# cebarker1000/heatflow

Hardware: AMD Instinct MI355X
Metric: DOF-updates/s (timesteps/s x nDOF) on geballe_with_diamond (higher is better)
Workload: dtype f64

## Files before the change

### heatflow_amd/csrc/heatflow_hip.hip

```cpp

#include "hf_amg_io.hpp"

namespace {

struct MeshTables {
  std::vector<int32_t> rowptr, colidx;
  ColDict spmv;
  RowGather rg;
  std::vector<char> tag_used;
  int max_blk_nnz = 0;
};

constexpr char BLOB_MAGIC[8] = {'H', 'F', 'P', 'A', 'T', '0', '2', 0};
struct BlobHeader {
  char magic[8];
  int64_t total_bytes, nnz;
  int32_t n, ne, rba, ts, max_blk_nnz, tab_len, rg_ok, rg_max_dict, spmv_max_dict, reserved;
  int64_t count[12];
};

void steady_swap(hf_ctx* ctx) {
  hf_ctx::Steady& S = ctx->steady;
  std::swap(ctx->nbc, S.nbc); std::swap(ctx->d_bc_dofs, S.bc_dofs); std::swap(ctx->d_g, S.g);
  std::swap(ctx->nlift_rows, S.nlift_rows); std::swap(ctx->nlift, S.nlift);
// ... 918 lines not shown
    ctx->pred_iters = 0;
    ctx->scheme = scheme;
  }
  return HF_OK;
}

int kt_set_tables(hf_ctx* ctx, bool cap, int32_t n_tab, const int32_t* tags, const double* t0, const double* dT, const int32_t* n_knots,
                  const double* values) {
  const char* fn = cap ? "hf_set_rhoc_tables" : "hf_set_kappa_tables";
  const char* what = cap ? "rho_c(T)" : "kappa(T)";
  if (!ctx) return HF_ERR_ARG;
  if (!ctx->have_mesh) return fail(ctx, HF_ERR_STATE, "%s before hf_set_mesh", fn);
  if (n_tab < 0) return fail(ctx, HF_ERR_ARG, "%s: negative table count", fn);
  HF_HIP(hipSetDevice(ctx->dev));
  hf_ctx::KappaT& K = ctx->kt;
  if (n_tab == 0) {
    if (ctx->steady.picard) ctx->steady.ready = false;
    if (cap ? K.c_on : K.k_on) {
      free_batch(ctx);
      ctx->assembled = false;
      ctx->pred_iters = 0;
    }
    if (!(cap ? K.k_on : K.c_on)) { kt_free(ctx); return HF_OK; }
    if (cap ? K.c_on : K.k_on) {
      const std::vector<KTab> none(64, KTab{0.0, 0.0, 0, 0});
      HF_HIP(copy_sync(ctx, cap ? K.chdr : K.hdr, none.data(), sizeof(KTab) * 64, hipMemcpyHostToDevice));
      dev_free(cap ? &K.cvals : &K.vals);
      (cap ? K.ctabled : K.tabled).clear();
      (cap ? K.c_on : K.k_on) = false;
      K.have_change = false;
    }
    return HF_OK;
  }
  if (!tags || !t0 || !dT || !n_knots || !values) return fail(ctx, HF_ERR_ARG, "%s: null pointer", fn);
  if (ctx->an.on) return fail(ctx, HF_ERR_STATE, "%s: anisotropic conductivities are set (hf_set_anisotropy; the table kernels are isotropic)", fn);
  if (!ctx->rg_ok || (ctx->assembled && ctx->mode != HF_ASM_ROW_GATHER))
    return fail(ctx, HF_ERR_ARG, "%s: %s is evaluated by the row-gather kernel only (HF_ASM_ROW_GATHER on a mesh with row-gather lists)", fn, what);
  if (cap && ct_smem_bytes(ctx->max_blk_nnz, ctx->rg_max_dict) + 2 * 64 * sizeof(KTab) > 160 * 1024)
    return fail(ctx, HF_ERR_ARG, "%s: the (M, A) slab, the staged state and the table headers of this mesh exceed the 160 KiB of LDS", fn);
  std::vector<KTab> hdr(64, KTab{0.0, 0.0, 0, 0});
  std::vector<double> vals;
  std::vector<char> tabled(ctx->tab_len, 0);
  for (int32_t i = 0; i < n_tab; ++i) {
    const int32_t tg = tags[i];
    if (tg < 0 || tg >= ctx->tab_len || !ctx->h_tag_used[tg]) return fail(ctx, HF_ERR_ARG, "%s: tag %d is not a cell tag of the mesh", fn, tg);
    if (tabled[tg]) return fail(ctx, HF_ERR_ARG, "%s: tag %d listed twice", fn, tg);
    if (n_knots[i] < 2 || n_knots[i] > KT_MAX_KNOTS)
      return fail(ctx, HF_ERR_ARG, "%s: table of tag %d has %d knots (2..%d)", fn, tg, n_knots[i], KT_MAX_KNOTS);
    if (!std::isfinite(t0[i]) || !(dT[i] > 0.0) || !std::isfinite(dT[i]) || !std::isfinite(t0[i] + (n_knots[i] - 1) * dT[i]))
      return fail(ctx, HF_ERR_ARG, "%s: table of tag %d: T0 finite and dT > 0 needed", fn, tg);
    tabled[tg] = 1;
    const size_t q = std::find(ctx->h_rg_tags.begin(), ctx->h_rg_tags.end(), tg) - ctx->h_rg_tags.begin();
    if (q >= ctx->h_rg_tags.size()) return fail(ctx, HF_ERR_ARG, "%s: tag %d has no row-gather dictionary entry", fn, tg);
    hdr[q] = KTab{t0[i], 1.0 / dT[i], n_knots[i], static_cast<int>(vals.size())};
    for (int32_t k = 0; k < n_knots[i]; ++k) {
      const double v = values[vals.size()];
      if (!(v > 0.0) || !std::isfinite(v)) return fail(ctx, HF_ERR_ARG, "%s: value %d of the table of tag %d is not positive and finite", fn, k, tg);
      vals.push_back(v);
    }
  }
  free_batch(ctx);
  if (ctx->steady.picard) ctx->steady.ready = false;
  if (!K.hdr) {
    HF_TRY(dev_alloc(ctx, &K.hdr, 64));
    HF_TRY(dev_alloc(ctx, &K.pic, ctx->n));
    HF_TRY(dev_alloc(ctx, &K.b0, ctx->n));
    HF_TRY(dev_alloc(ctx, &K.change, 1));
  }
  if (cap && !K.chdr) {
    HF_TRY(dev_alloc(ctx, &K.chdr, 64));
    HF_TRY(dev_alloc(ctx, &K.w, ctx->n));
    if (!K.k_on) {
      const std::vector<KTab> none(64, KTab{0.0, 0.0, 0, 0});
      HF_HIP(copy_sync(ctx, K.hdr, none.data(), sizeof(KTab) * 64, hipMemcpyHostToDevice));
    }
  }
  double*& dvals = cap ? K.cvals : K.vals;
  dev_free(&dvals);
  HF_TRY(dev_alloc(ctx, &dvals, vals.size()));
  HF_HIP(copy_sync(ctx, cap ? K.chdr : K.hdr, hdr.data(), sizeof(KTab) * 64, hipMemcpyHostToDevice));
  HF_HIP(copy_sync(ctx, dvals, vals.data(), sizeof(double) * vals.size(), hipMemcpyHostToDevice));
  (cap ? K.ctabled : K.tabled) = std::move(tabled);
  (cap ? K.c_on : K.k_on) = true;
  K.on = true;
  K.have_change = false;
  ctx->assembled = false;
  ctx->pred_iters = 0;
  return HF_OK;
}

int hf_set_kappa_tables(hf_ctx* ctx, int32_t n_tab, const int32_t* tags, const double* t0, const double* dT, const int32_t* n_knots,
                        const double* values, int32_t picard_sweeps) {
  if (ctx && ctx->have_mesh && n_tab > 0 && tags && t0 && dT && n_knots && values &&
      (picard_sweeps < 1 || picard_sweeps > KT_MAX_PICARD))
    return fail(ctx, HF_ERR_ARG, "hf_set_kappa_tables: picard_sweeps %d outside 1..%d", picard_sweeps, KT_MAX_PICARD);
  HF_TRY(kt_set_tables(ctx, false, n_tab, tags, t0, dT, n_knots, values));
  if (n_tab > 0) ctx->kt.picard = picard_sweeps;
  return HF_OK;
}

int hf_set_rhoc_tables(hf_ctx* ctx, int32_t n_tab, const int32_t* tags, const double* t0, const double* dT, const int32_t* n_knots,
                       const double* values) {
  return kt_set_tables(ctx, true, n_tab, tags, t0, dT, n_knots, values);
}

int hf_set_picard(hf_ctx* ctx, int32_t sweeps) {
  if (!ctx) return HF_ERR_ARG;
  if (sweeps < 1 || sweeps > KT_MAX_PICARD) return fail(ctx, HF_ERR_ARG, "hf_set_picard: sweeps %d outside 1..%d", sweeps, KT_MAX_PICARD);
  if (!ctx->kt.on) return fail(ctx, HF_ERR_STATE, "hf_set_picard: no tables are set (hf_set_kappa_tables / hf_set_rhoc_tables first)");
  ctx->kt.picard = sweeps;
  return HF_OK;
}

int hf_get_picard_change(hf_ctx* ctx, double* max_du) {
  if (!ctx || !max_du) return HF_ERR_ARG;
  if (!ctx->kt.on || !ctx->kt.have_change) return fail(ctx, HF_ERR_STATE, "hf_get_picard_change: no step with kappa(T) tables since they were set");
  HF_HIP(hipSetDevice(ctx->dev));
  unsigned long long bits = 0;
  HF_HIP(copy_sync(ctx, &bits, ctx->kt.change, sizeof bits, hipMemcpyDeviceToHost));
  std::memcpy(max_du, &bits, sizeof bits);
  return HF_OK;
}

int hf_set_start_vector(hf_ctx* ctx, int32_t kind) {
  if (!ctx) return HF_ERR_ARG;
  if (kind < 0 || kind > 3) return fail(ctx, HF_ERR_ARG, "hf_set_start_vector: unknown kind %d", kind);
  ctx->start_kind = kind;
  ctx->extrapolate = kind >= 1 ? 1 : 0;
  if (kind == 0) ctx->have_prev = false;
  return HF_OK;
}

int hf_get_response_solves(hf_ctx* ctx, int64_t* count) {
  if (!ctx || !count) return HF_ERR_ARG;
  *count = ctx->resp_solves;
  return HF_OK;
}

int hf_get_amg_fallbacks(hf_ctx* ctx, int64_t* count) {
  if (!ctx || !count) return HF_ERR_ARG;
  *count = ctx->amg_fallbacks;
  return HF_OK;
}

int hf_get_amg_info(hf_ctx* ctx, int32_t* n_levels, int32_t* level_rows, int32_t max_levels, double* op_complexity,
                    double* setup_seconds) {
  if (!ctx) return HF_ERR_ARG;
  const int nl = ctx->amg_ready ? static_cast<int>(ctx->amg.size()) : 0;
  if (n_levels) *n_levels = nl;
  if (level_rows)
    for (int l = 0; l < nl && l < max_levels; ++l) level_rows[l] = ctx->amg[l].n;
  if (op_complexity) *op_complexity = ctx->amg_ready ? ctx->amg_opc : 0.0;
  if (setup_seconds) *setup_seconds = ctx->amg_ready ? ctx->amg_setup_s : 0.0;
  return HF_OK;
}

int hf_amg_export_size(hf_ctx* ctx, int64_t* bytes) {
  if (!ctx || !bytes) return HF_ERR_ARG;
  if (!ctx->amg_ready || !ctx->assembled) return fail(ctx, HF_ERR_STATE, "hf_amg_export_size: no multigrid hierarchy (hf_set_precond(1, ...) and hf_assemble first)");
  BlobOut o;
  o.ctx = ctx;
  HF_TRY(walk_hierarchy(ctx, o, ctx->amg_print));
  *bytes = static_cast<int64_t>(o.at);
  return HF_OK;
}

int hf_amg_export(hf_ctx* ctx, void* blob, int64_t bytes) {
  if (!ctx || !blob) return HF_ERR_ARG;
  if (!ctx->amg_ready || !ctx->assembled) return fail(ctx, HF_ERR_STATE, "hf_amg_export: no multigrid hierarchy (hf_set_precond(1, ...) and hf_assemble first)");
  HF_HIP(hipSetDevice(ctx->dev));
  BlobOut sz;
  sz.ctx = ctx;
  HF_TRY(walk_hierarchy(ctx, sz, ctx->amg_print));
  if (bytes != static_cast<int64_t>(sz.at)) return fail(ctx, HF_ERR_ARG, "hf_amg_export: buffer of %lld bytes, need %lld", (long long)bytes, (long long)sz.at);
  std::vector<unsigned char> host(sz.at, 0);
  BlobOut o;
  o.ctx = ctx;
  o.dst = host.data();
  HF_TRY(walk_hierarchy(ctx, o, ctx->amg_print));
  HF_HIP(hipStreamSynchronize(ctx->stream));
  HF_HIP(hipMemcpy(blob, host.data(), host.size(), hipMemcpyDefault));
  return HF_OK;
}

int hf_amg_install(hf_ctx* ctx, const void* blob, int64_t bytes) {
  if (!ctx || !blob || bytes <= 0) return HF_ERR_ARG;
  if (!ctx->have_mesh) return fail(ctx, HF_ERR_STATE, "hf_amg_install before hf_set_mesh");
  if (ctx->precond != 1 || !ctx->amg_reuse) return fail(ctx, HF_ERR_STATE, "hf_amg_install needs hf_set_precond(1, reuse = 1): an installed hierarchy is a kept one");
  HF_HIP(hipSetDevice(ctx->dev));
  free_batch(ctx);
  std::vector<unsigned char> staged;
  const unsigned char* src = nullptr;
  HF_TRY(blob_on_host(ctx, blob, bytes, staged, &src));
  HF_TRY(install_hierarchy(ctx, src, static_cast<size_t>(bytes)));
  ctx->assembled = false;
  return HF_OK;
}

int hf_flux_setup(hf_ctx* ctx) {
  if (!ctx) return HF_ERR_ARG;
  if (!ctx->have_mesh) return fail(ctx, HF_ERR_STATE, "hf_flux_setup before hf_set_mesh");
  HF_HIP(hipSetDevice(ctx->dev));
  const int n = ctx->n;
  HF_TRY(dev_alloc(ctx, &ctx->d_M1, ctx->nnz));
  HF_TRY(dev_alloc(ctx, &ctx->d_dinv1, n));
  HF_TRY(dev_alloc(ctx, &ctx->d_gz, n));
  HF_TRY(dev_alloc(ctx, &ctx->d_gr, n));
  HF_TRY(dev_alloc(ctx, &ctx->d_bz, n));
  HF_TRY(dev_alloc(ctx, &ctx->d_br, n));
  const int tab = ctx->rg_ok ? 64 : ctx->tab_len;
  DevTemp<double> t_one, t_zero, t_scratch;
  double *&d_one = t_one.p, *&d_zero = t_zero.p, *&d_scratch = t_scratch.p;
  HF_TRY(dev_alloc(ctx, &d_one, tab));
  HF_TRY(dev_alloc(ctx, &d_zero, tab));
  HF_TRY(dev_alloc(ctx, &d_scratch, ctx->nnz));
  std::vector<double> ones(tab, 1.0), zeros(tab, 0.0);
  HF_HIP(copy_sync(ctx, d_one, ones.data(), sizeof(double) * tab, hipMemcpyHostToDevice));
  HF_HIP(copy_sync(ctx, d_zero, zeros.data(), sizeof(double) * tab, hipMemcpyHostToDevice));
  if (ctx->rg_ok) HF_TRY(launch_assemble_rows(ctx, d_zero, d_one, 0.0, ctx->d_M1, d_scratch));
  else HF_TRY(launch_assemble_lds(ctx, true, d_zero, d_one, 0.0, ctx->d_M1, d_scratch));
  hipLaunchKernelGGL(k_dinv, dim3((n + 255) / 256), dim3(256), 0, ctx->stream, n, ctx->d_rowptr, ctx->d_colidx,
                     ctx->d_M1, ctx->d_dinv1);
  HF_HIP(hipMemsetAsync(ctx->d_gz, 0, sizeof(double) * n, ctx->stream));
  HF_HIP(hipMemsetAsync(ctx->d_gr, 0, sizeof(double) * n, ctx->stream));
  HF_HIP(hipGetLastError());
  HF_HIP(hipStreamSynchronize(ctx->stream));
  {
    hf_ctx::Batch& F = ctx->fluxb;
    free_batch_state(F);
    const size_t vec = static_cast<size_t>(n) * 2;
    for (double** v : {&F.u, &F.b, &F.r, &F.p, &F.Ap, &F.z}) {
      HF_TRY(dev_alloc(ctx, v, vec));
      HF_HIP(hipMemsetAsync(*v, 0, sizeof(double) * vec, ctx->stream));
    }
    HF_TRY(dev_alloc(ctx, &F.part_pAp, 2 * static_cast<size_t>(MAXP)));
    HF_TRY(dev_alloc(ctx, &F.part_rz, 4 * static_cast<size_t>(MAXP)));
    HF_TRY(dev_alloc(ctx, &F.part_zz, 2 * static_cast<size_t>(MAXP)));
    HF_TRY(dev_alloc(ctx, &F.part_bn, 2 * static_cast<size_t>(MAXP)));
    HF_TRY(dev_alloc(ctx, &F.scal, 2));
    HF_TRY(dev_alloc(ctx, &F.red, 1));
    HF_HIP(hipMemsetAsync(F.scal, 0, sizeof(Scal) * 2, ctx->stream));
    HF_HIP(hipMemsetAsync(F.red, 0, sizeof(BRed), ctx->stream));
    if (hipHostMalloc(reinterpret_cast<void**>(&F.h_scal), sizeof(Scal) * 2) != hipSuccess) return fail(ctx, HF_ERR_ALLOC, "hipHostMalloc failed");
    F.Pb = static_cast<int>(std::min<size_t>((static_cast<size_t>(n) + 127) / 128, MAXP));
    if (F.Pb >= 64) F.Pb &= ~7;
    F.nv = 2; F.opk = 0; F.pred_iters = 0;
    F.sysA = ctx->d_M1; F.sysDinv = ctx->d_dinv1;
    HF_HIP(hipStreamSynchronize(ctx->stream));
  }
  ctx->flux_ready = true;
  ctx->pred_flux[0] = ctx->pred_flux[1] = 0;
  return HF_OK;
}

int hf_flux_solve(hf_ctx* ctx, int32_t components, double rtol, int32_t max_it, int32_t* iters) {
  if (!ctx) return HF_ERR_ARG;
  if (!ctx->flux_ready) return fail(ctx, HF_ERR_STATE, "hf_flux_solve before hf_flux_setup");
  if (max_it <= 0 || rtol < 0 || components < 0 || components > 3) return fail(ctx, HF_ERR_ARG, "hf_flux_solve: bad arguments");
  HF_HIP(hipSetDevice(ctx->dev));
  const bool both = components == 3 && ctx->rg_ok && ctx->fluxb.nv == 2;
  if (ctx->rg_ok) {
    const int capd = ctx->rg_max_dict;
    const size_t sm = static_cast<size_t>(capd) * 16 + static_cast<size_t>(capd + (capd & 1)) * 8 + (RBA + 4) * 4 +
                      (static_cast<size_t>((ctx->max_blk_nnz + 1) & ~1) / 8 + 3) * 16;
    const int grid = std::min(ctx->nblk_a, 2048);
    hipLaunchKernelGGL(k_grad_rows, dim3(grid), dim3(RBA), sm, ctx->stream, ctx->nblk_a, capd, ctx->d_rg_hdr,
                       reinterpret_cast<const uint4*>(ctx->d_rg_ell), reinterpret_cast<const uint4*>(ctx->d_rg_cid), ctx->d_rg_zrb,
                       ctx->d_rg_dict, ctx->d_rowptr, ctx->d_u, both ? ctx->fluxb.b : ctx->d_bz, both ? ctx->fluxb.b + 1 : ctx->d_br,
                       both ? 2 : 1, 1, 0);
  } else {
    HF_TRY(ensure_owner_lists(ctx));
    hipLaunchKernelGGL(k_grad_rhs, dim3(ctx->nblk_a), dim3(RBA), 0, ctx->stream, ctx->n, ctx->d_blk_eptr, ctx->d_blk_ent,
                       ctx->d_zr, ctx->d_u, ctx->d_bz, ctx->d_br);
  }
  HF_HIP(hipGetLastError());
  if (both) {
    std::swap(ctx->batch, ctx->fluxb);
    const int rc = BatchOps<2, OP_SHARED>::pcg(ctx, false, rtol, 0.0, max_it);
    const int it0 = ctx->batch.h_scal[0].iters, it1 = ctx->batch.h_scal[1].iters;
    std::swap(ctx->batch, ctx->fluxb);
    if (iters) { iters[0] = it0; iters[1] = it1; }
    ctx->flux_valid = 0;
    if (rc != HF_OK) return rc;
    hipLaunchKernelGGL(kb_get_column, dim3(1024), dim3(256), 0, ctx->stream, static_cast<size_t>(ctx->n), 2, 0, ctx->fluxb.u, ctx->d_gz);
    hipLaunchKernelGGL(kb_get_column, dim3(1024), dim3(256), 0, ctx->stream, static_cast<size_t>(ctx->n), 2, 1, ctx->fluxb.u, ctx->d_gr);
    HF_HIP(hipGetLastError());
    ctx->flux_valid = 3;
    return HF_OK;
  }
  if (iters) iters[0] = iters[1] = 0;
  ctx->flux_valid = 0;
  if (components & 1) {
    const LinSys sz{ctx->d_M1, ctx->d_dinv1, ctx->d_gz, ctx->d_bz};
    const int rc = pcg_solve(ctx, sz, false, rtol, 0.0, max_it, &ctx->pred_flux[0]);
    if (iters) iters[0] = ctx->h_scal->iters;
    if (rc != HF_OK) return rc;
    ctx->flux_valid |= 1;
  }
  if (components & 2) {
    const LinSys sr{ctx->d_M1, ctx->d_dinv1, ctx->d_gr, ctx->d_br};
    const int rc = pcg_solve(ctx, sr, false, rtol, 0.0, max_it, &ctx->pred_flux[1]);
    if (iters) iters[1] = ctx->h_scal->iters;
    if (rc != HF_OK) return rc;
    ctx->flux_valid |= 2;
  }
  return HF_OK;
// ... 1274 lines not shown
```

### heatflow_amd/csrc/hf_context.hpp

```cpp

#pragma once
#include <hip/hip_runtime.h>
#include <hip/hip_ext.h>

#include <algorithm>
#include <chrono>
#include <cmath>
#include <cstdarg>
#include <cstdint>
#include <cstdio>
#include <cstdlib>
#include <cstring>
#include <string>
#include <thread>
#include <vector>

#include "amg_host.hpp"
#include "heatflow_hip.h"

namespace {

constexpr int RB = 256;
#ifndef HF_RBA
#define HF_RBA 256
// ... 31 lines not shown
  unsigned long long tested_st;
};
inline int mirror_tested(const ScalMirror* m, unsigned epoch) {
  const unsigned long long v = __atomic_load_n(&m->tested_st, __ATOMIC_ACQUIRE);
  return static_cast<unsigned>(v >> 32) == epoch ? static_cast<int>(v & 0xffffffffu) - 1 : -1;
}
inline int mirror_done(const ScalMirror* m, unsigned epoch) {
  const unsigned long long v = __atomic_load_n(&m->done_st, __ATOMIC_ACQUIRE);
  return static_cast<unsigned>(v >> 32) == epoch ? static_cast<int>(v & 0xffffffffu) : 0;
}

struct Scal {
  double tol2;
  double bn2;
  double zz;
  int iters;
  int done;
  int first;
  unsigned epoch;
  ScalMirror* mirror;
};

constexpr int NV_MAX = 16;
struct BRed { double pAp[NV_MAX], rz[2][NV_MAX], zz[NV_MAX], bn[NV_MAX]; };

constexpr int KT_MAX_KNOTS = 256;
constexpr int KT_MAX_PICARD = 8;
struct KTab { double t0, inv_dt; int n, off; };

struct TanDir { int32_t c_r, c_z; double w_r, w_z; };

enum RgVariant { RG_ROWS, RG_ROWS_K, RG_AN, RG_AN_K, RG_KT, RG_CT, RG_KT_K, RG_SOURCE, RG_SHAPE1, RG_SHAPE2, RG_SHAPE4, RG_VARIANTS };

}

struct hf_ctx {
  int dev = 0;
  hipStream_t stream = nullptr;
  hipEvent_t ev0 = nullptr, ev1 = nullptr;
  std::string err;
  double last_ms = 0.0;

  int32_t n = 0, ne = 0, nbc = 0;
  int64_t nnz = 0;
  int nchunks = 0, P = 0;
  int nchunks_s = 0, Ps = 0;
  int max_chunk_nnz_s = 0;
  int32_t *d_cdict_ptr = nullptr, *d_cdict = nullptr;
  uint16_t* d_cid = nullptr;
  int max_cdict = 0;
  bool cdict_own = false;
  bool c16 = true;
  struct ValueLists {
    const double* src = nullptr;
    int32_t *vptr = nullptr, *count = nullptr, *info = nullptr;
    double* vlist = nullptr;
    uint32_t* cv = nullptr;
    int64_t cap = 0;
    int64_t sum_vlist = 0;
    int max_vlist = 0;
    bool valid = false;
  } vl[2];
  int vl_mode = 1;
  int vl_vcap = 0;
  int vl_occ = 0;
  bool have_mesh = false, have_mat = false, assembled = false;
  double dt = 0.0;
  double dt_step = 0.0;
  int mode = 0;
  int scheme = HF_TIME_BACKWARD_EULER;

  std::vector<int32_t> h_rowptr, h_colidx, h_tri, h_tag;
  std::vector<char> h_tag_used;
  bool owner_ready = false;

  double2* d_zr = nullptr;
  int4* d_elem = nullptr;
  int tab_len = 0;
  double *d_kappa = nullptr, *d_rhoc = nullptr;
  int32_t *d_rowptr = nullptr, *d_colidx = nullptr;
  int32_t *d_blk_eptr = nullptr, *d_blk_cptr = nullptr;
  int2* d_blk_ent = nullptr;
  int nblk_a = 0;
  int max_blk_nnz = 0, ncolors = 0;
  int64_t elist_len = 0;
  bool rg_ok = false;
  int4* d_rg_hdr = nullptr;
  uint16_t *d_rg_ell = nullptr, *d_rg_cid = nullptr;
  int32_t* d_rg_dict = nullptr;
  double2* d_rg_zrb = nullptr;
  int rg_max_dict = 0;
  int rg_grid[RG_VARIANTS] = {};
  int64_t n_rg_ell = 0, n_rg_dict = 0, n_cdict = 0;
  std::vector<int32_t> h_rg_tags;
  double *d_kappa_rg = nullptr, *d_rhoc_rg = nullptr;
  struct Aniso {
    bool on = false;
    double2* d_m = nullptr;
    std::vector<char> h_tag;
    std::vector<double> h_m;
    uint64_t hash = 0;
  } an;
  double *d_M = nullptr, *d_A = nullptr, *d_dinv = nullptr;
  int32_t* d_bc_dofs = nullptr;
  double* d_g = nullptr;
  int32_t nlift_rows = 0, nlift = 0;
  int32_t *d_lift_rows = nullptr, *d_lift_ptr = nullptr, *d_lift_bc = nullptr, *d_lift_slot = nullptr;
  double* d_lift_val = nullptr;
  double *d_u = nullptr, *d_b = nullptr, *d_r = nullptr, *d_p = nullptr, *d_Ap = nullptr;
  double *d_uprev = nullptr, *d_ustart = nullptr;
  bool have_prev = false;
  bool bdf_hist = false;
  int extrapolate = 1;
  int start_kind = 3;
  std::vector<double> h_g0, h_g1;
  int g_hist = 0;
  struct BcResponse { std::vector<double> dir; double* w = nullptr; };
  std::vector<BcResponse> resp;
  long long resp_solves = 0;
  struct Proj {
    double *V[PROJ_MT] = {nullptr}, *F[PROJ_MT] = {nullptr};
    bool used[PROJ_MT] = {false};
    int next = 0, pending = -1;
    double *G = nullptr, *alpha = nullptr, *part = nullptr;
    bool ready = false;
  } proj;
  double *d_tmp = nullptr;
  double *d_part_pAp = nullptr, *d_part_rz = nullptr, *d_part_zz = nullptr, *d_part_bn = nullptr;
  Scal* d_scal = nullptr;
  Scal* h_scal = nullptr;
  ScalMirror* h_mirror = nullptr;
  ScalMirror* d_mirror = nullptr;
  unsigned epoch = 0;
  int32_t* d_samp_idx = nullptr;
  double* d_samp = nullptr;
  int samp_cap = 0;
  int pred_iters = 0;
  int precond = 0;
  int amg_reuse = 0;
  bool amg_ready = false;
  struct DevCsr {
    int nrow = 0, ncol = 0, lanes = 8; int64_t nnz = 0; int32_t *ptr = nullptr, *idx = nullptr; double* val = nullptr;
    float* valf = nullptr;
    int max_row = 0;
    int rpc = 0, nchunks = 0, chunk_nnz = 0;
    int32_t *dptr = nullptr, *dict = nullptr;
    uint16_t* cid = nullptr;
    int max_dict = 0;
    int64_t ndict = 0;
  };
  struct DevLevel {
    DevCsr A, P, R, Rt, GP;
    double *dinv = nullptr, *x = nullptr, *cat = nullptr, *b = nullptr, *res = nullptr;
    bool own_b = false;
    double omega = 0; int n = 0;
  };
  std::vector<DevLevel> amg;
  double* d_coarse_inv = nullptr;
  float* d_coarse_inv_f = nullptr;
  int coarse_n = 0, coarse_ld = 0;
  bool amg_fine_stale = false;
  int amg_fuse0 = 0;
  bool amg_f32 = true;
  double amg_opc = 0.0, amg_setup_s = 0.0;
  struct OperatorPrint { double dt = 0.0; std::vector<double> kappa, rhoc; int32_t nbc = 0; uint64_t bc_hash = 0; int32_t scheme = 0; uint64_t an_hash = 0; } amg_print;
  long long amg_fallbacks = 0;
  struct Steady {
    bool ready = false;
    bool picard = false;
    KTab* hdr0 = nullptr;
    double* xprev = nullptr;
    unsigned long long* change = nullptr;
    int precond = 0, pred_iters = 0;
    int32_t nbc = 0, nlift_rows = 0, nlift = 0;
    int32_t *bc_dofs = nullptr, *lift_rows = nullptr, *lift_ptr = nullptr, *lift_bc = nullptr, *lift_slot = nullptr;
    double *g = nullptr, *lift_val = nullptr, *K = nullptr, *dinv = nullptr, *Kfree = nullptr;
    std::vector<DevLevel> amg;
    double* coarse_inv = nullptr;
    float* coarse_inv_f = nullptr;
    int coarse_n = 0, coarse_ld = 0;
    bool amg_ready = false, amg_fine_stale = false;
    double amg_opc = 0.0, amg_setup_s = 0.0;
    OperatorPrint amg_print;
  } steady;
  double* d_load = nullptr;
  bool have_load = false;
  struct Source {
    bool on = false;
    double* F1 = nullptr;
    double* sum = nullptr;
    int32_t* absorb = nullptr;
    std::vector<double> amp;
    size_t next = 0;
  } src;
  double *d_z = nullptr, *d_z2 = nullptr;
  bool flux_ready = false;
  int flux_valid = 0;
  double *d_M1 = nullptr, *d_dinv1 = nullptr, *d_gz = nullptr, *d_gr = nullptr, *d_bz = nullptr, *d_br = nullptr;
  int pred_flux[2] = {0, 0};
  struct BatchLevel { double *x = nullptr, *cat = nullptr, *b = nullptr, *res = nullptr; bool own_b = false; };
  struct Batch {
    int nv = 0;
    int opk = 0;
    const double *sysA = nullptr, *sysDinv = nullptr;
    double *A = nullptr, *dinv = nullptr, *lift_val = nullptr;
    double *A1 = nullptr, *lift1 = nullptr;
    double delta[NV_MAX] = {};
    double *g = nullptr;
    double *u = nullptr, *uprev = nullptr, *ustart = nullptr, *b = nullptr, *r = nullptr, *p = nullptr, *Ap = nullptr;
    double *z = nullptr, *z2 = nullptr, *tmp = nullptr;
    double *part_pAp = nullptr, *part_rz = nullptr, *part_zz = nullptr, *part_bn = nullptr;
    Scal *scal = nullptr, *h_scal = nullptr;
    ScalMirror *h_mirror = nullptr, *d_mirror = nullptr;
    unsigned epoch = 0;
    BRed* red = nullptr;
    std::vector<BatchLevel> lev;
    int Pb = 0, pred_iters = 0;
    bool have_prev = false;
    bool bdf_hist = false;
    double *pV[PROJ_MH] = {nullptr}, *pF[PROJ_MH] = {nullptr}, *pG = nullptr, *palpha = nullptr, *ppart = nullptr;
    bool pused[PROJ_MH] = {false};
    int pnext = 0, ppending = -1;
    unsigned loaded = 0;
    bool lds = false;
    const double* load = nullptr;
  } batch;
  struct BatchCols {
    int nv = 0, rpc = 0, nchunks = 0, cap_nnz = 0, cap_dict = 0;
    int32_t *ptr = nullptr, *dict = nullptr, *own = nullptr;
    uint16_t* id = nullptr;
  } bcols;
  Batch fluxb;
  Batch fluxnb;
  int32_t* d_fsamp_idx = nullptr;
  Batch tanb;
  struct Tangent {
    bool ready = false;
    int npar = 0, nv = 0;
    int32_t* col = nullptr;
    TanDir* dir = nullptr;
    double* F = nullptr;
    bool steady_state = false;
    std::vector<int64_t> lev_sig;
    struct Shape {
      int ncol = 0, ns = 0;
      int32_t col[4] = {0, 0, 0, 0};
      std::vector<double> h_v[4];
      double* d_v = nullptr;
      double *un = nullptr, *um1 = nullptr;
      int wmode = 0;
      bool hist = false;
    } sh;
  } tan;
  int fsamp_cap = 0;
  struct KappaT {
    bool on = false;
    bool k_on = false, c_on = false;
    int picard = 1;
    KTab* hdr = nullptr;
    double* vals = nullptr;
    std::vector<char> tabled;
    KTab* chdr = nullptr;
    double* cvals = nullptr;
    std::vector<char> ctabled;
    double* w = nullptr;
    double *pic = nullptr, *b0 = nullptr;
    unsigned long long* change = nullptr;
    bool have_change = false;
  } kt;
  bool prof = false;
  std::vector<hipEvent_t> prof_ev;
  int prof_used = 0, prof_base = 0;
  double prof_spmv_ms = 0.0;
  long long prof_spmv_n = 0;
};

namespace {

int fail(hf_ctx* c, int code, const char* fmt, ...);
inline size_t pad16(size_t b) { return (b + 15) & ~static_cast<size_t>(15); }

inline void cpu_relax() {
#if defined(__x86_64__) || defined(__i386__)
  __builtin_ia32_pause();
#else
  std::this_thread::yield();
#endif
}

hipError_t copy_sync(hf_ctx* ctx, void* dst, const void* src, size_t bytes, hipMemcpyKind kind) {
  if (bytes == 0) return hipSuccess;
  const hipError_t e = hipMemcpyAsync(dst, src, bytes, kind, ctx->stream);
  return e != hipSuccess ? e : hipStreamSynchronize(ctx->stream);
}

int fail(hf_ctx* c, int code, const char* fmt, ...) {
  char buf[512];
  va_list ap;
  va_start(ap, fmt);
  vsnprintf(buf, sizeof buf, fmt, ap);
  va_end(ap);
  if (c) c->err = buf;
  return code;
}

#define HF_HIP(call)                                                                          \
// ... 34 lines not shown
```

### heatflow_amd/csrc/hf_kernels.hpp

```cpp
#pragma once
#include <type_traits>

#include "hf_context.hpp"

namespace {


template <int NW = 4>
__device__ __forceinline__ double block_sum(double v, double* sw) {
#pragma unroll
  for (int o = 32; o > 0; o >>= 1) v += __shfl_down(v, o, 64);
  const int w = threadIdx.x >> 6;
  if ((threadIdx.x & 63) == 0) sw[w] = v;
  __syncthreads();
  double t = sw[0];
#pragma unroll
  for (int k = 1; k < NW; ++k) t += sw[k];
  __syncthreads();
  return t;
}

__device__ __forceinline__ double sum_partials(const double* __restrict__ part, int P, double* s4) {
  double v = 0.0;
  for (int k = threadIdx.x; k < P; k += TPB) v += part[k];
  return block_sum(v, s4);
}

#ifndef HF_XCD_MAP
#define HF_XCD_MAP 1
#endif
struct ChunkIter {
  int chunk, step, end;
  __device__ __forceinline__ ChunkIter(int nchunks) {
    if (HF_XCD_MAP && (gridDim.x & 7) == 0) {
      const int per = (nchunks + 7) >> 3;
      const int xcd = blockIdx.x & 7;
      chunk = xcd * per + (blockIdx.x >> 3);
      step = gridDim.x >> 3;
      end = min(nchunks, (xcd + 1) * per);
    } else {
      chunk = blockIdx.x;
      step = gridDim.x;
      end = nchunks;
    }
  }
};

__device__ __forceinline__ void element_local(const double2 p0, const double2 p1, const double2 p2, double rho_c,
                                              double kappa, double m[6], double k[6]) {
#pragma clang fp contract(off)
  const double d = (p1.x - p0.x) * (p2.y - p0.y) - (p2.x - p0.x) * (p1.y - p0.y);
  const double area = 0.5 * fabs(d);
  const double b0 = p1.y - p2.y, b1 = p2.y - p0.y, b2 = p0.y - p1.y;
  const double c0 = p2.x - p1.x, c1 = p0.x - p2.x, c2 = p1.x - p0.x;
  const double rsum = (p0.y + p1.y) + p2.y;
  const double ks = kappa * area * (rsum / 3.0) / (d * d);
  k[0] = ks * (b0 * b0 + c0 * c0);
  k[1] = ks * (b1 * b1 + c1 * c1);
  k[2] = ks * (b2 * b2 + c2 * c2);
  k[3] = ks * (b0 * b1 + c0 * c1);
  k[4] = ks * (b0 * b2 + c0 * c2);
  k[5] = ks * (b1 * b2 + c1 * c2);
  const double ms = rho_c * area;
  m[0] = ms * ((2.0 * p0.y + rsum) / 30.0);
  m[1] = ms * ((2.0 * p1.y + rsum) / 30.0);
  m[2] = ms * ((2.0 * p2.y + rsum) / 30.0);
  m[3] = ms * ((rsum + p0.y + p1.y) / 60.0);
  m[4] = ms * ((rsum + p0.y + p2.y) / 60.0);
  m[5] = ms * ((rsum + p1.y + p2.y) / 60.0);
}

__device__ __forceinline__ int sym_index(int a, int b) {
  return a == b ? a : (a + b + 2);
}

struct AsmEntry { int n0, n1, n2; unsigned w3, off03, off47; };

__device__ __forceinline__ AsmEntry load_entry(const int2* __restrict__ ent, int q) {
  const int2 a = ent[3 * q], b = ent[3 * q + 1], c = ent[3 * q + 2];
  return AsmEntry{a.x, a.y, b.x, static_cast<unsigned>(b.y), static_cast<unsigned>(c.x), static_cast<unsigned>(c.y)};
}

template <bool COLORED>
__global__ __launch_bounds__(RBA) void k_assemble_lds(int n, int cap, const int32_t* __restrict__ rowptr,
                                                      const int32_t* __restrict__ blk_eptr,
                                                      const int32_t* __restrict__ blk_cptr,
                                                      const int2* __restrict__ blk_ent,
                                                      const double2* __restrict__ zr,
                                                      const double* __restrict__ kappa_tab,
                                                      const double* __restrict__ rhoc_tab, double dt,
                                                      double* __restrict__ Mv, double* __restrict__ Av) {
  extern __shared__ double smem[];
  double2* sMA = reinterpret_cast<double2*>(smem);
  double* sM = smem;
  double* sA = smem + cap;
  int* sR = reinterpret_cast<int*>(smem + 2 * cap);

  const int blk = blockIdx.x;
  const int r0 = blk * RBA;
  const int r1 = min(n, r0 + RBA);
  const int k0 = rowptr[r0];
  const int nk = rowptr[r1] - k0;
  for (int k = threadIdx.x; k < nk; k += RBA) {
    if (COLORED) {
      sMA[k] = make_double2(0.0, 0.0);
    } else {
      sM[k] = 0.0;
      sA[k] = 0.0;
    }
  }
  for (int k = threadIdx.x; k <= r1 - r0; k += RBA) sR[k] = rowptr[r0 + k] - k0;
  __syncthreads();

  auto scatter = [&](const AsmEntry e, const double2 p0, const double2 p1, const double2 p2) {
    double m[6], kk[6], av6[6];
    const int tag = static_cast<int>(e.w3 >> 11);
    element_local(p0, p1, p2, rhoc_tab[tag], kappa_tab[tag], m, kk);
#pragma unroll
    for (int q = 0; q < 6; ++q) av6[q] = fma(dt, kk[q], m[q]);
    const int nd[3] = {e.n0, e.n1, e.n2};
#pragma unroll
    for (int a = 0; a < 3; ++a) {
      if (!((e.w3 >> (8 + a)) & 1u)) continue;
      const int base = sR[nd[a] - r0];
#pragma unroll
      for (int b = 0; b < 3; ++b) {
        const int q9 = a * 3 + b;
        const unsigned off = q9 < 4 ? (e.off03 >> (8 * q9)) & 0xFFu : q9 < 8 ? (e.off47 >> (8 * (q9 - 4))) & 0xFFu : e.w3 & 0xFFu;
        const int slot = base + static_cast<int>(off);
        const int q = sym_index(a, b);
        if (COLORED) {
          double2 t = sMA[slot];
          t.x += m[q];
          t.y += av6[q];
          sMA[slot] = t;
        } else {
          atomicAdd(&sM[slot], m[q]);
          atomicAdd(&sA[slot], av6[q]);
        }
      }
    }
  };
  constexpr int NF = 3;
  auto run_range = [&](int e0, int e1) {
    for (int k = e0 + threadIdx.x; k < e1; k += NF * RBA) {
      AsmEntry e[NF];
      double2 pa[NF], pb[NF], pc[NF];
#pragma unroll
      for (int u = 0; u < NF; ++u) e[u] = load_entry(blk_ent, min(k + u * RBA, e1 - 1));
#pragma unroll
      for (int u = 0; u < NF; ++u) { pa[u] = zr[e[u].n0]; pb[u] = zr[e[u].n1]; pc[u] = zr[e[u].n2]; }
#pragma unroll
      for (int u = 0; u < NF; ++u)
        if (k + u * RBA < e1) scatter(e[u], pa[u], pb[u], pc[u]);
    }
  };

  if (COLORED) {
    const int32_t* cp = blk_cptr + static_cast<size_t>(blk) * (NCOL + 1);
    for (int c = 0; c < NCOL; ++c) {
      const int e0 = cp[c], e1 = cp[c + 1];
      if (e0 == e1) { if (e1 == cp[NCOL]) break; else continue; }
      run_range(e0, e1);
      __syncthreads();
    }
  } else {
    run_range(blk_eptr[blk], blk_eptr[blk + 1]);
  }
  __syncthreads();
  for (int k = threadIdx.x; k < nk; k += RBA) {
    if (COLORED) {
      const double2 t = sMA[k];
      Mv[k0 + k] = t.x;
      Av[k0 + k] = t.y;
    } else {
      Mv[k0 + k] = sM[k];
      Av[k0 + k] = sA[k];
    }
  }
}

struct ElemRow { double m0, m1, m2, k0, k1, k2; };

__device__ __forceinline__ double sorted_sum3(double a, double b, double c) {
#pragma clang fp contract(off)
  const double ab_lo = fmin(a, b), ab_hi = fmax(a, b);
  const double lo = fmin(ab_lo, c), hi = fmax(ab_hi, c), mid = fmax(ab_lo, fmin(ab_hi, c));
  return (lo + mid) + hi;
}

template <bool ANISO>
__device__ __forceinline__ ElemRow element_row_of(const double2 Pi, const double2 Pj, const double2 Pk, double rho_c, double k_z, double k_r) {
#pragma clang fp contract(off)
  const double eix = Pk.x - Pj.x, eiy = Pk.y - Pj.y;
  const double ejx = Pi.x - Pk.x, ejy = Pi.y - Pk.y;
// ... 777 lines not shown
#pragma clang fp contract(off)
    const AsmEntry e = load_entry(blk_ent, q);
    const double2 p0 = zr[e.n0], p1 = zr[e.n1], p2 = zr[e.n2];
    const double u0 = u[e.n0], u1 = u[e.n1], u2 = u[e.n2];
    const double d = (p1.x - p0.x) * (p2.y - p0.y) - (p2.x - p0.x) * (p1.y - p0.y);
    const double area = 0.5 * fabs(d);
    const double gz = (u0 * (p1.y - p2.y) + u1 * (p2.y - p0.y) + u2 * (p0.y - p1.y)) / d;
    const double gr = (u0 * (p2.x - p1.x) + u1 * (p0.x - p2.x) + u2 * (p1.x - p0.x)) / d;
    const double rsum = (p0.y + p1.y) + p2.y;
    const double wgt[3] = {area * (p0.y + rsum) / 12.0, area * (p1.y + rsum) / 12.0, area * (p2.y + rsum) / 12.0};
    const int nd[3] = {e.n0, e.n1, e.n2};
    const unsigned owned = (e.w3 >> 8) & 7u;
#pragma unroll
    for (int a = 0; a < 3; ++a) {
      if (!((owned >> a) & 1u)) continue;
      atomicAdd(&sB[2 * (nd[a] - r0)], gz * wgt[a]);
      atomicAdd(&sB[2 * (nd[a] - r0) + 1], gr * wgt[a]);
    }
  }
  __syncthreads();
  for (int k = threadIdx.x; k < r1 - r0; k += RBA) {
    bz[r0 + k] = sB[2 * k];
    br[r0 + k] = sB[2 * k + 1];
  }
}

__global__ void k_take_lift(int nlift, const int32_t* __restrict__ slot, double* __restrict__ A,
                            double* __restrict__ val) {
  const int q = blockIdx.x * blockDim.x + threadIdx.x;
  if (q >= nlift) return;
  val[q] = A[slot[q]];
  A[slot[q]] = 0.0;
}

__global__ void k_bc_rows(int nbc, const int32_t* __restrict__ dofs, const int32_t* __restrict__ rowptr,
                          const int32_t* __restrict__ colidx, double* __restrict__ A) {
  const int q = blockIdx.x * blockDim.x + threadIdx.x;
  if (q >= nbc) return;
  const int row = dofs[q];
  for (int k = rowptr[row]; k < rowptr[row + 1]; ++k) A[k] = (colidx[k] == row) ? 1.0 : 0.0;
}

__global__ void k_dinv(int n, const int32_t* __restrict__ rowptr, const int32_t* __restrict__ colidx,
                       const double* __restrict__ A, double* __restrict__ dinv) {
  const int row = blockIdx.x * blockDim.x + threadIdx.x;
  if (row >= n) return;
  double d = 0.0;
  for (int k = rowptr[row]; k < rowptr[row + 1]; ++k)
    if (colidx[k] == row) d = A[k];
  dinv[row] = 1.0 / d;
}

__global__ void k_lift(int nrows, const int32_t* __restrict__ rows, const int32_t* __restrict__ ptr,
                       const int32_t* __restrict__ bc, const double* __restrict__ val,
                       const double* __restrict__ g, double* __restrict__ b) {
  const int q = blockIdx.x * blockDim.x + threadIdx.x;
  if (q >= nrows) return;
  double s = 0.0;
  for (int k = ptr[q]; k < ptr[q + 1]; ++k) s += val[k] * g[bc[k]];
  b[rows[q]] -= s;
}

__global__ void k_set_bc(int nbc, const int32_t* __restrict__ dofs, const double* __restrict__ g,
                         double* __restrict__ b, double* __restrict__ u) {
  const int q = blockIdx.x * blockDim.x + threadIdx.x;
  if (q >= nbc) return;
  b[dofs[q]] = g[q];
  u[dofs[q]] = g[q];
}

__global__ void k_gather(int ns, const int32_t* __restrict__ idx, const double* __restrict__ u,
                         double* __restrict__ out) {
  const int q = blockIdx.x * blockDim.x + threadIdx.x;
  if (q < ns) out[q] = u[idx[q]];
}

__global__ __launch_bounds__(TPB) void k_hold_load(int n, const int32_t* __restrict__ rowptr, const int32_t* __restrict__ colidx,
                                                   const double* __restrict__ K, const double* __restrict__ u,
                                                   const unsigned char* __restrict__ mask, double* __restrict__ F) {
  const int row = blockIdx.x * blockDim.x + threadIdx.x;
  if (row >= n) return;
  double s = 0.0;
  if (!mask[row])
    for (int k = rowptr[row]; k < rowptr[row + 1]; ++k) s += K[k] * u[colidx[k]];
  F[row] = s;
}

__global__ void k_mark_rows(int nq, const int32_t* __restrict__ idx, unsigned char* __restrict__ mask) {
  const int q = blockIdx.x * blockDim.x + threadIdx.x;
  if (q < nq) mask[idx[q]] = 1;
}

__device__ __forceinline__ unsigned long long mirror_stamp(unsigned epoch, int v) {
  return (static_cast<unsigned long long>(epoch) << 32) | static_cast<unsigned>(v);
}
__device__ __forceinline__ void mirror_publish(ScalMirror* m, double zz, int iters, int done, unsigned epoch) {
  if (m == nullptr) return;
  m->zz = zz;
  m->iters = iters;
  __hip_atomic_store(&m->done_st, mirror_stamp(epoch, done), __ATOMIC_RELAXED, __HIP_MEMORY_SCOPE_SYSTEM);
  __threadfence_system();
  __hip_atomic_store(&m->tested_st, mirror_stamp(epoch, iters + 1), __ATOMIC_RELEASE, __HIP_MEMORY_SCOPE_SYSTEM);
}
__device__ __forceinline__ void mirror_breakdown(ScalMirror* m, unsigned epoch) {
  if (m != nullptr) __hip_atomic_store(&m->done_st, mirror_stamp(epoch, 2), __ATOMIC_RELEASE, __HIP_MEMORY_SCOPE_SYSTEM);
}

struct ColComp { const int32_t* dptr; const int32_t* dict; const uint16_t* id; int xd_off; int own; };
struct ValComp : ColComp { const int32_t* vptr; const double* vlist; const uint32_t* cv; int vl_off; int vcap; };

#ifndef HF_NT_STREAM
#define HF_NT_STREAM 0
#endif
#ifndef HF_PIPE
#define HF_PIPE 1
#endif
#ifndef HF_PHASE_CLOCK
#define HF_PHASE_CLOCK -1
#endif
#if HF_PHASE_CLOCK >= 0
#ifndef HF_PHASE_CONV
#define HF_PHASE_CONV 0
#endif
__device__ unsigned long long g_phase[MAXP * 16];
#define HF_STAMP(slot)                                                                                   \
  do {                                                                                                   \
    if (MODE == HF_PHASE_CLOCK && C16 && (MODE != 0 || (part2 != nullptr) == (HF_PHASE_CONV != 0)) && threadIdx.x == 0 && (slot) < 16) \
      g_phase[blockIdx.x * 16 + (slot)] = wall_clock64();                                                \
  } while (0)
#else
#define HF_STAMP(slot) do { } while (0)
#endif
template <typename T>
__device__ __forceinline__ T stream_load(const T* p) {
#if HF_NT_STREAM
  return __builtin_nontemporal_load(p);
#else
  return *p;
#endif
}

__device__ __forceinline__ double bdf2_operand(double un, double unm1) { return (4.0 * un - unm1) * (1.0 / 3.0); }

template <int MODE, bool C16 = false, typename VT = double, int UN = 8, bool VC = false>
__global__ __launch_bounds__(TS) __attribute__((amdgpu_waves_per_eu(8, 8))) void k_spmv(int n, int nchunks, int rpc ,
                                              const int32_t* __restrict__ rowptr, const int32_t* __restrict__ colidx,
                                              const VT* __restrict__ vals, const double* __restrict__ x,
                                              double* __restrict__ y, Scal* __restrict__ scal,
                                              double* __restrict__ part0, const double* __restrict__ bvec,
                                              const double* __restrict__ dinv, double* __restrict__ pvec,
                                              double* __restrict__ part1, double* __restrict__ part2, double w,
                                              int npart ,
                                              int parity, typename std::conditional<VC, ValComp, ColComp>::type comp) {
  extern __shared__ double sprod[];
  __shared__ double s4[TS / 64];
  __shared__ int s_own;
  constexpr bool BDF = MODE >= 12 && MODE <= 15;
  auto opnd = [&](int c) { return BDF ? bdf2_operand(x[c], bvec[c]) : x[c]; };
  if ((MODE == 3 || MODE == 4 || MODE == 6 || MODE == 9) && scal->done) return;
  if ((MODE == 0 || MODE == 7) && scal != nullptr && scal->done) return;
  double acc0 = 0.0, acc1 = 0.0, acc2 = 0.0;
  double beta = 0.0;
  bool first9 = false;
  if (MODE == 9) {
    first9 = scal->first != 0;
    if (!first9) {
      double v0 = 0.0, v1 = 0.0, v2 = 0.0;
      for (int k = threadIdx.x; k < npart; k += TS) {
        v0 += part1[parity * MAXP + k];
        v1 += part1[(parity ^ 1) * MAXP + k];
        v2 += part2[k];
      }
      const double rz_new = block_sum<TS / 64>(v0, s4);
      const double rz_old = block_sum<TS / 64>(v1, s4);
      const double zz = block_sum<TS / 64>(v2, s4);
      const bool conv = zz <= scal->tol2;
      if (blockIdx.x == 0 && threadIdx.x == 0) {
        scal->zz = zz;
        if (conv) scal->done = 1;
      }
      if (conv) return;
      beta = rz_new / rz_old;
    }
  }
  auto cycle_gate = [&]() {
    if (!((MODE == 3 || MODE == 0) && part2 != nullptr)) return false;
    double v2 = 0.0;
    for (int k = threadIdx.x; k < npart; k += TS) v2 += part2[k];
    const double zz = block_sum<TS / 64>(v2, s4);
    const bool conv = zz <= scal->tol2;
    if (blockIdx.x == 0 && threadIdx.x == 0) {
      if (conv) { scal->zz = zz; scal->done = 1; }
      mirror_publish(scal->mirror, zz, scal->iters, conv ? 1 : 0, scal->epoch);
    }
    return conv;
  };
  constexpr bool PIPELINED = C16 && !VC && (HF_PIPE == 2 || (HF_PIPE == 1 && sizeof(VT) == 4));
  static_assert(!VC || (C16 && sizeof(VT) == 8), "value lists: the fine operator's f64 arrays on compressed columns");
  if (!PIPELINED && cycle_gate()) return;
  const ChunkIter sched(nchunks);
  HF_STAMP(0);
  int stamp_at = 1;
  (void)stamp_at;
  const int tpr = (MODE == 0 || MODE == 6 || MODE == 7) ? TS / rpc : 1;
  const int prel = static_cast<int>(threadIdx.x) / tpr;
  const int psub = static_cast<int>(threadIdx.x) % tpr;
  struct RowOps { double b, d, y, p, x; };
  auto row_operands = [&](int prc, bool from_slice) {
    RowOps e{0.0, 0.0, 0.0, 0.0, 0.0};
    if (MODE == 2 || MODE == 3 || MODE == 4 || MODE == 5 || MODE == 7 || MODE == 8 || MODE == 11 || MODE == 13 || MODE == 15) e.b = bvec[prc];
    if (MODE == 2 || MODE == 4 || MODE == 5 || MODE == 10 || MODE == 11 || MODE == 14 || MODE == 15) e.d = dinv[prc];
    if (MODE == 6 || (MODE == 9 && !first9)) e.y = y[prc];
    if (MODE == 9 && !first9) e.p = pvec[prc];
    if ((MODE == 4 || MODE == 8 || MODE == 9 || MODE == 11) && !from_slice) e.x = x[prc];
    if (BDF) e.x = x[prc];
    return e;
  };
  auto rows_phase = [&](bool pin, int prow, int pa, int pb, const RowOps& e) {
    if ((MODE == 0 || MODE == 6 || MODE == 7) && tpr > 1) {
      double s = 0.0;
      if (pin)
        for (int j = pa + psub; j < pb; j += tpr) s += sprod[j];
      for (int o = tpr >> 1; o > 0; o >>= 1) s += __shfl_down(s, o, 64);
      if (pin && psub == 0) {
        y[prow] = (MODE == 6) ? e.y + s : s;
        if (MODE == 7) acc0 += e.b * s;
      }
    } else if (pin) {
      const int row = prow;
      double s = 0.0;
      for (int j = pa; j < pb; ++j) s += sprod[j];
      if (MODE == 0) {
        y[row] = s;
      } else if (MODE == 2) {
        const double ri = e.b - s;
        const double zi = e.d * ri;
        y[row] = ri;
        pvec[row] = zi;
        acc0 += ri * zi;
        acc1 += zi * zi;
        acc2 += (e.d * e.b) * (e.d * e.b);
      } else if (MODE == 3) {
        y[row] = e.b - s;
      } else if (MODE == 4) {
        const double yi = e.x + w * e.d * (e.b - s);
        y[row] = yi;
        acc0 += e.b * yi;
      } else if (MODE == 5) {
        const double ri = e.b - s;
        y[row] = ri;
        pvec[row] = w * e.d * ri;
        acc1 += (e.d * ri) * (e.d * ri);
        acc2 += (e.d * e.b) * (e.d * e.b);
      } else if (MODE == 7) {
        y[row] = s;
        acc0 += e.b * s;
      } else if (MODE == 6) {
        y[row] = e.y + s;
      } else if (MODE == 8) {
        y[row] = s;
        pvec[row] = 2.0 * e.x - e.b;
      } else if (MODE == 10) {
        y[row] = s + w * e.d;
      } else if (MODE == 11) {
        y[row] = s + w * e.d;
        pvec[row] = 2.0 * e.x - e.b;
      } else if (BDF) {
        y[row] = (MODE == 14 || MODE == 15) ? s + w * e.d : s;
        pvec[row] = (MODE == 13 || MODE == 15) ? 2.0 * e.x - e.b : e.x;
      } else {
        const double api = first9 ? s : s + beta * e.y;
        const double pi = first9 ? e.x : e.x + beta * e.p;
        y[row] = api;
        pvec[row] = pi;
        acc0 += pi * api;
      }
    }
  };
  if (PIPELINED) {
    struct Bounds { int k0, k1, d0, d1; };
    auto bounds = [&](int ch) {
      Bounds q;
      const int a0 = ch * rpc, a1 = min(n, a0 + rpc);
      q.k0 = rowptr[a0]; q.k1 = rowptr[a1];
      q.d0 = comp.dptr[ch]; q.d1 = comp.dptr[ch + 1];
      return q;
    };
    int lhead[HF_STAGE_U];
    double v[UN];
    int id[UN];
    auto heads = [&](const Bounds& q, bool live) {
      const int dl = max(q.d1 - 1, 0), kl = max(q.k1 - 1, 0);
      const int t = static_cast<int>(threadIdx.x);
#pragma unroll
      for (int u = 0; u < HF_STAGE_U; ++u) lhead[u] = comp.dict[min(q.d0 + (live ? t + u * TS : (t & 31)), dl)];
      __builtin_amdgcn_sched_barrier(0);
#pragma unroll
      for (int u = 0; u < UN; ++u) {
        const int kk = min(q.k0 + (live ? t + u * TS : (t & 31)), kl);
        v[u] = static_cast<double>(stream_load(&vals[kk]));
        id[u] = static_cast<int>(stream_load(&comp.id[kk]));
      }
    };
    double* xd = sprod + comp.xd_off;
    Bounds cur = bounds(min(sched.chunk, nchunks - 1));
    heads(cur, sched.chunk < sched.end);
    if (cycle_gate()) return;
    for (int chunk = sched.chunk; chunk < sched.end; chunk += sched.step) {
      const bool more = chunk + sched.step < sched.end;
      const int r0 = chunk * rpc, r1 = min(n, r0 + rpc);
      const int k0 = cur.k0, k1 = cur.k1, d0 = cur.d0, nd = cur.d1 - cur.d0;
      const int prow = r0 + prel;
      const bool pin = prow < r1;
      const int prc = min(prow, r1 - 1);
      int c0[HF_STAGE_U];
      double x0[HF_STAGE_U];
#pragma unroll
      for (int u = 0; u < HF_STAGE_U; ++u) { c0[u] = lhead[u]; x0[u] = opnd(c0[u]); }
      const Bounds nxt = bounds(more ? chunk + sched.step : chunk);
      const int pa = rowptr[prc] - k0, pb = rowptr[prc + 1] - k0;
      RowOps e = row_operands(prc, comp.own != 0);
#pragma unroll
      for (int u = 0; u < HF_STAGE_U; ++u) {
        const int i = static_cast<int>(threadIdx.x) + u * TS;
        if (i < nd) {
          xd[i] = x0[u];
          if ((MODE == 4 || MODE == 8 || MODE == 9 || MODE == 11) && c0[u] == r0) s_own = i;
        }
      }
      for (int i = threadIdx.x + HF_STAGE_U * TS; i < nd; i += HF_STAGE_U * TS) {
        int c[HF_STAGE_U];
        double xv[HF_STAGE_U];
#pragma unroll
        for (int u = 0; u < HF_STAGE_U; ++u) c[u] = comp.dict[d0 + min(i + u * TS, nd - 1)];
#pragma unroll
        for (int u = 0; u < HF_STAGE_U; ++u) xv[u] = opnd(c[u]);
#pragma unroll
        for (int u = 0; u < HF_STAGE_U; ++u)
          if (i + u * TS < nd) {
            xd[i + u * TS] = xv[u];
            if ((MODE == 4 || MODE == 8 || MODE == 9 || MODE == 11) && c[u] == r0) s_own = i + u * TS;
          }
      }
      __syncthreads();
      HF_STAMP(stamp_at); ++stamp_at;
      if ((MODE == 4 || MODE == 8 || MODE == 9 || MODE == 11) && comp.own && pin) e.x = xd[s_own + (prow - r0)];
#pragma unroll
      for (int u = 0; u < UN; ++u) {
        const int kk = k0 + static_cast<int>(threadIdx.x) + u * TS;
        if (kk < k1) sprod[kk - k0] = v[u] * xd[id[u]];
      }
      for (int kb = k0 + UN * TS; kb < k1; kb += UN * TS) {
#pragma unroll
        for (int u = 0; u < UN; ++u) {
          const int kk = min(kb + static_cast<int>(threadIdx.x) + u * TS, k1 - 1);
          v[u] = static_cast<double>(stream_load(&vals[kk]));
          id[u] = static_cast<int>(stream_load(&comp.id[kk]));
        }
#pragma unroll
        for (int u = 0; u < UN; ++u) {
          const int kk = kb + static_cast<int>(threadIdx.x) + u * TS;
          if (kk < k1) sprod[kk - k0] = v[u] * xd[id[u]];
        }
      }
      heads(nxt, more);
      __syncthreads();
      HF_STAMP(stamp_at); ++stamp_at;
      rows_phase(pin, prow, pa, pb, e);
      __syncthreads();
      HF_STAMP(stamp_at); ++stamp_at;
      cur = nxt;
    }
  } else {
  const ChunkIter& sched_ = sched;
  for (int chunk = sched_.chunk; chunk < sched_.end; chunk += sched_.step) {
    const int r0 = chunk * rpc;
    const int r1 = min(n, r0 + rpc);
    const int k0 = rowptr[r0];
    const int k1 = rowptr[r1];
    const int prow = r0 + prel;
    const bool pin = prow < r1;
    int pa = 0, pb = 0;
    if (pin) {
      pa = rowptr[prow] - k0;
      pb = rowptr[prow + 1] - k0;
    }
    RowOps e = row_operands(min(prow, r1 - 1), C16 && comp.own != 0);
    if constexpr (VC) {
      double* xd = sprod + comp.xd_off;
      double* vl = sprod + comp.vl_off;
      const int d0 = comp.dptr[chunk], nd = comp.dptr[chunk + 1] - d0;
      const int v0 = comp.vptr[chunk], nv = comp.vptr[chunk + 1] - v0;
      const bool vin = nv <= comp.vcap;
      int k = k0 + threadIdx.x;
      std::uint32_t cw[HF_UNROLL];
#pragma unroll
      for (int u = 0; u < HF_UNROLL; ++u) cw[u] = (k + u * TS < k1) ? stream_load(&comp.cv[k + u * TS]) : 0u;
      double lv[2];
#pragma unroll
      for (int u = 0; u < 2; ++u) {
        const int i = static_cast<int>(threadIdx.x) + u * TS;
        lv[u] = (vin && i < nv) ? comp.vlist[v0 + i] : 0.0;
      }
      for (int i = threadIdx.x; i < nd; i += HF_STAGE_U * TS) {
        int c[HF_STAGE_U];
        double xv[HF_STAGE_U];
#pragma unroll
        for (int u = 0; u < HF_STAGE_U; ++u) c[u] = (i + u * TS < nd) ? comp.dict[d0 + i + u * TS] : 0;
#pragma unroll
        for (int u = 0; u < HF_STAGE_U; ++u) xv[u] = (i + u * TS < nd) ? opnd(c[u]) : 0.0;
#pragma unroll
        for (int u = 0; u < HF_STAGE_U; ++u)
          if (i + u * TS < nd) {
            xd[i + u * TS] = xv[u];
            if ((MODE == 4 || MODE == 8 || MODE == 9 || MODE == 11) && c[u] == r0) s_own = i + u * TS;
          }
      }
#pragma unroll
      for (int u = 0; u < 2; ++u) {
        const int i = static_cast<int>(threadIdx.x) + u * TS;
        if (vin && i < nv) vl[i] = lv[u];
      }
      if (vin)
        for (int i = threadIdx.x + 2 * TS; i < nv; i += TS) vl[i] = comp.vlist[v0 + i];
      __syncthreads();
      HF_STAMP(stamp_at); ++stamp_at;
      if ((MODE == 4 || MODE == 8 || MODE == 9 || MODE == 11) && comp.own && pin) e.x = xd[s_own + (prow - r0)];
      while (k < k1) {
        const int kn = k + HF_UNROLL * TS;
        std::uint32_t cn[HF_UNROLL];
#pragma unroll
        for (int u = 0; u < HF_UNROLL; ++u) cn[u] = (kn + u * TS < k1) ? stream_load(&comp.cv[kn + u * TS]) : 0u;
        if (vin) {
#pragma unroll
          for (int u = 0; u < HF_UNROLL; ++u)
            if (k + u * TS < k1) sprod[k - k0 + u * TS] = vl[cw[u] >> 16] * xd[cw[u] & 0xffffu];
        } else {
          double gv[HF_UNROLL];
#pragma unroll
          for (int u = 0; u < HF_UNROLL; ++u) gv[u] = (k + u * TS < k1) ? comp.vlist[v0 + static_cast<int>(cw[u] >> 16)] : 0.0;
#pragma unroll
          for (int u = 0; u < HF_UNROLL; ++u)
            if (k + u * TS < k1) sprod[k - k0 + u * TS] = gv[u] * xd[cw[u] & 0xffffu];
        }
#pragma unroll
        for (int u = 0; u < HF_UNROLL; ++u) cw[u] = cn[u];
        k = kn;
      }
    } else if (C16) {
      double* xd = sprod + comp.xd_off;
      const int d0 = comp.dptr[chunk], nd = comp.dptr[chunk + 1] - d0;
      int k = k0 + threadIdx.x;
      double v[HF_UNROLL];
      int id[HF_UNROLL];
#pragma unroll
      for (int u = 0; u < HF_UNROLL; ++u) {
        const bool in = k + u * TS < k1;
        v[u] = in ? static_cast<double>(stream_load(&vals[k + u * TS])) : 0.0;
        id[u] = in ? static_cast<int>(stream_load(&comp.id[k + u * TS])) : 0;
      }
      for (int i = threadIdx.x; i < nd; i += HF_STAGE_U * TS) {
        int c[HF_STAGE_U];
        double xv[HF_STAGE_U];
#pragma unroll
        for (int u = 0; u < HF_STAGE_U; ++u) c[u] = (i + u * TS < nd) ? comp.dict[d0 + i + u * TS] : 0;
#pragma unroll
        for (int u = 0; u < HF_STAGE_U; ++u) xv[u] = (i + u * TS < nd) ? opnd(c[u]) : 0.0;
#pragma unroll
        for (int u = 0; u < HF_STAGE_U; ++u)
          if (i + u * TS < nd) {
            xd[i + u * TS] = xv[u];
            if ((MODE == 4 || MODE == 8 || MODE == 9 || MODE == 11) && c[u] == r0) s_own = i + u * TS;
          }
      }
      __syncthreads();
      HF_STAMP(stamp_at); ++stamp_at;
      if ((MODE == 4 || MODE == 8 || MODE == 9 || MODE == 11) && comp.own && pin) e.x = xd[s_own + (prow - r0)];
      while (k < k1) {
        const int kn = k + HF_UNROLL * TS;
        double vn[HF_UNROLL];
        int idn[HF_UNROLL];
#pragma unroll
        for (int u = 0; u < HF_UNROLL; ++u) {
          const bool in = kn + u * TS < k1;
          vn[u] = in ? static_cast<double>(stream_load(&vals[kn + u * TS])) : 0.0;
          idn[u] = in ? static_cast<int>(stream_load(&comp.id[kn + u * TS])) : 0;
        }
#pragma unroll
        for (int u = 0; u < HF_UNROLL; ++u)
          if (k + u * TS < k1) sprod[k - k0 + u * TS] = v[u] * xd[id[u]];
#pragma unroll
        for (int u = 0; u < HF_UNROLL; ++u) { v[u] = vn[u]; id[u] = idn[u]; }
        k = kn;
      }
    } else {
      for (int k = k0 + threadIdx.x; k < k1; k += HF_UNROLL * TS) {
        int c[HF_UNROLL];
        double v[HF_UNROLL], xv[HF_UNROLL];
#pragma unroll
        for (int u = 0; u < HF_UNROLL; ++u) {
          const bool in = k + u * TS < k1;
          c[u] = in ? colidx[k + u * TS] : 0;
          v[u] = in ? static_cast<double>(vals[k + u * TS]) : 0.0;
        }
#pragma unroll
        for (int u = 0; u < HF_UNROLL; ++u) xv[u] = (k + u * TS < k1) ? opnd(c[u]) : 0.0;
#pragma unroll
        for (int u = 0; u < HF_UNROLL; ++u)
          if (k + u * TS < k1) sprod[k - k0 + u * TS] = v[u] * xv[u];
      }
    }
    __syncthreads();
    HF_STAMP(stamp_at); ++stamp_at;
    rows_phase(pin, prow, pa, pb, e);
    __syncthreads();
    HF_STAMP(stamp_at); ++stamp_at;
  }
  }
  if (MODE == 2 || MODE == 7 || MODE == 9 || (MODE == 4 && part0 != nullptr)) {
    const double t0 = block_sum<TS / 64>(acc0, s4);
    if (threadIdx.x == 0) {
      part0[blockIdx.x] = t0;
      for (int q = blockIdx.x + gridDim.x; q < npart; q += gridDim.x) part0[q] = 0.0;
    }
  }
  if (MODE == 2 || MODE == 5) {
    const double t1 = block_sum<TS / 64>(acc1, s4);
    const double t2 = block_sum<TS / 64>(acc2, s4);
    if (threadIdx.x == 0) {
      part1[blockIdx.x] = t1;
      part2[blockIdx.x] = t2;
      for (int q = blockIdx.x + gridDim.x; q < npart; q += gridDim.x) { part1[q] = 0.0; part2[q] = 0.0; }
    }
  }
}

constexpr int VL_MAX_CHUNK = 4096;

template <int NW>
__device__ __forceinline__ int block_scan_incl(int v, int* sw, int& total) {
  const int lane = threadIdx.x & 63, w = threadIdx.x >> 6;
#pragma unroll
  for (int o = 1; o < 64; o <<= 1) {
    const int t = __shfl_up(v, o, 64);
    if (lane >= o) v += t;
  }
  if (lane == 63) sw[w] = v;
  __syncthreads();
  int before = 0;
  total = 0;
#pragma unroll
  for (int q = 0; q < NW; ++q) {
    const int t = sw[q];
    if (q < w) before += t;
    total += t;
  }
  __syncthreads();
  return v + before;
}

__global__ __launch_bounds__(TS) void k_vl_ids(int n, int nchunks, int rpc, const int32_t* __restrict__ rowptr,
                                               const double* __restrict__ vals, const uint16_t* __restrict__ cid,
                                               std::uint32_t* __restrict__ cv, int32_t* __restrict__ count) {
  __shared__ unsigned long long skey[VL_MAX_CHUNK];
  __shared__ uint16_t sorg[VL_MAX_CHUNK];
  __shared__ int sw[TS / 64];
  const int tid = static_cast<int>(threadIdx.x);
  for (int chunk = blockIdx.x; chunk < nchunks; chunk += gridDim.x) {
    const int r0 = chunk * rpc, r1 = min(n, r0 + rpc);
    const int k0 = rowptr[r0], m = min(rowptr[r1] - k0, VL_MAX_CHUNK);
    int np = 64;
    while (np < m) np <<= 1;
    for (int i = tid; i < np; i += TS) {
      skey[i] = i < m ? static_cast<unsigned long long>(__double_as_longlong(vals[k0 + i])) : ~0ull;
      sorg[i] = static_cast<uint16_t>(i);
    }
    __syncthreads();
    for (int size = 2; size <= np; size <<= 1)
      for (int stride = size >> 1; stride > 0; stride >>= 1) {
        for (int t = tid; t < (np >> 1); t += TS) {
          const int lo = 2 * t - (t & (stride - 1)), hi = lo + stride;
          const bool up = (lo & size) == 0;
          const unsigned long long ka = skey[lo], kb = skey[hi];
          const uint16_t oa = sorg[lo], ob = sorg[hi];
          const bool gt = ka > kb || (ka == kb && oa > ob);
          if (gt == up) { skey[lo] = kb; skey[hi] = ka; sorg[lo] = ob; sorg[hi] = oa; }
        }
        __syncthreads();
      }
    const int per = (np + TS - 1) / TS;
    const int i0 = tid * per;
    int heads = 0;
    for (int j = 0; j < per; ++j) {
      const int i = i0 + j;
      if (i < m && (i == 0 || skey[i] != skey[i - 1])) ++heads;
    }
    int total = 0;
    int run = block_scan_incl<TS / 64>(heads, sw, total) - heads;
    for (int j = 0; j < per; ++j) {
      const int i = i0 + j;
      if (i < m) {
        if (i == 0 || skey[i] != skey[i - 1]) ++run;
        const int k = k0 + sorg[i];
        cv[k] = static_cast<std::uint32_t>(cid[k]) | (static_cast<std::uint32_t>(run - 1) << 16);
      }
    }
    if (tid == 0) count[chunk] = total;
    __syncthreads();
  }
}

__global__ __launch_bounds__(1024) void k_vl_scan(int nchunks, const int32_t* __restrict__ count, int32_t* __restrict__ vptr,
                                                  int32_t* __restrict__ info) {
  __shared__ int sw[16];
  __shared__ int smax[16];
  const int tid = static_cast<int>(threadIdx.x);
  int carry = 0, mx = 0;
  for (int base = 0; base < nchunks; base += 1024) {
    const int i = base + tid;
    const int v = i < nchunks ? count[i] : 0;
    mx = max(mx, v);
    int total = 0;
    const int incl = block_scan_incl<16>(v, sw, total);
    if (i < nchunks) vptr[i] = carry + incl - v;
    carry += total;
  }
#pragma unroll
  for (int o = 32; o > 0; o >>= 1) mx = max(mx, __shfl_down(mx, o, 64));
  if ((tid & 63) == 0) smax[tid >> 6] = mx;
  __syncthreads();
  if (tid == 0) {
    for (int q = 1; q < 16; ++q) mx = max(mx, smax[q]);
    vptr[nchunks] = carry;
    info[0] = carry;
    info[1] = mx;
  }
}

__global__ __launch_bounds__(TS) void k_vl_lists(int n, int nchunks, int rpc, const int32_t* __restrict__ rowptr,
                                                 const double* __restrict__ vals, const std::uint32_t* __restrict__ cv,
                                                 const int32_t* __restrict__ vptr, long long cap, double* __restrict__ vlist) {
  if (vptr[nchunks] > cap) return;
  for (int chunk = blockIdx.x; chunk < nchunks; chunk += gridDim.x) {
    const int r0 = chunk * rpc, r1 = min(n, r0 + rpc);
    const int k0 = rowptr[r0], k1 = rowptr[r1], v0 = vptr[chunk];
    for (int k = k0 + threadIdx.x; k < k1; k += TS) vlist[v0 + static_cast<int>(cv[k] >> 16)] = vals[k];
  }
}

__global__ __launch_bounds__(TPB) void k_pcg_begin(int P, double rtol, double atol, const double* __restrict__ part_zz,
                                                   const double* __restrict__ part_bn, Scal* __restrict__ scal, unsigned epoch) {
  __shared__ double s4[4];
  const double zz = sum_partials(part_zz, P, s4);
  const double bn2 = sum_partials(part_bn, P, s4);
  if (threadIdx.x == 0) {
    const double tol = fmax(rtol * sqrt(bn2 > 0.0 ? bn2 : zz), atol);
    scal->tol2 = tol * tol;
    scal->bn2 = bn2;
    scal->zz = zz;
    scal->iters = 0;
    scal->first = 1;
    scal->done = (zz <= tol * tol) ? 1 : 0;
    scal->epoch = epoch;
    if (scal->mirror != nullptr) scal->mirror->bn2 = bn2;
    mirror_publish(scal->mirror, zz, 0, scal->done, epoch);
  }
}

__global__ __launch_bounds__(TPB) void k_pcg_update(int n, int nchunks, int P, int parity, Scal* __restrict__ scal,
                                                    const double* __restrict__ part_pAp, double* __restrict__ part_rz,
                                                    double* __restrict__ part_zz, double* __restrict__ x,
                                                    double* __restrict__ r, const double* __restrict__ p,
                                                    const double* __restrict__ Ap, const double* __restrict__ dinv,
                                                    double* __restrict__ z) {
  __shared__ double s4[4];
  if (scal->done) return;
  const double pAp = sum_partials(part_pAp, P, s4);
  const double rz = sum_partials(part_rz + parity * MAXP, P, s4);
  if (!(pAp > 0.0)) {
    if (blockIdx.x == 0 && threadIdx.x == 0) {
      scal->done = 2;
      mirror_breakdown(scal->mirror, scal->epoch);
    }
    return;
  }
  if (blockIdx.x == 0 && threadIdx.x == 0) { scal->iters += 1; scal->first = 0; }
  const double alpha = rz / pAp;
  double a_rz = 0.0, a_zz = 0.0;
  const ChunkIter sched(nchunks);
  for (int chunk = sched.chunk; chunk < sched.end; chunk += sched.step) {
    const int i = chunk * RB + threadIdx.x;
    if (i < n) {
      const double ri = r[i] - alpha * Ap[i];
      const double zi = dinv[i] * ri;
      x[i] += alpha * p[i];
      r[i] = ri;
      z[i] = zi;
      a_rz += ri * zi;
      a_zz += zi * zi;
    }
  }
  const double t0 = block_sum(a_rz, s4);
  const double t1 = block_sum(a_zz, s4);
  if (threadIdx.x == 0) {
    part_rz[(parity ^ 1) * MAXP + blockIdx.x] = t0;
    part_zz[blockIdx.x] = t1;
  }
}

template <int LANES, int VMODE, typename VT = double>
__global__ __launch_bounds__(TPB) void k_spmv_vec(int nrow, const int32_t* __restrict__ ptr,
                                                  const int32_t* __restrict__ idx, const VT* __restrict__ val,
                                                  const double* __restrict__ x, double* __restrict__ y,
                                                  const Scal* __restrict__ scal) {
  if (scal->done) return;
  const int lane = threadIdx.x % LANES;
  const int rows_per_pass = (gridDim.x * TPB) / LANES;
  for (int row = (blockIdx.x * TPB + threadIdx.x) / LANES; row < nrow; row += rows_per_pass) {
    const int k1 = ptr[row + 1];
    const double y0 = (VMODE == 1 && lane == 0) ? y[row] : 0.0;
    double s = 0.0;
    for (int k = ptr[row] + lane; k < k1; k += 4 * LANES) {
      int c[4];
      double v[4], xv[4];
#pragma unroll
      for (int u = 0; u < 4; ++u) {
        const bool in = k + u * LANES < k1;
        c[u] = in ? idx[k + u * LANES] : 0;
        v[u] = in ? static_cast<double>(val[k + u * LANES]) : 0.0;
      }
#pragma unroll
      for (int u = 0; u < 4; ++u) xv[u] = (k + u * LANES < k1) ? x[c[u]] : 0.0;
#pragma unroll
      for (int u = 0; u < 4; ++u) s += v[u] * xv[u];
    }
#pragma unroll
    for (int o = LANES / 2; o > 0; o >>= 1) s += __shfl_down(s, o, LANES);
    if (lane == 0) y[row] = (VMODE == 1) ? y0 + s : s;
  }
}

template <int VMODE, typename VT = double>
__global__ __launch_bounds__(TPB) void k_spmv_row(int nrow, const int32_t* __restrict__ ptr,
                                                  const int32_t* __restrict__ idx, const VT* __restrict__ val,
                                                  const double* __restrict__ x, double* __restrict__ y,
                                                  const Scal* __restrict__ scal) {
  __shared__ double s4[TPB / 64];
  if (scal->done) return;
  for (int row = blockIdx.x; row < nrow; row += gridDim.x) {
    const int k1 = ptr[row + 1];
    const double y0 = (VMODE == 1 && threadIdx.x == 0) ? y[row] : 0.0;
    double s = 0.0;
    for (int k = ptr[row] + threadIdx.x; k < k1; k += 4 * TPB) {
      int c[4];
      double v[4], xv[4];
#pragma unroll
      for (int u = 0; u < 4; ++u) {
        const bool in = k + u * TPB < k1;
        c[u] = in ? idx[k + u * TPB] : 0;
        v[u] = in ? static_cast<double>(val[k + u * TPB]) : 0.0;
      }
#pragma unroll
      for (int u = 0; u < 4; ++u) xv[u] = (k + u * TPB < k1) ? x[c[u]] : 0.0;
#pragma unroll
      for (int u = 0; u < 4; ++u) s += v[u] * xv[u];
    }
    const double t = block_sum<TPB / 64>(s, s4);
    if (threadIdx.x == 0) y[row] = (VMODE == 1) ? y0 + t : t;
  }
}

struct RespArgs { const double* w[MAXRESP]; double c[MAXRESP]; int k; };
__global__ __launch_bounds__(TPB) void k_start_vector(int n, const double* __restrict__ base, RespArgs a,
                                                      double* __restrict__ u) {
  for (int i = blockIdx.x * TPB + threadIdx.x; i < n; i += gridDim.x * TPB) {
    double s = base[i];
    for (int k = 0; k < a.k; ++k) s += a.c[k] * a.w[k][i];
    u[i] = s;
  }
}

struct ProjVecs { const double* V[PROJ_MT]; int slot[PROJ_MT]; int m; };

__global__ __launch_bounds__(TPB) void k_proj_dots(int n, ProjVecs a, const double* __restrict__ f, const double* __restrict__ Fnew,
                                                   double* __restrict__ part ) {
  __shared__ double sw[TPB / 64][2 * PROJ_MT];
  double ah[PROJ_MT], ag[PROJ_MT];
#pragma unroll
  for (int k = 0; k < PROJ_MT; ++k) { ah[k] = 0.0; ag[k] = 0.0; }
  const int stride = gridDim.x * TPB;
  for (int i = blockIdx.x * TPB + threadIdx.x; i < n; i += 2 * stride) {
    const int i2 = i + stride;
    const bool two = i2 < n;
    const double fi = f ? f[i] : 0.0, gi = Fnew ? Fnew[i] : 0.0;
    const double fj = (f && two) ? f[i2] : 0.0, gj = (Fnew && two) ? Fnew[i2] : 0.0;
    double v0[PROJ_MT], v1[PROJ_MT];
#pragma unroll
    for (int k = 0; k < PROJ_MT; ++k) {
      v0[k] = k < a.m ? a.V[k][i] : 0.0;
      v1[k] = (k < a.m && two) ? a.V[k][i2] : 0.0;
    }
#pragma unroll
    for (int k = 0; k < PROJ_MT; ++k) {
      ah[k] += v0[k] * fi;
      ag[k] += v0[k] * gi;
      ah[k] += v1[k] * fj;
      ag[k] += v1[k] * gj;
    }
  }
  const int lane = threadIdx.x & 63, wave = threadIdx.x >> 6;
#pragma unroll
  for (int k = 0; k < PROJ_MT; ++k)
    if (k < a.m) {
      double th = ah[k], tg = ag[k];
#pragma unroll
      for (int o = 32; o > 0; o >>= 1) { th += __shfl_down(th, o, 64); tg += __shfl_down(tg, o, 64); }
      if (lane == 0) { sw[wave][2 * k] = th; sw[wave][2 * k + 1] = tg; }
    }
  __syncthreads();
  if (static_cast<int>(threadIdx.x) < 2 * a.m) {
    double t = sw[0][threadIdx.x];
#pragma unroll
    for (int w = 1; w < TPB / 64; ++w) t += sw[w][threadIdx.x];
    part[threadIdx.x * MAXP + blockIdx.x] = t;
  }
}

static_assert(PROJ_MT * PROJ_MT <= 1024, "k_proj_solve holds one matrix entry per thread");
constexpr int PROJ_SOLVE_T = 1024;
__global__ __launch_bounds__(PROJ_SOLVE_T) void k_proj_solve(int P, ProjVecs a, int jnew, int do_solve, double* __restrict__ part,
                                                    double* __restrict__ G , double* __restrict__ alpha) {
  __shared__ double sh[PROJ_MT], sg[PROJ_MT];
  __shared__ double A[PROJ_MT][PROJ_MT + 1], bb[PROJ_MT], dd[PROJ_MT], xx[PROJ_MT];
  __shared__ int perm[PROJ_MT], piv, stop, rank_s;
  __shared__ double pmax;
  part += static_cast<size_t>(blockIdx.x) * 2 * PROJ_MT * MAXP;
  G += blockIdx.x * PROJ_MT * PROJ_MT;
  alpha += blockIdx.x * (PROJ_MT + 1);
  const int m = a.m, t = threadIdx.x, lane = t & 63, wave = t >> 6;
  for (int q = wave; q < 2 * m; q += PROJ_SOLVE_T / 64) {
    double v = 0.0;
    for (int k0 = 0; k0 < P; k0 += 256) {
      double e[4];
#pragma unroll
      for (int u = 0; u < 4; ++u) { const int k = k0 + lane + 64 * u; e[u] = k < P ? part[q * MAXP + k] : 0.0; }
      v += (e[0] + e[1]) + (e[2] + e[3]);
    }
#pragma unroll
    for (int o = 32; o > 0; o >>= 1) v += __shfl_down(v, o, 64);
    if (lane == 0) { if (q & 1) sg[q >> 1] = v; else sh[q >> 1] = v; }
  }
  __syncthreads();
  if (jnew >= 0 && t < m) { G[a.slot[t] * PROJ_MT + jnew] = sg[t]; G[jnew * PROJ_MT + a.slot[t]] = sg[t]; }
  if (!do_solve) return;
  __syncthreads();
  if (t < PROJ_MT + 1) alpha[t] = 0.0;
  if (t < m) {
    double gii = (jnew >= 0 && a.slot[t] == jnew) ? sg[t] : G[a.slot[t] * PROJ_MT + a.slot[t]];
    const bool ok = gii > 0.0 && gii < 1e300;
    dd[t] = ok ? 1.0 / sqrt(gii) : 0.0;
    perm[t] = t;
    xx[t] = 0.0;
  }
  __syncthreads();
  const int i = t / PROJ_MT, j = t % PROJ_MT;
  if (i < m && j < m) {
    double gij;
    if (jnew >= 0 && a.slot[j] == jnew) gij = sg[i];
    else if (jnew >= 0 && a.slot[i] == jnew) gij = sg[j];
    else gij = G[a.slot[i] * PROJ_MT + a.slot[j]];
    const bool ok = dd[i] > 0.0 && dd[j] > 0.0;
    A[i][j] = ok ? gij * dd[i] * dd[j] : (i == j ? 0.0 : 0.0);
  }
  if (t < m) bb[t] = sh[t] * dd[t];
  if (t == 0) { rank_s = 0; stop = 0; }
  __syncthreads();
  for (int c = 0; c < m; ++c) {
    if (t == 0) {
      int pi = c;
      double best = A[c][c];
      for (int q = c + 1; q < m; ++q)
        if (A[q][q] > best) { best = A[q][q]; pi = q; }
      if (c == 0) pmax = best;
      piv = pi;
      stop = !(best > 1e-12 * pmax) || !(best > 0.0);
    }
    __syncthreads();
    if (stop) break;
    const int pv = piv;
    if (pv != c) {
      if (t < m) { const double x0 = A[c][t]; A[c][t] = A[pv][t]; A[pv][t] = x0; }
      __syncthreads();
      if (t < m) { const double x0 = A[t][c]; A[t][c] = A[t][pv]; A[t][pv] = x0; }
// ... 128 lines not shown
      const int nv = ld >> 2;
      for (int j = (wave & 1) * 64 + lane; j < nv; j += 128) {
        const float4 a = arow[j];
        const double2 v0 = bv[2 * j], v1 = bv[2 * j + 1];
        s += static_cast<double>(a.x) * v0.x + static_cast<double>(a.y) * v0.y + static_cast<double>(a.z) * v1.x + static_cast<double>(a.w) * v1.y;
      }
    }
#pragma unroll
    for (int o = 32; o > 0; o >>= 1) s += __shfl_down(s, o, 64);
    if (lane == 0) half_sum[wave] = s;
    __syncthreads();
    if (lane == 0 && (wave & 1) == 0 && row < n) x[row] = half_sum[wave] + half_sum[wave + 1];
    __syncthreads();
  }
}

__global__ void k_to_float(size_t n, const double* __restrict__ src, float* __restrict__ dst) {
  for (size_t i = static_cast<size_t>(blockIdx.x) * blockDim.x + threadIdx.x; i < n; i += static_cast<size_t>(gridDim.x) * blockDim.x)
    dst[i] = static_cast<float>(src[i]);
}

constexpr int GJ_B = 32;
__global__ __launch_bounds__(TPB) void k_gjb_rows(int n, int c0, int b, const double* __restrict__ W, double* __restrict__ R ) {
  __shared__ double D[GJ_B][GJ_B + 1], Di[GJ_B][GJ_B + 1];
  const int t = threadIdx.x, ld = 2 * n;
  for (int q = t; q < GJ_B * GJ_B; q += TPB) {
    const int r = q / GJ_B, c = q % GJ_B;
    D[r][c] = (r < b && c < b) ? W[static_cast<size_t>(c0 + r) * ld + c0 + c] : (r == c ? 1.0 : 0.0);
    Di[r][c] = r == c ? 1.0 : 0.0;
  }
  __syncthreads();
  for (int p = 0; p < b; ++p) {
    const double piv = D[p][p];
    __syncthreads();
    for (int q = t; q < 2 * GJ_B; q += TPB) {
      if (q < GJ_B) D[p][q] /= piv; else Di[p][q - GJ_B] /= piv;
    }
    __syncthreads();
    for (int q = t; q < GJ_B * 2 * GJ_B; q += TPB) {
      const int r = q / (2 * GJ_B), c = q % (2 * GJ_B);
      if (r == p) continue;
      const double f = D[r][p];
      if (c < GJ_B) { if (c != p) D[r][c] -= f * D[p][c]; } else Di[r][c - GJ_B] -= f * Di[p][c - GJ_B];
    }
    __syncthreads();
    for (int r = t; r < GJ_B; r += TPB)
      if (r != p) D[r][p] = 0.0;
    __syncthreads();
  }
  for (int j = blockIdx.x * TPB + t; j < n; j += gridDim.x * TPB) {
    const size_t col = static_cast<size_t>(c0 + b + j);
    double w[GJ_B];
#pragma unroll
    for (int r = 0; r < GJ_B; ++r) w[r] = r < b ? W[static_cast<size_t>(c0 + r) * ld + col] : 0.0;
    for (int r = 0; r < b; ++r) {
      double s = 0.0;
#pragma unroll
      for (int c = 0; c < GJ_B; ++c) s += Di[r][c] * w[c];
      R[static_cast<size_t>(r) * n + j] = s;
    }
  }
}

__global__ void k_gjb_fill(int n, const int32_t* __restrict__ ptr, const int32_t* __restrict__ idx, const double* __restrict__ val,
                           double* __restrict__ W) {
  const int i = blockIdx.x * blockDim.x + threadIdx.x;
  if (i >= n) return;
  double* w = W + static_cast<size_t>(i) * 2 * n;
  for (int k = ptr[i]; k < ptr[i + 1]; ++k) w[idx[k]] = val[k];
  w[n + i] = 1.0;
}

__global__ __launch_bounds__(TPB) void k_gjb_update(int n, int c0, int b, double* __restrict__ W, const double* __restrict__ R) {
  __shared__ double sC[64][GJ_B + 1], sR[GJ_B][64 + 1];
  const int ld = 2 * n, t = threadIdx.x;
  const int i0 = blockIdx.y * 64, j0 = blockIdx.x * 64;
  for (int q = t; q < 64 * GJ_B; q += TPB) {
    const int r = q / GJ_B, c = q % GJ_B;
    sC[r][c] = (i0 + r < n && c < b) ? W[static_cast<size_t>(i0 + r) * ld + c0 + c] : 0.0;
  }
  for (int q = t; q < GJ_B * 64; q += TPB) {
    const int r = q / 64, c = q % 64;
    sR[r][c] = (r < b && j0 + c < n) ? R[static_cast<size_t>(r) * n + j0 + c] : 0.0;
  }
  __syncthreads();
  const int ti = (t / 16) * 4, tj = (t % 16) * 4;
  double acc[4][4];
#pragma unroll
  for (int u = 0; u < 4; ++u)
#pragma unroll
    for (int v = 0; v < 4; ++v) acc[u][v] = 0.0;
  for (int k = 0; k < GJ_B; ++k) {
    double cu[4], rv[4];
#pragma unroll
    for (int u = 0; u < 4; ++u) cu[u] = sC[ti + u][k];
#pragma unroll
    for (int v = 0; v < 4; ++v) rv[v] = sR[k][tj + v];
#pragma unroll
    for (int u = 0; u < 4; ++u)
#pragma unroll
      for (int v = 0; v < 4; ++v) acc[u][v] += cu[u] * rv[v];
  }
#pragma unroll
  for (int u = 0; u < 4; ++u) {
    const int i = i0 + ti + u;
    if (i >= n) continue;
    const bool pivot_row = i >= c0 && i < c0 + b;
#pragma unroll
    for (int v = 0; v < 4; ++v) {
      const int j = j0 + tj + v;
      if (j >= n) continue;
      double* w = W + static_cast<size_t>(i) * ld + c0 + b + j;
      *w = pivot_row ? sR[i - c0][tj + v] : *w - acc[u][v];
    }
  }
}

__global__ __launch_bounds__(TPB) void k_pcg_update_amg(int n, int nchunks, int P, int parity, Scal* __restrict__ scal,
                                                        const double* __restrict__ part_pAp,
                                                        const double* __restrict__ part_rz, double* __restrict__ part_zz,
                                                        double* __restrict__ x, double* __restrict__ r,
                                                        const double* __restrict__ p, const double* __restrict__ Ap,
                                                        const double* __restrict__ dinv, double w, double* __restrict__ z0) {
  __shared__ double s4[4];
  if (scal->done) return;
  const double pAp = sum_partials(part_pAp, P, s4);
  const double rz = sum_partials(part_rz + parity * MAXP, P, s4);
  if (!(pAp > 0.0)) {
    if (blockIdx.x == 0 && threadIdx.x == 0) {
      scal->done = 2;
      mirror_breakdown(scal->mirror, scal->epoch);
    }
    return;
  }
  if (blockIdx.x == 0 && threadIdx.x == 0) { scal->iters += 1; scal->first = 0; }
  const double alpha = rz / pAp;
  double a_zz = 0.0;
  const ChunkIter sched(nchunks);
  for (int chunk = sched.chunk; chunk < sched.end; chunk += sched.step) {
    const int i = chunk * RB + threadIdx.x;
    if (i < n) {
      const double ri = r[i] - alpha * Ap[i];
      const double zi = dinv[i] * ri;
      x[i] += alpha * p[i];
      r[i] = ri;
      if (z0 != nullptr) z0[i] = w * zi;
      a_zz += zi * zi;
    }
  }
  const double t1 = block_sum(a_zz, s4);
  if (threadIdx.x == 0) part_zz[blockIdx.x] = t1;
}

}
```

### heatflow_amd/csrc/hf_solver.hpp

```cpp
#pragma once
#include "hf_pattern.hpp"

namespace {

using DevCsr = hf_ctx::DevCsr;
using DevLevel = hf_ctx::DevLevel;

void free_dev_csr(DevCsr& m) { dev_free(&m.ptr); dev_free(&m.idx); dev_free(&m.val); dev_free(&m.valf); dev_free(&m.dptr); dev_free(&m.dict); dev_free(&m.cid); m = DevCsr(); }

void free_amg(hf_ctx* ctx) {
  for (size_t l = 0; l < ctx->amg.size(); ++l) {
    DevLevel& L = ctx->amg[l];
    if (l > 0) { free_dev_csr(L.A); dev_free(&L.dinv); dev_free(&L.x); dev_free(&L.cat); }
    if (L.own_b) dev_free(&L.b);
    free_dev_csr(L.P); free_dev_csr(L.R); free_dev_csr(L.Rt); free_dev_csr(L.GP);
  }
  ctx->amg.clear();
  dev_free(&ctx->d_coarse_inv);
  dev_free(&ctx->d_coarse_inv_f);
  ctx->coarse_n = 0;
  ctx->amg_ready = false;
}

int lanes_for_avg(double avg) {
// ... 151 lines not shown
                          hipMemcpyDeviceToDevice, ctx->stream));
  HF_HIP(hipStreamSynchronize(ctx->stream));
  return HF_OK;
}

int finish_amg(hf_ctx* ctx, const amg::Csr& Ac, int coarse_n, double op_complexity, const std::chrono::steady_clock::time_point t0) {
  const bool f32 = ctx->amg_f32;
  const size_t nl = ctx->amg.size();
  auto lap = [&](const char* what) {
    if (std::getenv("HEATFLOW_DEBUG")) std::fprintf(stderr, "[amg setup] %-28s %.3f s\n", what, std::chrono::duration<double>(std::chrono::steady_clock::now() - t0).count());
  };
  {
    DevLevel& L = ctx->amg[0];
    if (L.Rt.nrow > 0 && (L.Rt.rpc == 0 || (L.GP.nrow > 0 && L.GP.rpc == 0))) {
      free_dev_csr(L.Rt);
      free_dev_csr(L.GP);
    }
  }
  if (std::getenv("HEATFLOW_DEBUG")) {
    auto show = [](const char* nm, size_t l, const DevCsr& m) {
      if (m.nrow) std::fprintf(stderr, "[amg] level %zu %-2s %8d x %8d nnz %9lld (%.1f/row, max %d) %s rpc %d lanes %d %s%s\n", l, nm, m.nrow, m.ncol,
                               static_cast<long long>(m.nnz), static_cast<double>(m.nnz) / m.nrow, m.max_row, m.rpc ? "stream" : "vec", m.rpc, m.lanes,
                               m.valf ? "f32" : "f64", m.cid ? " c16" : "");
    };
    for (size_t l = 0; l < nl; ++l) {
      show("A", l, ctx->amg[l].A); show("P", l, ctx->amg[l].P); show("R", l, ctx->amg[l].R);
      show("Rt", l, ctx->amg[l].Rt); show("GP", l, ctx->amg[l].GP);
    }
  }
  HF_TRY(wire_levels(ctx));
  lap("+ operators on the device");
  ctx->coarse_n = 0;
  if (nl > 1 && coarse_n > 0 && coarse_n <= 4096) {
    const int nc = coarse_n;
    const int ld = (nc + 3) & ~3;
    HF_TRY(dev_alloc(ctx, &ctx->d_coarse_inv, static_cast<size_t>(nc) * ld));
    HF_TRY(dense_inverse(ctx, nc, Ac.ptr.data(), Ac.idx.data(), Ac.val.data(), ctx->d_coarse_inv));
    if (f32) {
      HF_TRY(dev_alloc(ctx, &ctx->d_coarse_inv_f, static_cast<size_t>(nc) * ld));
      hipLaunchKernelGGL(k_to_float, dim3(1024), dim3(256), 0, ctx->stream, static_cast<size_t>(nc) * ld, ctx->d_coarse_inv, ctx->d_coarse_inv_f);
      HF_HIP(hipGetLastError());
    }
    HF_HIP(hipStreamSynchronize(ctx->stream));
    ctx->coarse_ld = ld;
    ctx->coarse_n = nc;
  }
  lap("+ dense inverse");
  ctx->amg_opc = op_complexity;
  ctx->amg_fine_stale = false;
  ctx->amg_ready = true;
  ctx->amg_setup_s = std::chrono::duration<double>(std::chrono::steady_clock::now() - t0).count();
  return HF_OK;
}

int build_amg(hf_ctx* ctx) {
  const auto t0 = std::chrono::steady_clock::now();
  free_amg(ctx);
  amg::Csr A0;
  A0.nrow = A0.ncol = ctx->n;
  A0.ptr.assign(ctx->h_rowptr.begin(), ctx->h_rowptr.end());
  A0.idx.assign(ctx->h_colidx.begin(), ctx->h_colidx.end());
  A0.val.resize(ctx->nnz);
  HF_HIP(copy_sync(ctx, A0.val.data(), ctx->d_A, sizeof(double) * ctx->nnz, hipMemcpyDeviceToHost));
  amg::Hierarchy H;
  amg::Params prm;
  amg_params(ctx, prm);
  auto lap = [&](const char* what) {
    if (prm.verbose) std::fprintf(stderr, "[amg setup] %-28s %.3f s\n", what, std::chrono::duration<double>(std::chrono::steady_clock::now() - t0).count());
  };
  lap("operator downloaded");
  if (!amg::build(std::move(A0), prm, H)) return fail(ctx, HF_ERR_STATE, "AMG set-up failed (non-positive diagonal or singular coarse operator)");
  lap("+ host hierarchy");
  ctx->amg.resize(H.levels.size());
  HF_TRY(upload_host_levels(ctx, H, 0));
  return finish_amg(ctx, H.levels.back().A, H.coarse_n, H.op_complexity, t0);
}

inline bool short_chunks(const DevCsr& m) { return m.nchunks > 0 && m.nnz <= static_cast<int64_t>(m.nchunks) * (7 * TS / 2); }

template <int SM, typename VT>
void launch_stream_t(hf_ctx* c, const DevCsr& m, const VT* val, const double* x, double* y, double* part0, const double* bvec,
                     double* conv_part) {
  const int npart = c->P;
  static const int grid_cap = std::getenv("HEATFLOW_STREAM_GRID") ? std::atoi(std::getenv("HEATFLOW_STREAM_GRID")) : MAXP;
  int grid = std::min(m.nchunks, (SM == 0 && part0 == nullptr) ? std::max(grid_cap, 1) : npart);
  if (grid >= 64) grid &= ~7;
#define HF_STREAM_ARGS2 m.nrow, m.nchunks, m.rpc, m.ptr, m.idx, val, x, y, c->d_scal, part0, bvec, static_cast<const double*>(nullptr), \
                        static_cast<double*>(nullptr), static_cast<double*>(nullptr), conv_part, 0.0, npart, 0
  if (m.cid != nullptr && sizeof(VT) == 4 && short_chunks(m))
    hipLaunchKernelGGL((k_spmv<SM, true, VT, 4>), dim3(grid), dim3(TS), static_cast<size_t>(m.chunk_nnz + m.max_dict) * 8, c->stream,
                       HF_STREAM_ARGS2, ColComp{m.dptr, m.dict, m.cid, m.chunk_nnz, 0});
  else if (m.cid != nullptr)
    hipLaunchKernelGGL((k_spmv<SM, true, VT>), dim3(grid), dim3(TS), static_cast<size_t>(m.chunk_nnz + m.max_dict) * 8, c->stream,
                       HF_STREAM_ARGS2, ColComp{m.dptr, m.dict, m.cid, m.chunk_nnz, 0});
  else
    hipLaunchKernelGGL((k_spmv<SM, false, VT>), dim3(grid), dim3(TS), static_cast<size_t>(m.chunk_nnz) * 8, c->stream,
                       HF_STREAM_ARGS2, ColComp{nullptr, nullptr, nullptr, 0, 0});
#undef HF_STREAM_ARGS2
}

template <int SM>
void launch_stream(hf_ctx* c, const DevCsr& m, const double* x, double* y, double* part0, const double* bvec, double* conv_part) {
  if (m.valf != nullptr) launch_stream_t<SM, float>(c, m, m.valf, x, y, part0, bvec, conv_part);
  else launch_stream_t<SM, double>(c, m, m.val, x, y, part0, bvec, conv_part);
}

template <int VMODE, typename VT>
void launch_vec_t(hf_ctx* c, const DevCsr& m, const VT* val, const double* x, double* y) {
  if (m.rpc > 0) {
    constexpr int SM = VMODE == 0 ? 0 : 6;
    static const int grid_cap = std::getenv("HEATFLOW_STREAM_GRID") ? std::atoi(std::getenv("HEATFLOW_STREAM_GRID")) : MAXP;
    int grid = std::min(m.nchunks, std::max(grid_cap, 1));
    if (grid >= 64) grid &= ~7;
#define HF_STREAM_ARGS m.nrow, m.nchunks, m.rpc, m.ptr, m.idx, val, x, y, c->d_scal, static_cast<double*>(nullptr),                       \
                       static_cast<const double*>(nullptr), static_cast<const double*>(nullptr), static_cast<double*>(nullptr),   \
                       static_cast<double*>(nullptr), static_cast<double*>(nullptr), 0.0, 0, 0
    if (m.cid != nullptr && sizeof(VT) == 4 && short_chunks(m))
      hipLaunchKernelGGL((k_spmv<SM, true, VT, 4>), dim3(grid), dim3(TS), static_cast<size_t>(m.chunk_nnz + m.max_dict) * 8, c->stream,
                         HF_STREAM_ARGS, ColComp{m.dptr, m.dict, m.cid, m.chunk_nnz, 0});
    else if (m.cid != nullptr)
      hipLaunchKernelGGL((k_spmv<SM, true, VT>), dim3(grid), dim3(TS), static_cast<size_t>(m.chunk_nnz + m.max_dict) * 8, c->stream,
                         HF_STREAM_ARGS, ColComp{m.dptr, m.dict, m.cid, m.chunk_nnz, 0});
    else
      hipLaunchKernelGGL((k_spmv<SM, false, VT>), dim3(grid), dim3(TS), static_cast<size_t>(m.chunk_nnz) * 8, c->stream,
                         HF_STREAM_ARGS, ColComp{nullptr, nullptr, nullptr, 0, 0});
#undef HF_STREAM_ARGS
    return;
  }
  if (m.lanes > 64) {
    hipLaunchKernelGGL((k_spmv_row<VMODE, VT>), dim3(std::max(1, std::min(m.nrow, 4096))), dim3(TPB), 0, c->stream, m.nrow, m.ptr,
                       m.idx, val, x, y, c->d_scal);
    return;
  }
  const int lanes = m.lanes;
  const long long threads = static_cast<long long>(m.nrow) * lanes;
  const int grid = static_cast<int>(std::max(1LL, std::min<long long>((threads + TPB - 1) / TPB, 2048)));
#define HF_VEC(L) hipLaunchKernelGGL((k_spmv_vec<L, VMODE, VT>), dim3(grid), dim3(TPB), 0, c->stream, m.nrow, m.ptr, m.idx, val, x, y, c->d_scal)
  switch (lanes) {
    case 4: HF_VEC(4); break;
    case 8: HF_VEC(8); break;
    case 16: HF_VEC(16); break;
    case 32: HF_VEC(32); break;
    default: HF_VEC(64); break;
  }
#undef HF_VEC
}

template <int VMODE>
void launch_vec(hf_ctx* c, const DevCsr& m, const double* x, double* y) {
  if (m.valf != nullptr) launch_vec_t<VMODE, float>(c, m, m.valf, x, y);
  else launch_vec_t<VMODE, double>(c, m, m.val, x, y);
}

enum CyclePart { CYCLE_ALL = 0, CYCLE_FIRST = 1, CYCLE_REST = 2 };
void vcycle(hf_ctx* c, int out_slot, bool test_convergence = false, CyclePart part = CYCLE_ALL) {
  const int nl = static_cast<int>(c->amg.size());
  DevLevel& L0 = c->amg[0];
  if (nl == 1) {
    if (part != CYCLE_REST)
      launch_spmv<4>(c, c->d_A, c->d_z, c->d_z2, c->d_part_rz + out_slot * MAXP, c->d_r, nullptr, nullptr, nullptr, L0.omega);
    return;
  }
  const bool fused0 = L0.GP.nrow > 0;
  if (L0.Rt.nrow > 0 && (fused0 || !c->amg_fine_stale)) {
    if (part != CYCLE_REST) launch_stream<0>(c, L0.Rt, c->d_r, c->amg[1].b, nullptr, nullptr, test_convergence ? c->d_part_zz : nullptr);
  } else {
    if (part != CYCLE_REST)
      launch_spmv<3>(c, c->d_A, c->d_z, c->d_tmp, nullptr, c->d_r, nullptr, nullptr,
                     test_convergence ? c->d_part_zz : nullptr);
    if (part != CYCLE_FIRST) launch_vec<0>(c, L0.R, c->d_tmp, c->amg[1].b);
  }
  if (part == CYCLE_FIRST) return;
  for (int l = 1; l + 1 < nl; ++l) launch_vec<0>(c, c->amg[l].Rt, c->amg[l].b, c->amg[l + 1].b);
  {
    DevLevel& Lc = c->amg[nl - 1];
    if (c->coarse_n > 0) {
      const int g = std::max(1, std::min((Lc.n + 1) / 2, 2048));
      if (c->d_coarse_inv_f != nullptr)
        hipLaunchKernelGGL(k_dense_mv_f32, dim3(g), dim3(TPB), 0, c->stream, Lc.n, c->coarse_ld, c->d_coarse_inv_f, Lc.b, Lc.res, c->d_scal);
      else
        hipLaunchKernelGGL(k_dense_mv, dim3(g), dim3(TPB), 0, c->stream, Lc.n, c->coarse_ld, c->d_coarse_inv, Lc.b, Lc.res, c->d_scal);
    } else {
      const int g = std::max(1, std::min((Lc.n + TPB - 1) / TPB, 1024));
      hipLaunchKernelGGL(k_scale, dim3(g), dim3(TPB), 0, c->stream, Lc.n, Lc.omega, Lc.dinv, Lc.b, Lc.res, c->d_scal);
    }
  }
  for (int l = nl - 2; l >= 1; --l) launch_vec<0>(c, c->amg[l].GP, c->amg[l].cat, c->amg[l].res);
  if (fused0) {
    launch_stream<7>(c, L0.GP, c->d_r, c->d_z2, c->d_part_rz + out_slot * MAXP, c->d_r, nullptr);
    return;
  }
  launch_vec<1>(c, L0.P, c->amg[1].res, c->d_z);
  launch_spmv<4>(c, c->d_A, c->d_z, c->d_z2, c->d_part_rz + out_slot * MAXP, c->d_r, nullptr, nullptr, nullptr, L0.omega);
}

void launch_amg_iteration(hf_ctx* c, double* x, int parity, CyclePart part = CYCLE_ALL) {
  if (part == CYCLE_REST) { vcycle(c, parity ^ 1, true, CYCLE_REST); return; }
  const bool timed = c->prof && c->prof_used < PROF_PAIRS;
  hipEvent_t e0 = timed ? c->prof_ev[2 * c->prof_used] : nullptr, e1 = timed ? c->prof_ev[2 * c->prof_used + 1] : nullptr;
  launch_spmv<9>(c, c->d_A, c->d_z2, c->d_Ap, c->d_part_pAp, nullptr, c->d_p, c->d_part_rz, c->d_part_zz, 0.0, nullptr, e0,
                 e1, parity);
  if (timed) c->prof_used++;
  hipLaunchKernelGGL(k_pcg_update_amg, dim3(c->P), dim3(TPB), 0, c->stream, c->n, c->nchunks, c->P, parity, c->d_scal,
                     c->d_part_pAp, c->d_part_rz, c->d_part_zz, x, c->d_r, c->d_p, c->d_Ap, c->d_dinv,
                     c->amg[0].omega, c->amg[0].GP.nrow > 0 ? static_cast<double*>(nullptr) : c->d_z);
  vcycle(c, parity ^ 1, true, part);
}

inline bool poll_enabled() {
  static const bool on = !(std::getenv("HEATFLOW_POLL") && std::getenv("HEATFLOW_POLL")[0] == '0');
  return on;
}

int reset_scal(hf_ctx* ctx) {
  *ctx->h_scal = Scal{};
  ctx->h_scal->mirror = ctx->d_mirror;
  HF_HIP(hipMemcpyAsync(ctx->d_scal, ctx->h_scal, sizeof(Scal), hipMemcpyHostToDevice, ctx->stream));
  HF_HIP(hipStreamSynchronize(ctx->stream));
  return HF_OK;
}

void harvest_profile(hf_ctx* ctx);

int read_scal(hf_ctx* ctx) {
  HF_HIP(hipMemcpyAsync(ctx->h_scal, ctx->d_scal, sizeof(Scal), hipMemcpyDeviceToHost, ctx->stream));
  HF_HIP(hipStreamSynchronize(ctx->stream));
  harvest_profile(ctx);
  return HF_OK;
}

int wait_tested(hf_ctx* ctx, int k) {
  static const double limit_s = std::getenv("HEATFLOW_POLL_TIMEOUT_S") ? std::atof(std::getenv("HEATFLOW_POLL_TIMEOUT_S")) : 60.0;
  ScalMirror* m = ctx->h_mirror;
  const unsigned ep = ctx->epoch;
  const auto t0 = std::chrono::steady_clock::now();
  auto last_query = t0;
  for (unsigned spin = 1;; ++spin) {
    const int tested = mirror_tested(m, ep);
    const int done = mirror_done(m, ep);
    if (tested >= k || done != 0) break;
    cpu_relax();
    if ((spin & 0x3ff) == 0) {
      const auto now = std::chrono::steady_clock::now();
      if (now - last_query < std::chrono::milliseconds(2)) continue;
      last_query = now;
      if (hipStreamQuery(ctx->stream) == hipSuccess) {
        if (mirror_tested(m, ep) >= k || mirror_done(m, ep) != 0) break;
        return fail(ctx, HF_ERR_HIP, "PCG progress: stream drained before the test of iteration %d ran (%s)", k, hipGetErrorString(hipGetLastError()));
      }
      if (std::chrono::duration<double>(std::chrono::steady_clock::now() - t0).count() > limit_s)
        return fail(ctx, HF_ERR_HIP, "PCG progress: no convergence test within %.0f s (waiting for iteration %d, at %d)", limit_s, k, tested);
    }
  }
  __atomic_thread_fence(__ATOMIC_ACQUIRE);
  ctx->h_scal->iters = m->iters;
  ctx->h_scal->zz = m->zz;
  ctx->h_scal->bn2 = m->bn2;
  ctx->h_scal->done = mirror_done(m, ep);
  return HF_OK;
}

void harvest_profile(hf_ctx* ctx) {
  if (ctx->prof) {
    for (int k = 0; k < ctx->prof_used; ++k) {
      float ms = 0.f;
      const bool ran = !ctx->h_scal->done || (ctx->prof_base + k) < ctx->h_scal->iters;
      if (ran && hipEventElapsedTime(&ms, ctx->prof_ev[2 * k], ctx->prof_ev[2 * k + 1]) == hipSuccess) {
        ctx->prof_spmv_ms += ms;
        ctx->prof_spmv_n += 1;
      }
    }
    ctx->prof_used = 0;
  }
}

int pcg_solve(hf_ctx* ctx, const LinSys& sys, bool use_amg, double rtol, double atol, int max_it, int* pred) {
  static const bool trace_res = std::getenv("HEATFLOW_TRACE_RES") != nullptr;
  ctx->epoch += 1;
  if (!use_amg) {
    launch_spmv<2>(ctx, sys.A, sys.x, ctx->d_r, ctx->d_part_rz, sys.b, ctx->d_z, ctx->d_part_zz, ctx->d_part_bn, 0.0,
                   sys.dinv);
    hipLaunchKernelGGL(k_pcg_begin, dim3(1), dim3(TPB), 0, ctx->stream, ctx->P, rtol, atol, ctx->d_part_zz,
                       ctx->d_part_bn, ctx->d_scal, ctx->epoch);
  } else {
    launch_spmv<5>(ctx, sys.A, sys.x, ctx->d_r, nullptr, sys.b, ctx->d_z, ctx->d_part_zz, ctx->d_part_bn,
                   ctx->amg[0].omega);
    hipLaunchKernelGGL(k_pcg_begin, dim3(1), dim3(TPB), 0, ctx->stream, ctx->P, rtol, atol, ctx->d_part_zz,
                       ctx->d_part_bn, ctx->d_scal, ctx->epoch);
    vcycle(ctx, 0);
  }
  HF_HIP(hipGetLastError());

  int launched = 0;
  if (use_amg && !trace_res && ctx->amg.size() > 1 && poll_enabled()) {
    ctx->prof_base = 0;
    auto finish = [&](int rc) {
      if (ctx->prof) { (void)hipStreamSynchronize(ctx->stream); harvest_profile(ctx); }
      return rc;
    };
    if (*pred <= 0) {
      HF_TRY(wait_tested(ctx, 0));
      if (ctx->h_scal->done == 1) return finish(HF_OK);
    }
    static const bool hold_back = !(std::getenv("HEATFLOW_HOLD_BACK") && std::getenv("HEATFLOW_HOLD_BACK")[0] == '0');
    int burst = std::max(1, std::min(max_it, *pred - 2));
    bool rest_pending = false;
    while (true) {
      if (rest_pending) launch_amg_iteration(ctx, sys.x, (launched - 1) & 1, CYCLE_REST);
      const bool split = hold_back && burst == 1 && launched > 0;
      for (int k = 0; k < burst; ++k) launch_amg_iteration(ctx, sys.x, (launched + k) & 1, split ? CYCLE_FIRST : CYCLE_ALL);
      rest_pending = split;
      launched += burst;
      HF_HIP(hipGetLastError());
      const int rc = wait_tested(ctx, launched);
      if (rc != HF_OK) return finish(rc);
      if (ctx->h_scal->done || launched >= max_it) break;
      burst = 1;
    }
    *pred = ctx->h_scal->iters;
    if (ctx->h_scal->done == 2) return finish(fail(ctx, HF_ERR_NOCONV, "PCG breakdown (p.Ap <= 0) after %d iterations", ctx->h_scal->iters));
    if (!ctx->h_scal->done)
      return finish(fail(ctx, HF_ERR_NOCONV, "PCG not converged in %d iterations (rel. residual %.3e)", ctx->h_scal->iters,
                         std::sqrt(ctx->h_scal->zz / std::max(ctx->h_scal->bn2, 1e-300))));
    return finish(HF_OK);
  }
  if (*pred <= 0) {
    HF_TRY(read_scal(ctx));
    if (ctx->h_scal->done == 1) return HF_OK;
  }
  int burst = std::max(1, std::min(max_it, *pred > 0 ? *pred : (use_amg ? 8 : 32)));
  if (trace_res) burst = 2;
  while (true) {
    ctx->prof_base = launched;
    for (int k = 0; k < burst; ++k) {
      if (use_amg) launch_amg_iteration(ctx, sys.x, (launched + k) & 1);
      else launch_pcg_iteration(ctx, sys, (launched + k) & 1);
    }
    launched += burst;
    HF_HIP(hipGetLastError());
    HF_TRY(read_scal(ctx));
    if (trace_res) std::fprintf(stderr, "[res] it %d rel %.3e\n", ctx->h_scal->iters, std::sqrt(ctx->h_scal->zz / std::max(ctx->h_scal->bn2, 1e-300)));
    if (ctx->h_scal->done) break;
    if (launched >= max_it) break;
    burst = std::max(1, std::min(std::max(use_amg ? 1 : 8, launched / 8), max_it - launched));
    if (trace_res) burst = 2;
  }
  *pred = ctx->h_scal->iters;
  if (ctx->h_scal->done == 2) return fail(ctx, HF_ERR_NOCONV, "PCG breakdown (p.Ap <= 0) after %d iterations", ctx->h_scal->iters);
  if (!ctx->h_scal->done)
    return fail(ctx, HF_ERR_NOCONV, "PCG not converged in %d iterations (rel. residual %.3e)", ctx->h_scal->iters,
                std::sqrt(ctx->h_scal->zz / std::max(ctx->h_scal->bn2, 1e-300)));
  return HF_OK;
}

void proj_clear(hf_ctx* ctx, bool ring_only = false) {
// ... 379 lines not shown
```

### heatflow_amd/hip_backend.py

```python
from __future__ import annotations

import ctypes as C
import os
import subprocess

import numpy as np

_HERE = os.path.dirname(os.path.abspath(__file__))
LIB_PATH = os.environ.get("HEATFLOW_HIP_LIB") or os.path.join(_HERE, "csrc", "libheatflow_hip.so")

HF_OK, HF_ERR_ARG, HF_ERR_STATE, HF_ERR_HIP, HF_ERR_NOCONV, HF_ERR_ALLOC = 0, -1, -2, -3, -4, -5
ASM_LDS_ATOMIC, ASM_LDS_COLORED, ASM_GLOBAL_ATOMIC, ASM_ROW_GATHER = 0, 1, 2, 3
PC_JACOBI, PC_AMG = 0, 1
K_SPMV, K_PCG_SPMV, K_PCG_UPDATE, K_PCG_DIR, K_ASSEMBLE, K_RHS, K_STREAM_READ = range(7)
BATCH_SHARED, BATCH_PER_COLUMN, BATCH_AFFINE = 0, 1, 2
TIME_BACKWARD_EULER, TIME_BDF2 = 0, 1
TIME_SCHEMES = {"backward_euler": TIME_BACKWARD_EULER, "bdf2": TIME_BDF2}


def time_scheme_code(name):
    if name not in TIME_SCHEMES:
        raise ValueError(f"unknown time scheme {name!r} (expected one of {sorted(TIME_SCHEMES)})")
    return TIME_SCHEMES[name]

EXPORTS = [
    "hf_version", "hf_create", "hf_destroy", "hf_last_error", "hf_set_mesh", "hf_set_mesh_prebuilt", "hf_pattern_export_size",
    "hf_pattern_export", "hf_amg_export_size", "hf_amg_export", "hf_amg_install", "hf_set_materials",
    "hf_update_kappa", "hf_set_dirichlet", "hf_assemble", "hf_set_time_scheme", "hf_set_precond", "hf_set_start_vector", "hf_get_response_solves", "hf_get_amg_info", "hf_get_amg_fallbacks", "hf_set_state", "hf_get_state", "hf_sample", "hf_step", "hf_run",
    "hf_batch_begin", "hf_batch_load_column", "hf_batch_set_affine", "hf_batch_set_state", "hf_batch_get_state", "hf_batch_run", "hf_batch_run_flux", "hf_batch_end",
    "hf_flux_setup", "hf_flux_project", "hf_flux_solve", "hf_flux_sample",
    "hf_steady_setup", "hf_steady_solve", "hf_steady_picard_setup", "hf_steady_picard_solve", "hf_set_load", "hf_get_load", "hf_hold_load",
    "hf_set_source", "hf_get_source", "hf_set_source_amplitudes",
    "hf_tangent_setup", "hf_tangent_setup_dir", "hf_tangent_set_shape", "hf_tangent_load", "hf_run_tangent", "hf_get_tangent", "hf_set_kappa_tables", "hf_get_picard_change", "hf_set_rhoc_tables", "hf_set_picard", "hf_set_anisotropy", "hf_get_sizes", "hf_get_csr", "hf_spmv",
    "hf_set_value_lists", "hf_get_value_lists", "hf_get_projection",
    "hf_amg_apply", "hf_batch_apply_precond", "hf_dense_inverse", "hf_time_kernel", "hf_set_profile", "hf_get_profile", "hf_last_gpu_ms",
]


class HipUnavailable(RuntimeError):
    """libheatflow_hip.so is not built or no HIP device is usable."""


class HipError(RuntimeError):
    def __init__(self, code, msg):
        super().__init__(f"heatflow_hip error {code}: {msg}")
        self.code = code


class NotConverged(HipError):
    pass


def build_library(force=False, verbose=False):
    src = os.path.join(_HERE, "csrc", "heatflow_hip.hip")
    hdr = os.path.join(_HERE, "..", "include", "heatflow_hip.h")
    if not force and os.path.isfile(LIB_PATH):
        csrc = os.path.join(_HERE, "csrc")
        newest = max([os.path.getmtime(src), os.path.getmtime(hdr)] +
                     [os.path.getmtime(os.path.join(csrc, f)) for f in os.listdir(csrc) if f.endswith(".hpp")])
        if os.path.getmtime(LIB_PATH) >= newest:
            return LIB_PATH
    cmd = ["make", "-C", os.path.join(_HERE, "csrc"), "libheatflow_hip.so"]
    if force:
        cmd.insert(1, "-B")
    res = subprocess.run(cmd, capture_output=True, text=True)
    if verbose or res.returncode != 0:
        print(res.stdout, res.stderr)
    if res.returncode != 0:
        raise RuntimeError("building libheatflow_hip.so failed:\n" + res.stderr)
    return LIB_PATH


_lib = None


def load_library():
    global _lib
    if _lib is not None:
        return _lib
    if not os.path.isfile(LIB_PATH):
        raise HipUnavailable(f"{LIB_PATH} not found - run `python -c 'import __graft_entry__ as g; g.build()'` "
                             "or `make -C heatflow_amd/csrc`")
    lib = C.CDLL(LIB_PATH)
    vp, i32, i64, dbl = C.c_void_p, C.c_int32, C.c_int64, C.c_double
    pd, pi = C.POINTER(C.c_double), C.POINTER(C.c_int32)
    lib.hf_version.restype = C.c_char_p
    lib.hf_last_error.restype = C.c_char_p
    lib.hf_last_error.argtypes = [vp]
    protos = {
        "hf_create": [C.c_int, C.POINTER(vp)],
        "hf_destroy": [vp],
        "hf_set_mesh": [vp, i32, i32, pd, pi, pi],
        "hf_set_mesh_prebuilt": [vp, i32, i32, pd, pi, pi, vp, i64],
        "hf_pattern_export_size": [vp, C.POINTER(i64)],
        "hf_pattern_export": [vp, vp, i64],
        "hf_amg_export_size": [vp, C.POINTER(i64)],
        "hf_amg_export": [vp, vp, i64],
        "hf_amg_install": [vp, vp, i64],
        "hf_set_materials": [vp, i32, pi, pd, pd],
        "hf_update_kappa": [vp, i32, pi, pd],
        "hf_set_dirichlet": [vp, i32, pi],
        "hf_assemble": [vp, dbl, i32],
        "hf_set_time_scheme": [vp, i32],
        "hf_set_precond": [vp, i32, i32],
        "hf_set_start_vector": [vp, i32],
        "hf_get_response_solves": [vp, C.POINTER(i64)],
        "hf_get_amg_info": [vp, pi, pi, i32, pd, pd],
        "hf_get_amg_fallbacks": [vp, C.POINTER(i64)],
        "hf_set_state": [vp, pd],
        "hf_get_state": [vp, pd],
        "hf_sample": [vp, i32, pi, pd],
        "hf_step": [vp, pd, dbl, dbl, i32, pi, pd],
        "hf_run": [vp, i32, pd, dbl, dbl, i32, i32, pi, pd, pi],
        "hf_batch_begin": [vp, i32, i32],
        "hf_batch_load_column": [vp, i32],
        "hf_batch_set_affine": [vp, i32, pi, pd],
        "hf_batch_set_state": [vp, i32, pd],
        "hf_batch_get_state": [vp, i32, pd],
        "hf_batch_run": [vp, i32, pd, dbl, dbl, i32, i32, pi, pd, pi],
        "hf_batch_run_flux": [vp, i32, pd, dbl, dbl, i32, i32, pi, pd, pi, i32, dbl, i32, i32, pi, pd, pi],
        "hf_batch_end": [vp],
        "hf_flux_setup": [vp],
        "hf_flux_project": [vp, dbl, i32, pd, pd, pi],
        "hf_flux_solve": [vp, i32, dbl, i32, pi],
        "hf_flux_sample": [vp, i32, pi, pd, pd],
        "hf_steady_setup": [vp, i32, pi, i32],
        "hf_steady_solve": [vp, pd, i32, dbl, dbl, i32, pi, pd],
        "hf_steady_picard_setup": [vp, i32, pi, i32],
        "hf_steady_picard_solve": [vp, pd, i32, dbl, dbl, i32, dbl, i32, pi, pi, pd, pd],
        "hf_set_load": [vp, pd],
        "hf_get_load": [vp, pd],
        "hf_hold_load": [vp],
        "hf_set_source": [vp, i32, pi, dbl, dbl, dbl],
        "hf_get_source": [vp, pd],
        "hf_set_source_amplitudes": [vp, i32, pd],
        "hf_tangent_setup": [vp, i32, pi],
        "hf_tangent_setup_dir": [vp, i32, pi, pi, pi],
        "hf_tangent_set_shape": [vp, i32, pd],
        "hf_tangent_load": [vp, i32, pd],
        "hf_run_tangent": [vp, i32, pd, pd, dbl, dbl, i32, i32, pi, pd, pi, pd, pi],
        "hf_get_tangent": [vp, i32, pd],
        "hf_set_kappa_tables": [vp, i32, pi, pd, pd, pi, pd, i32],
        "hf_get_picard_change": [vp, pd],
        "hf_set_rhoc_tables": [vp, i32, pi, pd, pd, pi, pd],
        "hf_set_picard": [vp, i32],
        "hf_set_anisotropy": [vp, i32, pi, pd, pd],
        "hf_get_sizes": [vp, pi, pi, C.POINTER(i64), pi],
        "hf_get_csr": [vp, pi, pi, pd, pd],
        "hf_spmv": [vp, i32, pd, pd],
        "hf_set_value_lists": [vp, i32],
        "hf_get_value_lists": [vp, i32, pi, C.POINTER(i64), pi, pi, pi, pd, C.POINTER(C.c_uint32)],
        "hf_get_projection": [vp, i32, pi, pi, pi, pi, pi, pd, pd, pd, pd],
        "hf_amg_apply": [vp, pd, pd, pd],
        "hf_batch_apply_precond": [vp, pd, pd, pd],
        "hf_dense_inverse": [vp, i32, pi, pi, pd, pd, pd, pd, pd],
        "hf_time_kernel": [vp, i32, i32, pd],
        "hf_last_gpu_ms": [vp, pd],
        "hf_set_profile": [vp, i32],
        "hf_get_profile": [vp, pd, C.POINTER(i64)],
    }
    for name, args in protos.items():
        fn = getattr(lib, name)
        fn.argtypes = args
        fn.restype = C.c_int
    _lib = lib
    return lib


def projection_sizes():
    mh, mt = C.c_int32(), C.c_int32()
    rc = load_library().hf_get_projection(None, -1, C.byref(mh), C.byref(mt), None, None, None, None, None, None, None)
    if rc != HF_OK:
        raise HipError(rc, "hf_get_projection: size query failed")
    return mh.value, mt.value


def blob_address(blob):
    if isinstance(blob, tuple):
        return int(blob[0]), int(blob[1]), blob
    if hasattr(blob, "address") and hasattr(blob, "nbytes") and not isinstance(blob, np.ndarray):
        return int(blob.address), int(blob.nbytes), blob
    arr = np.ascontiguousarray(blob, dtype=np.uint8)
    return arr.ctypes.data, arr.nbytes, arr


def _pd(a):
    return a.ctypes.data_as(C.POINTER(C.c_double)) if a is not None else None


def _pi(a):
    return a.ctypes.data_as(C.POINTER(C.c_int32)) if a is not None else None


def _f64(a):
    return np.ascontiguousarray(a, dtype=np.float64)


def _i32(a):
    return np.ascontiguousarray(a, dtype=np.int32)


class HeatflowHIP:

    def __init__(self, device_id=0):
        self._lib = load_library()
        self._ctx = C.c_void_p()
        rc = self._lib.hf_create(int(device_id), C.byref(self._ctx))
        if rc != HF_OK:
            msg = self._lib.hf_last_error(self._ctx).decode() if self._ctx else "no usable HIP device"
            if self._ctx:
                self._lib.hf_destroy(self._ctx)
                self._ctx = C.c_void_p()
            raise HipUnavailable(f"hf_create(device {device_id}) failed ({rc}): {msg}")
        self.n = self.n_e = self.n_bc = 0
        self.nnz = 0
        self.batch_nv = 0

    def close(self):
        if getattr(self, "_ctx", None):
            self._lib.hf_destroy(self._ctx)
            self._ctx = C.c_void_p()

    def __del__(self):
        try:
            self.close()
        except Exception:
            pass

    def __enter__(self):
        return self

    def __exit__(self, *exc):
        self.close()

    def _check(self, rc):
        if rc == HF_OK:
            return
        msg = self._lib.hf_last_error(self._ctx).decode()
        if rc == HF_ERR_NOCONV:
            raise NotConverged(rc, msg)
        if rc == HF_ERR_ARG:
            raise ValueError(f"heatflow_hip: {msg}")
        raise HipError(rc, msg)

    def set_mesh(self, coords, tris, tags, pattern=None):
        zr, tri, tag = _f64(coords), _i32(tris), _i32(tags)
        if zr.ndim != 2 or zr.shape[1] != 2 or tri.ndim != 2 or tri.shape[1] != 3 or tag.shape != (tri.shape[0],):
            raise ValueError("set_mesh: coords (n,2), tris (n_e,3), tags (n_e,) expected")
        self.tab_len = int(tag.max()) + 1 if tag.size else 0
        self.tangent_nv = 0
        if pattern is None:
            self._check(self._lib.hf_set_mesh(self._ctx, zr.shape[0], tri.shape[0], _pd(zr), _pi(tri), _pi(tag)))
        else:
            addr, nbytes, _keep = blob_address(pattern)
            self._check(self._lib.hf_set_mesh_prebuilt(self._ctx, zr.shape[0], tri.shape[0], _pd(zr), _pi(tri), _pi(tag),
                                                       C.c_void_p(addr), nbytes))
        self._refresh_sizes()

    def pattern_bytes(self):
        nb = C.c_int64()
        self._check(self._lib.hf_pattern_export_size(self._ctx, C.byref(nb)))
        return int(nb.value)

    def export_pattern(self, into=None):
        nb = self.pattern_bytes()
        if into is not None:
            if int(into[1]) != nb:
                raise ValueError(f"export_pattern: buffer of {into[1]} bytes, need {nb}")
            self._check(self._lib.hf_pattern_export(self._ctx, C.c_void_p(int(into[0])), nb))
            return None
        blob = np.empty(nb, dtype=np.uint8)
        self._check(self._lib.hf_pattern_export(self._ctx, C.c_void_p(blob.ctypes.data), nb))
        return blob

    def amg_export(self, into=None):
        nb = C.c_int64()
        self._check(self._lib.hf_amg_export_size(self._ctx, C.byref(nb)))
        if into is not None:
            if int(into[1]) != nb.value:
                raise ValueError(f"amg_export: buffer of {into[1]} bytes, need {nb.value}")
            self._check(self._lib.hf_amg_export(self._ctx, C.c_void_p(int(into[0])), nb.value))
            return None
        blob = np.empty(nb.value, dtype=np.uint8)
        self._check(self._lib.hf_amg_export(self._ctx, C.c_void_p(blob.ctypes.data), nb.value))
        return blob

    def amg_install(self, blob):
        addr, nbytes, _keep = blob_address(blob)
        self._check(self._lib.hf_amg_install(self._ctx, C.c_void_p(addr), nbytes))

    def _refresh_sizes(self):
        n, ne, nbc, nnz = C.c_int32(), C.c_int32(), C.c_int32(), C.c_int64()
        self._check(self._lib.hf_get_sizes(self._ctx, C.byref(n), C.byref(ne), C.byref(nnz), C.byref(nbc)))
        self.n, self.n_e, self.nnz, self.n_bc = n.value, ne.value, nnz.value, nbc.value

    def set_materials(self, tags, kappa, rho_c):
        t, k, c = _i32(tags), _f64(kappa), _f64(rho_c)
        if not (t.shape == k.shape == c.shape) or t.ndim != 1:
            raise ValueError("set_materials: three 1-D arrays of equal length expected")
        self._check(self._lib.hf_set_materials(self._ctx, len(t), _pi(t), _pd(k), _pd(c)))

    def update_kappa(self, tags, kappa):
        t, k = _i32(tags), _f64(kappa)
        self._check(self._lib.hf_update_kappa(self._ctx, len(t), _pi(t), _pd(k)))

    def set_dirichlet(self, dofs):
        d = _i32(dofs)
        self._check(self._lib.hf_set_dirichlet(self._ctx, len(d), _pi(d) if len(d) else None))
        self._refresh_sizes()

    def set_precond(self, kind=PC_JACOBI, reuse=False):
        self._check(self._lib.hf_set_precond(self._ctx, int(kind), 1 if reuse else 0))

    def set_time_scheme(self, scheme=TIME_BACKWARD_EULER):
        code = time_scheme_code(scheme) if isinstance(scheme, str) else int(scheme)
        self._check(self._lib.hf_set_time_scheme(self._ctx, code))

    def set_start_vector(self, kind=3):
        self._check(self._lib.hf_set_start_vector(self._ctx, int(kind)))

    def response_solves(self):
        c = C.c_int64()
        self._check(self._lib.hf_get_response_solves(self._ctx, C.byref(c)))
        return int(c.value)

    def amg_info(self):
        nl, opc, secs = C.c_int32(), C.c_double(), C.c_double()
        rows = np.zeros(16, dtype=np.int32)
        self._check(self._lib.hf_get_amg_info(self._ctx, C.byref(nl), _pi(rows), 16, C.byref(opc), C.byref(secs)))
        fb = C.c_int64()
        self._check(self._lib.hf_get_amg_fallbacks(self._ctx, C.byref(fb)))
        return {"levels": nl.value, "rows": rows[:nl.value].tolist(), "op_complexity": opc.value, "setup_s": secs.value,
                "jacobi_fallbacks": fb.value}

    def assemble(self, dt, mode=ASM_LDS_ATOMIC):
        self._check(self._lib.hf_assemble(self._ctx, float(dt), int(mode)))

    def set_state(self, u):
        u = _f64(u)
        if u.shape != (self.n,):
            raise ValueError(f"set_state: expected {self.n} values")
        self._check(self._lib.hf_set_state(self._ctx, _pd(u)))

    def get_state(self):
        u = np.empty(self.n, dtype=np.float64)
        self._check(self._lib.hf_get_state(self._ctx, _pd(u)))
        return u

    def sample(self, nodes):
        idx = _i32(nodes)
        out = np.empty(len(idx), dtype=np.float64)
        self._check(self._lib.hf_sample(self._ctx, len(idx), _pi(idx), _pd(out)))
        return out

    def step(self, g_bc, rtol=1e-10, atol=0.0, max_it=20000):
        g = _f64(g_bc)
        if g.shape != (self.n_bc,):
            raise ValueError(f"step: expected {self.n_bc} boundary values")
        it, res = C.c_int32(), C.c_double()
        rc = self._lib.hf_step(self._ctx, _pd(g) if self.n_bc else None, rtol, atol, int(max_it), C.byref(it), C.byref(res))
        self.last_iters, self.last_resid = it.value, res.value
        self._check(rc)
        return it.value, res.value

    def run(self, g_all, rtol=1e-10, atol=0.0, max_it=20000, nodes=None):
        g = _f64(g_all)
        if g.ndim != 2 or g.shape[1] != self.n_bc:
            raise ValueError(f"run: g_all must be (n_steps, {self.n_bc})")
        nsteps = g.shape[0]
        idx = _i32(nodes) if nodes is not None and len(nodes) else None
        ns = 0 if idx is None else len(idx)
        samples = np.empty((nsteps, ns), dtype=np.float64)
        iters = np.zeros(nsteps, dtype=np.int32)
        rc = self._lib.hf_run(self._ctx, nsteps, _pd(g) if self.n_bc else None, rtol, atol, int(max_it), ns, _pi(idx),
                              _pd(samples) if ns else None, _pi(iters))
        self.last_run_iters = iters
        self._check(rc)
        return samples, iters

    def tangent_setup(self, n_par, tag_col):
        tab = np.full(self.tab_len, -1, dtype=np.int32)
        for t, j in dict(tag_col).items():
            if not 0 <= int(t) < self.tab_len:
                raise ValueError(f"tangent_setup: tag {t} is not a cell tag of the mesh")
            tab[int(t)] = int(j)
        self.tangent_nv = 0
        self._check(self._lib.hf_tangent_setup(self._ctx, int(n_par), _pi(tab)))
        self.tangent_nv = next(v for v in (2, 4, 8, 16) if v >= int(n_par))

    def tangent_setup_dir(self, n_par, k=None, r=None, z=None):
        tabs = []
        for name, m in (("k", k), ("r", r), ("z", z)):
            if not m:
                tabs.append(None)
                continue
            tab = np.full(self.tab_len, -1, dtype=np.int32)
            for t, j in dict(m).items():
                if not 0 <= int(t) < self.tab_len:
                    raise ValueError(f"tangent_setup_dir: tag {t} ({name}) is not a cell tag of the mesh")
                tab[int(t)] = int(j)
            tabs.append(tab)
        self.tangent_nv = 0
        self._check(self._lib.hf_tangent_setup_dir(self._ctx, int(n_par), *(None if t is None else _pi(t) for t in tabs)))
        self.tangent_nv = next(v for v in (2, 4, 8, 16) if v >= int(n_par))

    def tangent_set_shape(self, j, vz):
        if vz is None:
            self._check(self._lib.hf_tangent_set_shape(self._ctx, int(j), None))
            return
        v = np.ascontiguousarray(vz, dtype=np.float64).reshape(-1)
        if v.size != self.n:
            raise ValueError(f"tangent_set_shape: {v.size} velocities for {self.n} nodes")
        self._check(self._lib.hf_tangent_set_shape(self._ctx, int(j), _pd(v)))

    def tangent_load(self, j):
        F = np.empty(self.n, dtype=np.float64)
        self._check(self._lib.hf_tangent_load(self._ctx, int(j), _pd(F)))
        return F

    def run_tangent(self, g_all, h_all=None, rtol=1e-10, atol=0.0, max_it=20000, nodes=None):
        g = _f64(g_all)
        if g.ndim != 2 or g.shape[1] != self.n_bc:
            raise ValueError(f"run_tangent: g_all must be (n_steps, {self.n_bc})")
        nsteps, nv = g.shape[0], self.tangent_nv or 2
        h = None
        if h_all is not None:
            h = _f64(h_all)
            if h.shape != (nsteps, self.n_bc, nv):
                raise ValueError(f"run_tangent: h_all must be ({nsteps}, {self.n_bc}, {nv})")
        idx = _i32(nodes) if nodes is not None and len(nodes) else None
        ns = 0 if idx is None else len(idx)
        samples = np.empty((nsteps, ns), dtype=np.float64)
        tsamples = np.empty((nsteps, nv, ns), dtype=np.float64)
        iters = np.zeros(nsteps, dtype=np.int32)
        titers = np.zeros((nsteps, nv), dtype=np.int32)
        rc = self._lib.hf_run_tangent(self._ctx, nsteps, _pd(g) if self.n_bc else None, _pd(h) if (h is not None and self.n_bc) else None,
                                      rtol, atol, int(max_it), ns, _pi(idx), _pd(samples) if ns else None, _pi(iters),
                                      _pd(tsamples) if ns else None, _pi(titers))
        self.last_run_iters = iters
        self._check(rc)
        return samples, iters, tsamples, titers

    def get_tangent(self, j):
        s = np.empty(self.n, dtype=np.float64)
        self._check(self._lib.hf_get_tangent(self._ctx, int(j), _pd(s)))
        return s

    def set_kappa_tables(self, tables, picard=1):
        items = sorted((int(t), v) for t, v in (tables or {}).items())
        if not items:
            self._check(self._lib.hf_set_kappa_tables(self._ctx, 0, None, None, None, None, None, int(picard)))
            return
        tags = _i32([t for t, _ in items])
        t0 = _f64([float(v[0]) for _, v in items])
        dT = _f64([float(v[1]) for _, v in items])
        vals = [np.asarray(v[2], dtype=np.float64).ravel() for _, v in items]
        nk = _i32([len(v) for v in vals])
        allv = _f64(np.concatenate(vals))
        self._check(self._lib.hf_set_kappa_tables(self._ctx, len(tags), _pi(tags), _pd(t0), _pd(dT), _pi(nk), _pd(allv),
                                                  int(picard)))

    def set_rhoc_tables(self, tables):
        items = sorted((int(t), v) for t, v in (tables or {}).items())
        if not items:
            self._check(self._lib.hf_set_rhoc_tables(self._ctx, 0, None, None, None, None, None))
            return
        tags = _i32([t for t, _ in items])
        t0 = _f64([float(v[0]) for _, v in items])
        dT = _f64([float(v[1]) for _, v in items])
        vals = [np.asarray(v[2], dtype=np.float64).ravel() for _, v in items]
        nk = _i32([len(v) for v in vals])
        allv = _f64(np.concatenate(vals))
        self._check(self._lib.hf_set_rhoc_tables(self._ctx, len(tags), _pi(tags), _pd(t0), _pd(dT), _pi(nk), _pd(allv)))

    def set_anisotropy(self, multipliers):
        items = sorted((int(t), v) for t, v in (multipliers or {}).items())
        if not items:
            self._check(self._lib.hf_set_anisotropy(self._ctx, 0, None, None, None))
            return
        for t, v in items:
            if len(tuple(v)) != 2:
                raise ValueError(f"set_anisotropy: tag {t} needs a pair (m_r, m_z)")
        tags = _i32([t for t, _ in items])
        m_r = _f64([float(v[0]) for _, v in items])
        m_z = _f64([float(v[1]) for _, v in items])
        self._check(self._lib.hf_set_anisotropy(self._ctx, len(tags), _pi(tags), _pd(m_z), _pd(m_r)))

# ... 258 lines not shown
```

### include/heatflow_hip.h

```cpp
#ifndef HEATFLOW_HIP_H
#define HEATFLOW_HIP_H

#include <stdint.h>

#ifdef __cplusplus
extern "C" {
#endif

typedef struct hf_ctx hf_ctx;

enum {
  HF_OK = 0,
  HF_ERR_ARG = -1,
  HF_ERR_STATE = -2,
  HF_ERR_HIP = -3,
  HF_ERR_NOCONV = -4,
  HF_ERR_ALLOC = -5
};

enum { HF_ASM_LDS_ATOMIC = 0, HF_ASM_LDS_COLORED = 1, HF_ASM_GLOBAL_ATOMIC = 2, HF_ASM_ROW_GATHER = 3 };

enum {
  HF_K_SPMV = 0,
  HF_K_PCG_SPMV = 1,
  HF_K_PCG_UPDATE = 2,
  HF_K_PCG_DIR = 3,
  HF_K_ASSEMBLE = 4,
  HF_K_RHS = 5,
  HF_K_STREAM_READ = 6
};

const char* hf_version(void);

int hf_create(int device_id, hf_ctx** out);
int hf_destroy(hf_ctx* ctx);
const char* hf_last_error(const hf_ctx* ctx);

int hf_set_mesh(hf_ctx* ctx, int32_t n, int32_t n_e, const double* zr, const int32_t* tri, const int32_t* tag);

int hf_pattern_export_size(hf_ctx* ctx, int64_t* bytes);
int hf_pattern_export(hf_ctx* ctx, void* blob, int64_t bytes);
int hf_set_mesh_prebuilt(hf_ctx* ctx, int32_t n, int32_t n_e, const double* zr, const int32_t* tri, const int32_t* tag,
                         const void* blob, int64_t bytes);

int hf_set_materials(hf_ctx* ctx, int32_t n_mat, const int32_t* tags, const double* kappa, const double* rho_c);

int hf_update_kappa(hf_ctx* ctx, int32_t n_mat, const int32_t* tags, const double* kappa);

int hf_set_anisotropy(hf_ctx* ctx, int32_t n, const int32_t* tags, const double* m_z, const double* m_r);

int hf_set_dirichlet(hf_ctx* ctx, int32_t n_bc, const int32_t* dofs);

int hf_assemble(hf_ctx* ctx, double dt, int32_t mode);

enum { HF_TIME_BACKWARD_EULER = 0, HF_TIME_BDF2 = 1 };
int hf_set_time_scheme(hf_ctx* ctx, int32_t scheme);

int hf_set_precond(hf_ctx* ctx, int32_t kind, int32_t reuse);
int hf_get_amg_info(hf_ctx* ctx, int32_t* n_levels, int32_t* level_rows, int32_t max_levels, double* op_complexity,
                    double* setup_seconds);

int hf_amg_export_size(hf_ctx* ctx, int64_t* bytes);
int hf_amg_export(hf_ctx* ctx, void* blob, int64_t bytes);
int hf_amg_install(hf_ctx* ctx, const void* blob, int64_t bytes);

int hf_set_start_vector(hf_ctx* ctx, int32_t kind);
int hf_get_response_solves(hf_ctx* ctx, int64_t* count);

int hf_get_amg_fallbacks(hf_ctx* ctx, int64_t* count);

int hf_set_state(hf_ctx* ctx, const double* u);
int hf_get_state(hf_ctx* ctx, double* u);
int hf_sample(hf_ctx* ctx, int32_t n_s, const int32_t* nodes, double* out);

int hf_step(hf_ctx* ctx, const double* g_bc, double rtol, double atol, int32_t max_it, int32_t* iters, double* resid);

int hf_run(hf_ctx* ctx, int32_t n_steps, const double* g_bc_all, double rtol, double atol, int32_t max_it,
           int32_t n_s, const int32_t* nodes, double* samples, int32_t* iters);

enum { HF_BATCH_SHARED = 0, HF_BATCH_PER_COLUMN = 1, HF_BATCH_AFFINE = 2 };
int hf_batch_begin(hf_ctx* ctx, int32_t nv, int32_t operator_kind);
int hf_batch_load_column(hf_ctx* ctx, int32_t j);
int hf_batch_set_affine(hf_ctx* ctx, int32_t n_tags, const int32_t* tags, const double* delta );
int hf_batch_set_state(hf_ctx* ctx, int32_t j, const double* u);
int hf_batch_get_state(hf_ctx* ctx, int32_t j, double* u);
int hf_batch_run(hf_ctx* ctx, int32_t n_steps, const double* g_bc_all, double rtol, double atol, int32_t max_it,
                 int32_t n_s, const int32_t* nodes, double* samples, int32_t* iters);
int hf_batch_run_flux(hf_ctx* ctx, int32_t n_steps, const double* g_bc_all, double rtol, double atol, int32_t max_it,
                      int32_t n_s, const int32_t* nodes, double* samples, int32_t* iters, int32_t flux_components,
                      double flux_rtol, int32_t flux_max_it, int32_t n_fs, const int32_t* flux_nodes, double* flux_samples,
                      int32_t* flux_iters);
int hf_batch_end(hf_ctx* ctx);

int hf_flux_setup(hf_ctx* ctx);
int hf_flux_project(hf_ctx* ctx, double rtol, int32_t max_it, double* grad_z, double* grad_r, int32_t* iters);
int hf_flux_solve(hf_ctx* ctx, int32_t components, double rtol, int32_t max_it, int32_t* iters);
int hf_flux_sample(hf_ctx* ctx, int32_t n_s, const int32_t* nodes, double* grad_z, double* grad_r);

int hf_steady_setup(hf_ctx* ctx, int32_t n_s, const int32_t* dofs_s, int32_t precond);
int hf_steady_solve(hf_ctx* ctx, const double* g_s, int32_t use_load, double rtol, double atol, int32_t max_it, int32_t* iters,
                    double* resid);

int hf_steady_picard_setup(hf_ctx* ctx, int32_t n_s, const int32_t* dofs_s, int32_t precond);
int hf_steady_picard_solve(hf_ctx* ctx, const double* g_s, int32_t use_load, double rtol, double atol, int32_t max_it,
                           double picard_tol, int32_t max_sweeps, int32_t* sweeps, int32_t* iters, double* change, double* nl_resid);
int hf_set_load(hf_ctx* ctx, const double* F);
int hf_hold_load(hf_ctx* ctx);
int hf_get_load(hf_ctx* ctx, double* F);

int hf_set_source(hf_ctx* ctx, int32_t n_tags, const int32_t* tags, double fwhm, double z0, double depth);
int hf_get_source(hf_ctx* ctx, double* F);
int hf_set_source_amplitudes(hf_ctx* ctx, int32_t n_amp, const double* p);

int hf_tangent_setup(hf_ctx* ctx, int32_t n_par, const int32_t* tag_col);
int hf_tangent_set_shape(hf_ctx* ctx, int32_t j, const double* vz);
int hf_tangent_setup_dir(hf_ctx* ctx, int32_t n_par, const int32_t* tag_col_k, const int32_t* tag_col_r, const int32_t* tag_col_z);
int hf_tangent_load(hf_ctx* ctx, int32_t j, double* F);
int hf_run_tangent(hf_ctx* ctx, int32_t n_steps, const double* g_all, const double* h_all, double rtol, double atol, int32_t max_it,
                   int32_t n_s, const int32_t* nodes, double* samples, int32_t* iters, double* tangent_samples, int32_t* tangent_iters);
int hf_get_tangent(hf_ctx* ctx, int32_t j, double* s);

int hf_set_kappa_tables(hf_ctx* ctx, int32_t n_tab, const int32_t* tags, const double* t0, const double* dT, const int32_t* n_knots,
                        const double* values, int32_t picard_sweeps);
int hf_get_picard_change(hf_ctx* ctx, double* max_du);

int hf_set_rhoc_tables(hf_ctx* ctx, int32_t n_tab, const int32_t* tags, const double* t0, const double* dT, const int32_t* n_knots,
                       const double* values);
int hf_set_picard(hf_ctx* ctx, int32_t sweeps);

int hf_get_sizes(hf_ctx* ctx, int32_t* n, int32_t* n_e, int64_t* nnz, int32_t* n_bc);
int hf_get_csr(hf_ctx* ctx, int32_t* rowptr, int32_t* colidx, double* A, double* M);
int hf_spmv(hf_ctx* ctx, int32_t which, const double* x, double* y);

int hf_set_value_lists(hf_ctx* ctx, int32_t mode);
int hf_get_value_lists(hf_ctx* ctx, int32_t which, int32_t* valid, int64_t* sum_vlist, int32_t* max_vlist, int32_t* vcap, int32_t* vptr,
                       double* vlist, uint32_t* cv);

int hf_amg_apply(hf_ctx* ctx, const double* r, double* z, double* rz);
int hf_batch_apply_precond(hf_ctx* ctx, const double* r, double* z, double* rz);
int hf_dense_inverse(hf_ctx* ctx, int32_t n, const int32_t* ptr, const int32_t* idx, const double* val, const double* b,
                     double* inv, double* x64, double* x32);

int hf_get_projection(hf_ctx* ctx, int32_t column, int32_t* mh, int32_t* mt, int32_t* used, int32_t* next, int32_t* pending, double* G,
                      double* alpha, double* V, double* F);

int hf_time_kernel(hf_ctx* ctx, int32_t which, int32_t reps, double* ms_avg);
int hf_set_profile(hf_ctx* ctx, int32_t on);
int hf_get_profile(hf_ctx* ctx, double* spmv_ms_sum, int64_t* spmv_launches);
int hf_last_gpu_ms(hf_ctx* ctx, double* ms);

#ifdef __cplusplus
}
#endif
#endif
```

Before: 794.3 million.

## Restructure SpMV kernel to take explicit workgroup ids and fuse multigrid restriction recurrence

Reworks the fused SpMV/CG kernel so its chunk scheduling and partial-sum writes use explicit workgroup indices (HF_WG/HF_NWG) through a new ChunkIter constructor and a wide partial-sum helper. This appears to let several logical workgroups share one launch or block, and adds a restrict_recurrence path with per-level residency state to fold the multigrid restriction into the iteration. It also exposes debug and query entry points. The intent is to cut launch and synchronisation overhead in the AMG-preconditioned solve, at the cost of more complex kernel indexing and a risk of correctness slips in the reduction bookkeeping.

After: 779.5 million. -1.9%, worse.

```diff
diff --git a/heatflow_amd/csrc/heatflow_hip.hip b/heatflow_amd/csrc/heatflow_hip.hip
--- a/heatflow_amd/csrc/heatflow_hip.hip
+++ b/heatflow_amd/csrc/heatflow_hip.hip
@@ -1094,6 +1094,22 @@
     for (int l = 0; l < nl && l < max_levels; ++l) level_rows[l] = ctx->amg[l].n;
   if (op_complexity) *op_complexity = ctx->amg_ready ? ctx->amg_opc : 0.0;
   if (setup_seconds) *setup_seconds = ctx->amg_ready ? ctx->amg_setup_s : 0.0;
+  return HF_OK;
+}
+
+int hf_get_iteration_form(hf_ctx* ctx, int32_t* form) {
+  if (!ctx || !form) return HF_ERR_ARG;
+  *form = (ctx->amg_ready && ctx->precond == 1 && restrict_recurrence(ctx)) ? 1 : 0;
+  return HF_OK;
+}
+
+int hf_debug_level_rhs(hf_ctx* ctx, int32_t level, double* out, int64_t n) {
+  if (!ctx || !out) return HF_ERR_ARG;
+  if (!ctx->amg_ready || level < 1 || level >= static_cast<int32_t>(ctx->amg.size()))
+    return fail(ctx, HF_ERR_ARG, "hf_debug_level_rhs: no level %d in the hierarchy", static_cast<int>(level));
+  if (n != ctx->amg[level].n) return fail(ctx, HF_ERR_ARG, "hf_debug_level_rhs: level %d has %d rows", static_cast<int>(level), ctx->amg[level].n);
+  HF_HIP(hipSetDevice(ctx->dev));
+  HF_HIP(copy_sync(ctx, out, ctx->amg[level].b, sizeof(double) * static_cast<size_t>(n), hipMemcpyDeviceToHost));
   return HF_OK;
 }
 
diff --git a/heatflow_amd/csrc/hf_context.hpp b/heatflow_amd/csrc/hf_context.hpp
--- a/heatflow_amd/csrc/hf_context.hpp
+++ b/heatflow_amd/csrc/hf_context.hpp
@@ -207,6 +207,7 @@
   struct DevLevel {
     DevCsr A, P, R, Rt, GP;
     double *dinv = nullptr, *x = nullptr, *cat = nullptr, *b = nullptr, *res = nullptr;
+    int ur_resident = 0;
     bool own_b = false;
     double omega = 0; int n = 0;
   };
diff --git a/heatflow_amd/csrc/hf_kernels.hpp b/heatflow_amd/csrc/hf_kernels.hpp
--- a/heatflow_amd/csrc/hf_kernels.hpp
+++ b/heatflow_amd/csrc/hf_kernels.hpp
@@ -23,6 +23,13 @@
 __device__ __forceinline__ double sum_partials(const double* __restrict__ part, int P, double* s4) {
   double v = 0.0;
   for (int k = threadIdx.x; k < P; k += TPB) v += part[k];
+  return block_sum(v, s4);
+}
+template <int NT>
+__device__ __forceinline__ double sum_partials_wide(const double* __restrict__ part, int P, double* s4) {
+  double v = 0.0;
+  if (threadIdx.x < TPB)
+    for (int k = threadIdx.x; k < P; k += TPB) v += part[k];
   return block_sum(v, s4);
 }
 
@@ -41,6 +48,19 @@
     } else {
       chunk = blockIdx.x;
       step = gridDim.x;
+      end = nchunks;
+    }
+  }
+  __device__ __forceinline__ ChunkIter(int nchunks, unsigned wg, unsigned nwg) {
+    if (HF_XCD_MAP && (nwg & 7) == 0) {
+      const int per = (nchunks + 7) >> 3;
+      const int xcd = wg & 7;
+      chunk = xcd * per + (wg >> 3);
+      step = nwg >> 3;
+      end = min(nchunks, (xcd + 1) * per);
+    } else {
+      chunk = wg;
+      step = nwg;
       end = nchunks;
     }
   }
@@ -1124,387 +1144,29 @@
                                               double* __restrict__ part1, double* __restrict__ part2, double w,
                                               int npart ,
                                               int parity, typename std::conditional<VC, ValComp, ColComp>::type comp) {
-  extern __shared__ double sprod[];
-  __shared__ double s4[TS / 64];
-  __shared__ int s_own;
-  constexpr bool BDF = MODE >= 12 && MODE <= 15;
-  auto opnd = [&](int c) { return BDF ? bdf2_operand(x[c], bvec[c]) : x[c]; };
-  if ((MODE == 3 || MODE == 4 || MODE == 6 || MODE == 9) && scal->done) return;
-  if ((MODE == 0 || MODE == 7) && scal != nullptr && scal->done) return;
-  double acc0 = 0.0, acc1 = 0.0, acc2 = 0.0;
-  double beta = 0.0;
-  bool first9 = false;
-  if (MODE == 9) {
-    first9 = scal->first != 0;
-    if (!first9) {
-      double v0 = 0.0, v1 = 0.0, v2 = 0.0;
-      for (int k = threadIdx.x; k < npart; k += TS) {
-        v0 += part1[parity * MAXP + k];
-        v1 += part1[(parity ^ 1) * MAXP + k];
-        v2 += part2[k];
-      }
-      const double rz_new = block_sum<TS / 64>(v0, s4);
-      const double rz_old = block_sum<TS / 64>(v1, s4);
-      const double zz = block_sum<TS / 64>(v2, s4);
-      const bool conv = zz <= scal->tol2;
-      if (blockIdx.x == 0 && threadIdx.x == 0) {
-        scal->zz = zz;
-        if (conv) scal->done = 1;
-      }
-      if (conv) return;
-      beta = rz_new / rz_old;
-    }
-  }
-  auto cycle_gate = [&]() {
-    if (!((MODE == 3 || MODE == 0) && part2 != nullptr)) return false;
-    double v2 = 0.0;
-    for (int k = threadIdx.x; k < npart; k += TS) v2 += part2[k];
-    const double zz = block_sum<TS / 64>(v2, s4);
-    const bool conv = zz <= scal->tol2;
-    if (blockIdx.x == 0 && threadIdx.x == 0) {
-      if (conv) { scal->zz = zz; scal->done = 1; }
-      mirror_publish(scal->mirror, zz, scal->iters, conv ? 1 : 0, scal->epoch);
-    }
-    return conv;
-  };
-  constexpr bool PIPELINED = C16 && !VC && (HF_PIPE == 2 || (HF_PIPE == 1 && sizeof(VT) == 4));
-  static_assert(!VC || (C16 && sizeof(VT) == 8), "value lists: the fine operator's f64 arrays on compressed columns");
-  if (!PIPELINED && cycle_gate()) return;
-  const ChunkIter sched(nchunks);
-  HF_STAMP(0);
-  int stamp_at = 1;
-  (void)stamp_at;
-  const int tpr = (MODE == 0 || MODE == 6 || MODE == 7) ? TS / rpc : 1;
-  const int prel = static_cast<int>(threadIdx.x) / tpr;
-  const int psub = static_cast<int>(threadIdx.x) % tpr;
-  struct RowOps { double b, d, y, p, x; };
-  auto row_operands = [&](int prc, bool from_slice) {
-    RowOps e{0.0, 0.0, 0.0, 0.0, 0.0};
-    if (MODE == 2 || MODE == 3 || MODE == 4 || MODE == 5 || MODE == 7 || MODE == 8 || MODE == 11 || MODE == 13 || MODE == 15) e.b = bvec[prc];
-    if (MODE == 2 || MODE == 4 || MODE == 5 || MODE == 10 || MODE == 11 || MODE == 14 || MODE == 15) e.d = dinv[prc];
-    if (MODE == 6 || (MODE == 9 && !first9)) e.y = y[prc];
-    if (MODE == 9 && !first9) e.p = pvec[prc];
-    if ((MODE == 4 || MODE == 8 || MODE == 9 || MODE == 11) && !from_slice) e.x = x[prc];
-    if (BDF) e.x = x[prc];
-    return e;
-  };
-  auto rows_phase = [&](bool pin, int prow, int pa, int pb, const RowOps& e) {
-    if ((MODE == 0 || MODE == 6 || MODE == 7) && tpr > 1) {
-      double s = 0.0;
-      if (pin)
-        for (int j = pa + psub; j < pb; j += tpr) s += sprod[j];
-      for (int o = tpr >> 1; o > 0; o >>= 1) s += __shfl_down(s, o, 64);
-      if (pin && psub == 0) {
-        y[prow] = (MODE == 6) ? e.y + s : s;
-        if (MODE == 7) acc0 += e.b * s;
-      }
-    } else if (pin) {
-      const int row = prow;
-      double s = 0.0;
-      for (int j = pa; j < pb; ++j) s += sprod[j];
-      if (MODE == 0) {
-        y[row] = s;
-      } else if (MODE == 2) {
-        const double ri = e.b - s;
-        const double zi = e.d * ri;
-        y[row] = ri;
-        pvec[row] = zi;
-        acc0 += ri * zi;
-        acc1 += zi * zi;
-        acc2 += (e.d * e.b) * (e.d * e.b);
-      } else if (MODE == 3) {
-        y[row] = e.b - s;
-      } else if (MODE == 4) {
-        const double yi = e.x + w * e.d * (e.b - s);
-        y[row] = yi;
-        acc0 += e.b * yi;
-      } else if (MODE == 5) {
-        const double ri = e.b - s;
-        y[row] = ri;
-        pvec[row] = w * e.d * ri;
-        acc1 += (e.d * ri) * (e.d * ri);
-        acc2 += (e.d * e.b) * (e.d * e.b);
-      } else if (MODE == 7) {
-        y[row] = s;
-        acc0 += e.b * s;
-      } else if (MODE == 6) {
-        y[row] = e.y + s;
-      } else if (MODE == 8) {
-        y[row] = s;
-        pvec[row] = 2.0 * e.x - e.b;
-      } else if (MODE == 10) {
-        y[row] = s + w * e.d;
-      } else if (MODE == 11) {
-        y[row] = s + w * e.d;
-        pvec[row] = 2.0 * e.x - e.b;
-      } else if (BDF) {
-        y[row] = (MODE == 14 || MODE == 15) ? s + w * e.d : s;
-        pvec[row] = (MODE == 13 || MODE == 15) ? 2.0 * e.x - e.b : e.x;
-      } else {
-        const double api = first9 ? s : s + beta * e.y;
-        const double pi = first9 ? e.x : e.x + beta * e.p;
-        y[row] = api;
-        pvec[row] = pi;
-        acc0 += pi * api;
-      }
-    }
-  };
-  if (PIPELINED) {
-    struct Bounds { int k0, k1, d0, d1; };
-    auto bounds = [&](int ch) {
-      Bounds q;
-      const int a0 = ch * rpc, a1 = min(n, a0 + rpc);
-      q.k0 = rowptr[a0]; q.k1 = rowptr[a1];
-      q.d0 = comp.dptr[ch]; q.d1 = comp.dptr[ch + 1];
-      return q;
-    };
-    int lhead[HF_STAGE_U];
-    double v[UN];
-    int id[UN];
-    auto heads = [&](const Bounds& q, bool live) {
-      const int dl = max(q.d1 - 1, 0), kl = max(q.k1 - 1, 0);
-      const int t = static_cast<int>(threadIdx.x);
-#pragma unroll
-      for (int u = 0; u < HF_STAGE_U; ++u) lhead[u] = comp.dict[min(q.d0 + (live ? t + u * TS : (t & 31)), dl)];
-      __builtin_amdgcn_sched_barrier(0);
-#pragma unroll
-      for (int u = 0; u < UN; ++u) {
-        const int kk = min(q.k0 + (live ? t + u * TS : (t & 31)), kl);
-        v[u] = static_cast<double>(stream_load(&vals[kk]));
-        id[u] = static_cast<int>(stream_load(&comp.id[kk]));
-      }
-    };
-    double* xd = sprod + comp.xd_off;
-    Bounds cur = bounds(min(sched.chunk, nchunks - 1));
-    heads(cur, sched.chunk < sched.end);
-    if (cycle_gate()) return;
-    for (int chunk = sched.chunk; chunk < sched.end; chunk += sched.step) {
-      const bool more = chunk + sched.step < sched.end;
-      const int r0 = chunk * rpc, r1 = min(n, r0 + rpc);
-      const int k0 = cur.k0, k1 = cur.k1, d0 = cur.d0, nd = cur.d1 - cur.d0;
-      const int prow = r0 + prel;
-      const bool pin = prow < r1;
-      const int prc = min(prow, r1 - 1);
-      int c0[HF_STAGE_U];
-      double x0[HF_STAGE_U];
-#pragma unroll
-      for (int u = 0; u < HF_STAGE_U; ++u) { c0[u] = lhead[u]; x0[u] = opnd(c0[u]); }
-      const Bounds nxt = bounds(more ? chunk + sched.step : chunk);
-      const int pa = rowptr[prc] - k0, pb = rowptr[prc + 1] - k0;
-      RowOps e = row_operands(prc, comp.own != 0);
-#pragma unroll
-      for (int u = 0; u < HF_STAGE_U; ++u) {
-        const int i = static_cast<int>(threadIdx.x) + u * TS;
-        if (i < nd) {
-          xd[i] = x0[u];
-          if ((MODE == 4 || MODE == 8 || MODE == 9 || MODE == 11) && c0[u] == r0) s_own = i;
-        }
-      }
-      for (int i = threadIdx.x + HF_STAGE_U * TS; i < nd; i += HF_STAGE_U * TS) {
-        int c[HF_STAGE_U];
-        double xv[HF_STAGE_U];
-#pragma unroll
-        for (int u = 0; u < HF_STAGE_U; ++u) c[u] = comp.dict[d0 + min(i + u * TS, nd - 1)];
-#pragma unroll
-        for (int u = 0; u < HF_STAGE_U; ++u) xv[u] = opnd(c[u]);
-#pragma unroll
-        for (int u = 0; u < HF_STAGE_U; ++u)
-          if (i + u * TS < nd) {
-            xd[i + u * TS] = xv[u];
-            if ((MODE == 4 || MODE == 8 || MODE == 9 || MODE == 11) && c[u] == r0) s_own = i + u * TS;
-          }
-      }
-      __syncthreads();
-      HF_STAMP(stamp_at); ++stamp_at;
-      if ((MODE == 4 || MODE == 8 || MODE == 9 || MODE == 11) && comp.own && pin) e.x = xd[s_own + (prow - r0)];
-#pragma unroll
-      for (int u = 0; u < UN; ++u) {
-        const int kk = k0 + static_cast<int>(threadIdx.x) + u * TS;
-        if (kk < k1) sprod[kk - k0] = v[u] * xd[id[u]];
-      }
-      for (int kb = k0 + UN * TS; kb < k1; kb += UN * TS) {
-#pragma unroll
-        for (int u = 0; u < UN; ++u) {
-          const int kk = min(kb + static_cast<int>(threadIdx.x) + u * TS, k1 - 1);
-          v[u] = static_cast<double>(stream_load(&vals[kk]));
-          id[u] = static_cast<int>(stream_load(&comp.id[kk]));
-        }
-#pragma unroll
-        for (int u = 0; u < UN; ++u) {
-          const int kk = kb + static_cast<int>(threadIdx.x) + u * TS;
-          if (kk < k1) sprod[kk - k0] = v[u] * xd[id[u]];
-        }
-      }
-      heads(nxt, more);
-      __syncthreads();
-      HF_STAMP(stamp_at); ++stamp_at;
-      rows_phase(pin, prow, pa, pb, e);
-      __syncthreads();
-      HF_STAMP(stamp_at); ++stamp_at;
-      cur = nxt;
-    }
-  } else {
-  const ChunkIter& sched_ = sched;
-  for (int chunk = sched_.chunk; chunk < sched_.end; chunk += sched_.step) {
-    const int r0 = chunk * rpc;
-    const int r1 = min(n, r0 + rpc);
-    const int k0 = rowptr[r0];
-    const int k1 = rowptr[r1];
-    const int prow = r0 + prel;
-    const bool pin = prow < r1;
-    int pa = 0, pb = 0;
-    if (pin) {
-      pa = rowptr[prow] - k0;
-      pb = rowptr[prow + 1] - k0;
-    }
-    RowOps e = row_operands(min(prow, r1 - 1), C16 && comp.own != 0);
-    if constexpr (VC) {
-      double* xd = sprod + comp.xd_off;
-      double* vl = sprod + comp.vl_off;
-      const int d0 = comp.dptr[chunk], nd = comp.dptr[chunk + 1] - d0;
-      const int v0 = comp.vptr[chunk], nv = comp.vptr[chunk + 1] - v0;
-      const bool vin = nv <= comp.vcap;
-      int k = k0 + threadIdx.x;
-      std::uint32_t cw[HF_UNROLL];
-#pragma unroll
-      for (int u = 0; u < HF_UNROLL; ++u) cw[u] = (k + u * TS < k1) ? stream_load(&comp.cv[k + u * TS]) : 0u;
-      double lv[2];
-#pragma unroll
-      for (int u = 0; u < 2; ++u) {
-        const int i = static_cast<int>(threadIdx.x) + u * TS;
-        lv[u] = (vin && i < nv) ? comp.vlist[v0 + i] : 0.0;
-      }
-      for (int i = threadIdx.x; i < nd; i += HF_STAGE_U * TS) {
-        int c[HF_STAGE_U];
-        double xv[HF_STAGE_U];
-#pragma unroll
-        for (int u = 0; u < HF_STAGE_U; ++u) c[u] = (i + u * TS < nd) ? comp.dict[d0 + i + u * TS] : 0;
-#pragma unroll
-        for (int u = 0; u < HF_STAGE_U; ++u) xv[u] = (i + u * TS < nd) ? opnd(c[u]) : 0.0;
-#pragma unroll
-        for (int u = 0; u < HF_STAGE_U; ++u)
-          if (i + u * TS < nd) {
-            xd[i + u * TS] = xv[u];
-            if ((MODE == 4 || MODE == 8 || MODE == 9 || MODE == 11) && c[u] == r0) s_own = i + u * TS;
-          }
-      }
-#pragma unroll
-      for (int u = 0; u < 2; ++u) {
-        const int i = static_cast<int>(threadIdx.x) + u * TS;
-        if (vin && i < nv) vl[i] = lv[u];
-      }
-      if (vin)
-        for (int i = threadIdx.x + 2 * TS; i < nv; i += TS) vl[i] = comp.vlist[v0 + i];
-      __syncthreads();
-      HF_STAMP(stamp_at); ++stamp_at;
-      if ((MODE == 4 || MODE == 8 || MODE == 9 || MODE == 11) && comp.own && pin) e.x = xd[s_own + (prow - r0)];
-      while (k < k1) {
-        const int kn = k + HF_UNROLL * TS;
-        std::uint32_t cn[HF_UNROLL];
-#pragma unroll
-        for (int u = 0; u < HF_UNROLL; ++u) cn[u] = (kn + u * TS < k1) ? stream_load(&comp.cv[kn + u * TS]) : 0u;
-        if (vin) {
-#pragma unroll
-          for (int u = 0; u < HF_UNROLL; ++u)
-            if (k + u * TS < k1) sprod[k - k0 + u * TS] = vl[cw[u] >> 16] * xd[cw[u] & 0xffffu];
-        } else {
-          double gv[HF_UNROLL];
-#pragma unroll
-          for (int u = 0; u < HF_UNROLL; ++u) gv[u] = (k + u * TS < k1) ? comp.vlist[v0 + static_cast<int>(cw[u] >> 16)] : 0.0;
-#pragma unroll
-          for (int u = 0; u < HF_UNROLL; ++u)
-            if (k + u * TS < k1) sprod[k - k0 + u * TS] = gv[u] * xd[cw[u] & 0xffffu];
-        }
-#pragma unroll
-        for (int u = 0; u < HF_UNROLL; ++u) cw[u] = cn[u];
-        k = kn;
-      }
-    } else if (C16) {
-      double* xd = sprod + comp.xd_off;
-      const int d0 = comp.dptr[chunk], nd = comp.dptr[chunk + 1] - d0;
-      int k = k0 + threadIdx.x;
-      double v[HF_UNROLL];
-      int id[HF_UNROLL];
-#pragma unroll
-      for (int u = 0; u < HF_UNROLL; ++u) {
-        const bool in = k + u * TS < k1;
-        v[u] = in ? static_cast<double>(stream_load(&vals[k + u * TS])) : 0.0;
-        id[u] = in ? static_cast<int>(stream_load(&comp.id[k + u * TS])) : 0;
-      }
-      for (int i = threadIdx.x; i < nd; i += HF_STAGE_U * TS) {
-        int c[HF_STAGE_U];
-        double xv[HF_STAGE_U];
-#pragma unroll
-        for (int u = 0; u < HF_STAGE_U; ++u) c[u] = (i + u * TS < nd) ? comp.dict[d0 + i + u * TS] : 0;
-#pragma unroll
-        for (int u = 0; u < HF_STAGE_U; ++u) xv[u] = (i + u * TS < nd) ? opnd(c[u]) : 0.0;
-#pragma unroll
-        for (int u = 0; u < HF_STAGE_U; ++u)
-          if (i + u * TS < nd) {
-            xd[i + u * TS] = xv[u];
-            if ((MODE == 4 || MODE == 8 || MODE == 9 || MODE == 11) && c[u] == r0) s_own = i + u * TS;
-          }
-      }
-      __syncthreads();
-      HF_STAMP(stamp_at); ++stamp_at;
-      if ((MODE == 4 || MODE == 8 || MODE == 9 || MODE == 11) && comp.own && pin) e.x = xd[s_own + (prow - r0)];
-      while (k < k1) {
-        const int kn = k + HF_UNROLL * TS;
-        double vn[HF_UNROLL];
-        int idn[HF_UNROLL];
-#pragma unroll
-        for (int u = 0; u < HF_UNROLL; ++u) {
-          const bool in = kn + u * TS < k1;
-          vn[u] = in ? static_cast<double>(stream_load(&vals[kn + u * TS])) : 0.0;
-          idn[u] = in ? static_cast<int>(stream_load(&comp.id[kn + u * TS])) : 0;
-        }
-#pragma unroll
-        for (int u = 0; u < HF_UNROLL; ++u)
-          if (k + u * TS < k1) sprod[k - k0 + u * TS] = v[u] * xd[id[u]];
-#pragma unroll
-        for (int u = 0; u < HF_UNROLL; ++u) { v[u] = vn[u]; id[u] = idn[u]; }
-        k = kn;
-      }
-    } else {
-      for (int k = k0 + threadIdx.x; k < k1; k += HF_UNROLL * TS) {
-        int c[HF_UNROLL];
-        double v[HF_UNROLL], xv[HF_UNROLL];
-#pragma unroll
-        for (int u = 0; u < HF_UNROLL; ++u) {
-          const bool in = k + u * TS < k1;
-          c[u] = in ? colidx[k + u * TS] : 0;
-          v[u] = in ? static_cast<double>(vals[k + u * TS]) : 0.0;
-        }
-#pragma unroll
-        for (int u = 0; u < HF_UNROLL; ++u) xv[u] = (k + u * TS < k1) ? opnd(c[u]) : 0.0;
-#pragma unroll
-        for (int u = 0; u < HF_UNROLL; ++u)
-          if (k + u * TS < k1) sprod[k - k0 + u * TS] = v[u] * xv[u];
-      }
-    }
-    __syncthreads();
-    HF_STAMP(stamp_at); ++stamp_at;
-    rows_phase(pin, prow, pa, pb, e);
-    __syncthreads();
-    HF_STAMP(stamp_at); ++stamp_at;
-  }
-  }
-  if (MODE == 2 || MODE == 7 || MODE == 9 || (MODE == 4 && part0 != nullptr)) {
-    const double t0 = block_sum<TS / 64>(acc0, s4);
-    if (threadIdx.x == 0) {
-      part0[blockIdx.x] = t0;
-      for (int q = blockIdx.x + gridDim.x; q < npart; q += gridDim.x) part0[q] = 0.0;
-    }
-  }
-  if (MODE == 2 || MODE == 5) {
-    const double t1 = block_sum<TS / 64>(acc1, s4);
-    const double t2 = block_sum<TS / 64>(acc2, s4);
-    if (threadIdx.x == 0) {
-      part1[blockIdx.x] = t1;
-      part2[blockIdx.x] = t2;
-      for (int q = blockIdx.x + gridDim.x; q < npart; q += gridDim.x) { part1[q] = 0.0; part2[q] = 0.0; }
-    }
-  }
+#define HF_WG blockIdx.x
+#define HF_NWG gridDim.x
+#define HF_SCHED nchunks
+#include "hf_spmv_body.inc"
+#undef HF_WG
+#undef HF_NWG
+#undef HF_SCHED
+}
+
+template <int MODE, bool C16, typename VT, int UN, bool VC>
+__device__ __forceinline__ void spmv_role(int n, int nchunks, int rpc, const int32_t* __restrict__ rowptr, const int32_t* __restrict__ colidx,
+                                          const VT* __restrict__ vals, const double* __restrict__ x, double* __restrict__ y,
+                                          Scal* __restrict__ scal, double* __restrict__ part0, const double* __restrict__ bvec,
+                                          const double* __restrict__ dinv, double* __restrict__ pvec, double* __restrict__ part1,
+                                          double* __restrict__ part2, double w, int npart, int parity,
+                                          typename std::conditional<VC, ValComp, ColComp>::type comp, const unsigned wg, const unsigned nwg) {
+#define HF_WG wg
+#define HF_NWG nwg
+#define HF_SCHED nchunks, wg, nwg
+#include "hf_spmv_body.inc"
+#undef HF_WG
+#undef HF_NWG
+#undef HF_SCHED
 }
 
 constexpr int VL_MAX_CHUNK = 4096;
@@ -1711,6 +1373,46 @@
     if (lane == 0) y[row] = (VMODE == 1) ? y0 + s : s;
   }
 }
+
+template <int LANES, typename VT = double>
+__global__ __launch_bounds__(TPB) void k_spmv_vec_gate(int nrow, const int32_t* __restrict__ ptr,
+                                                       const int32_t* __restrict__ idx, const VT* __restrict__ val,
+                                                       const double* __restrict__ x, double* __restrict__ y,
+                                                       Scal* __restrict__ scal, const double* __restrict__ part_zz, int npart) {
+  __shared__ double s4[TPB / 64];
+  if (scal->done) return;
+  const double zz = sum_partials(part_zz, npart, s4);
+  const bool conv = zz <= scal->tol2;
+  if (blockIdx.x == 0 && threadIdx.x == 0) {
+    if (conv) { scal->zz = zz; scal->done = 1; }
+    mirror_publish(scal->mirror, zz, scal->iters, conv ? 1 : 0, scal->epoch);
+  }
+  if (conv) return;
+  const int lane = threadIdx.x % LANES;
+  const int rows_per_pass = (gridDim.x * TPB) / LANES;
+  for (int row = (blockIdx.x * TPB + threadIdx.x) / LANES; row < nrow; row += rows_per_pass) {
+    const int k1 = ptr[row + 1];
+    double s = 0.0;
+    for (int k = ptr[row] + lane; k < k1; k += 4 * LANES) {
+      int c[4];
+      double v[4], xv[4];
+#pragma unroll
+      for (int u = 0; u < 4; ++u) {
+        const bool in = k + u * LANES < k1;
+        c[u] = in ? idx[k + u * LANES] : 0;
+        v[u] = in ? static_cast<double>(val[k + u * LANES]) : 0.0;
+      }
+#pragma unroll
+      for (int u = 0; u < 4; ++u) xv[u] = (k + u * LANES < k1) ? x[c[u]] : 0.0;
+#pragma unroll
+      for (int u = 0; u < 4; ++u) s += v[u] * xv[u];
+    }
+#pragma unroll
+    for (int o = LANES / 2; o > 0; o >>= 1) s += __shfl_down(s, o, LANES);
+    if (lane == 0) y[row] = s;
+  }
+}
+
 
 template <int VMODE, typename VT = double>
 __global__ __launch_bounds__(TPB) void k_spmv_row(int nrow, const int32_t* __restrict__ ptr,
@@ -2145,4 +1847,61 @@
   if (threadIdx.x == 0) part_zz[blockIdx.x] = t1;
 }
 
-}
+__device__ __forceinline__ void pcg_update_amg_role(int n, int nchunks, int P, int parity, Scal* __restrict__ scal,
+                                                    const double* __restrict__ part_pAp, const double* __restrict__ part_rz,
+                                                    double* __restrict__ part_zz, double* __restrict__ x, double* __restrict__ r,
+                                                    const double* __restrict__ p, const double* __restrict__ Ap,
+                                                    const double* __restrict__ dinv, double w, double* __restrict__ z0,
+                                                    const unsigned wg, const unsigned nwg) {
+  __shared__ double s4[TS / 64];
+  if (scal->done) return;
+  const double pAp = sum_partials_wide<TS>(part_pAp, P, s4);
+  const double rz = sum_partials_wide<TS>(part_rz + parity * MAXP, P, s4);
+  if (!(pAp > 0.0)) {
+    if (wg == 0 && threadIdx.x == 0) {
+      scal->done = 2;
+      mirror_breakdown(scal->mirror, scal->epoch);
+    }
+    return;
+  }
+  if (wg == 0 && threadIdx.x == 0) { scal->iters += 1; scal->first = 0; }
+  const double alpha = rz / pAp;
+  double a_zz = 0.0;
+  const ChunkIter sched(nchunks, wg, nwg);
+  for (int chunk = sched.chunk; chunk < sched.end; chunk += sched.step) {
+    const int i = chunk * TS + threadIdx.x;
+    if (i < n) {
+      const double ri = r[i] - alpha * Ap[i];
+      const double zi = dinv[i] * ri;
+      x[i] += alpha * p[i];
+      r[i] = ri;
+      z0[i] = w * zi;
+      a_zz += zi * zi;
+    }
+  }
+  const double t1 = block_sum<TS / 64>(a_zz, s4);
+  if (threadIdx.x == 0) {
+    part_zz[wg] = t1;
+    for (int q = wg + nwg; q < P; q += nwg) part_zz[q] = 0.0;
+  }
+}
+
+struct RoleDeal { int ng, mu, mr; };
+template <int UN>
+__global__ __launch_bounds__(TS) __attribute__((amdgpu_waves_per_eu(8, 8))) void k_update_restrict(
+    RoleDeal deal, int parity, Scal* __restrict__ scal, double* __restrict__ part_pAp, double* __restrict__ part_rz,
+    int n, int nchunks_u, int P, double* __restrict__ part_zz, double* __restrict__ x, double* __restrict__ r,
+    const double* __restrict__ p, const double* __restrict__ Ap, const double* __restrict__ dinv, double w, double* __restrict__ z0,
+    int nrow, int nchunks_r, int rpc, const int32_t* __restrict__ rowptr, const float* __restrict__ vals, double* __restrict__ b1,
+    ColComp comp) {
+  const unsigned g = blockIdx.x % deal.ng, j = blockIdx.x / deal.ng, m = deal.mu + deal.mr;
+  const unsigned ub = j * deal.mu / m;
+  if ((j + 1) * deal.mu / m > ub)
+    pcg_update_amg_role(n, nchunks_u, P, parity, scal, part_pAp, part_rz, part_zz, x, r, p, Ap, dinv, w, z0, ub * deal.ng + g,
+                        deal.mu * deal.ng);
+  else
+    spmv_role<16, true, float, UN, false>(nrow, nchunks_r, rpc, rowptr, nullptr, vals, Ap, b1, scal, part_pAp, nullptr, nullptr, nullptr,
+                                          part_rz, nullptr, 0.0, P, parity, comp, (j - ub) * deal.ng + g, deal.mr * deal.ng);
+}
+
+}
diff --git a/heatflow_amd/csrc/hf_solver.hpp b/heatflow_amd/csrc/hf_solver.hpp
--- a/heatflow_amd/csrc/hf_solver.hpp
+++ b/heatflow_amd/csrc/hf_solver.hpp
@@ -327,8 +327,70 @@
   else launch_vec_t<VMODE, double>(c, m, m.val, x, y);
 }
 
+inline bool gate_capable(const DevCsr& m) { return m.rpc > 0 || m.lanes <= 64; }
+void launch_vec_gate(hf_ctx* c, const DevCsr& m, const double* x, double* y) {
+  if (m.rpc > 0) { launch_stream<0>(c, m, x, y, nullptr, nullptr, c->d_part_zz); return; }
+  const long long threads = static_cast<long long>(m.nrow) * m.lanes;
+  const int grid = static_cast<int>(std::max(1LL, std::min<long long>((threads + TPB - 1) / TPB, 2048)));
+#define HF_VEC_GATE(L)                                                                                                                  \
+  do {                                                                                                                                  \
+    if (m.valf != nullptr)                                                                                                              \
+      hipLaunchKernelGGL((k_spmv_vec_gate<L, float>), dim3(grid), dim3(TPB), 0, c->stream, m.nrow, m.ptr, m.idx, m.valf, x, y, c->d_scal, \
+                         c->d_part_zz, c->P);                                                                                          \
+    else                                                                                                                                \
+      hipLaunchKernelGGL((k_spmv_vec_gate<L, double>), dim3(grid), dim3(TPB), 0, c->stream, m.nrow, m.ptr, m.idx, m.val, x, y, c->d_scal, \
+                         c->d_part_zz, c->P);                                                                                          \
+  } while (0)
+  switch (m.lanes) {
+    case 4: HF_VEC_GATE(4); break;
+    case 8: HF_VEC_GATE(8); break;
+    case 16: HF_VEC_GATE(16); break;
+    case 32: HF_VEC_GATE(32); break;
+    default: HF_VEC_GATE(64); break;
+  }
+#undef HF_VEC_GATE
+}
+
+inline bool restrict_recurrence_enabled() {
+  static const bool on = std::getenv("HEATFLOW_RESTRICT_RECURRENCE") && std::getenv("HEATFLOW_RESTRICT_RECURRENCE")[0] == '1';
+  return on;
+}
+inline bool restrict_recurrence(const hf_ctx* c) {
+  if (!restrict_recurrence_enabled() || c->amg.size() < 3) return false;
+  const DevCsr& Rt = c->amg[0].Rt;
+  const bool pipelined = HF_PIPE >= 1 && Rt.nrow > 0 && Rt.rpc > 0 && Rt.cid != nullptr && Rt.valf != nullptr;
+  return pipelined && c->amg[0].GP.nrow == 0 && !c->amg_fine_stale && gate_capable(c->amg[1].Rt);
+}
+
+int launch_update_restrict(hf_ctx* c, double* x, int parity) {
+  static const int share = std::getenv("HEATFLOW_UPDATE_SHARE") ? std::max(5, std::min(95, std::atoi(std::getenv("HEATFLOW_UPDATE_SHARE")))) : 50;
+  hf_ctx* ctx = c;
+  const DevCsr& m = c->amg[0].Rt;
+  const bool un4 = short_chunks(m);
+  const size_t smem = static_cast<size_t>(m.chunk_nnz + m.max_dict) * 8;
+  if (c->amg[0].ur_resident == 0) {
+    int per_cu = 0, ncu = 0;
+    const void* fn = un4 ? reinterpret_cast<const void*>(&k_update_restrict<4>) : reinterpret_cast<const void*>(&k_update_restrict<8>);
+    HF_HIP(hipOccupancyMaxActiveBlocksPerMultiprocessor(&per_cu, fn, TS, smem));
+    HF_HIP(hipDeviceGetAttribute(&ncu, hipDeviceAttributeMultiprocessorCount, c->dev));
+    c->amg[0].ur_resident = std::max(16, per_cu * ncu);
+  }
+  const int nchunks_u = (c->n + TS - 1) / TS;
+  const int want_u = std::max(1, std::min(c->amg[0].ur_resident - 1, static_cast<int>(static_cast<long long>(c->amg[0].ur_resident) * share / 100)));
+  RoleDeal deal{1, std::min({want_u, c->P, nchunks_u}), std::min(c->amg[0].ur_resident - want_u, m.nchunks)};
+  if (deal.mu >= 8 && deal.mr >= 8) { deal.ng = 8; deal.mu >>= 3; deal.mr >>= 3; }
+  const int grid = deal.ng * (deal.mu + deal.mr);
+#define HF_UR_ARGS deal, parity, c->d_scal, c->d_part_pAp, c->d_part_rz, c->n, nchunks_u, c->P, c->d_part_zz, x, c->d_r, c->d_p, c->d_Ap, \
+                   c->d_dinv, c->amg[0].omega, c->d_z, m.nrow, m.nchunks, m.rpc, m.ptr, m.valf, c->amg[1].b,                            \
+                   ColComp{m.dptr, m.dict, m.cid, m.chunk_nnz, 0}
+  if (un4) hipLaunchKernelGGL((k_update_restrict<4>), dim3(grid), dim3(TS), smem, c->stream, HF_UR_ARGS);
+  else hipLaunchKernelGGL((k_update_restrict<8>), dim3(grid), dim3(TS), smem, c->stream, HF_UR_ARGS);
+#undef HF_UR_ARGS
+  return HF_OK;
+}
+
 enum CyclePart { CYCLE_ALL = 0, CYCLE_FIRST = 1, CYCLE_REST = 2 };
-void vcycle(hf_ctx* c, int out_slot, bool test_convergence = false, CyclePart part = CYCLE_ALL) {
+void vcycle(hf_ctx* c, int out_slot, bool test_convergence = false, CyclePart part = CYCLE_ALL, bool behind_first_leg = false) {
   const int nl = static_cast<int>(c->amg.size());
   DevLevel& L0 = c->amg[0];
   if (nl == 1) {
@@ -337,7 +399,9 @@
     return;
   }
   const bool fused0 = L0.GP.nrow > 0;
-  if (L0.Rt.nrow > 0 && (fused0 || !c->amg_fine_stale)) {
+  if (behind_first_leg) {
+    if (part != CYCLE_REST) launch_vec_gate(c, c->amg[1].Rt, c->amg[1].b, c->amg[2].b);
+  } else if (L0.Rt.nrow > 0 && (fused0 || !c->amg_fine_stale)) {
     if (part != CYCLE_REST) launch_stream<0>(c, L0.Rt, c->d_r, c->amg[1].b, nullptr, nullptr, test_convergence ? c->d_part_zz : nullptr);
   } else {
     if (part != CYCLE_REST)
@@ -346,7 +410,7 @@
     if (part != CYCLE_FIRST) launch_vec<0>(c, L0.R, c->d_tmp, c->amg[1].b);
   }
   if (part == CYCLE_FIRST) return;
-  for (int l = 1; l + 1 < nl; ++l) launch_vec<0>(c, c->amg[l].Rt, c->amg[l].b, c->amg[l + 1].b);
+  for (int l = behind_first_leg ? 2 : 1; l + 1 < nl; ++l) launch_vec<0>(c, c->amg[l].Rt, c->amg[l].b, c->amg[l + 1].b);
   {
     DevLevel& Lc = c->amg[nl - 1];
     if (c->coarse_n > 0) {
@@ -370,12 +434,18 @@
 }
 
 void launch_amg_iteration(hf_ctx* c, double* x, int parity, CyclePart part = CYCLE_ALL) {
-  if (part == CYCLE_REST) { vcycle(c, parity ^ 1, true, CYCLE_REST); return; }
+  const bool recur = restrict_recurrence(c);
+  if (part == CYCLE_REST) { vcycle(c, parity ^ 1, true, CYCLE_REST, recur); return; }
   const bool timed = c->prof && c->prof_used < PROF_PAIRS;
   hipEvent_t e0 = timed ? c->prof_ev[2 * c->prof_used] : nullptr, e1 = timed ? c->prof_ev[2 * c->prof_used + 1] : nullptr;
   launch_spmv<9>(c, c->d_A, c->d_z2, c->d_Ap, c->d_part_pAp, nullptr, c->d_p, c->d_part_rz, c->d_part_zz, 0.0, nullptr, e0,
                  e1, parity);
   if (timed) c->prof_used++;
+  if (recur) {
+    (void)launch_update_restrict(c, x, parity);
+    vcycle(c, parity ^ 1, true, part, true);
+    return;
+  }
   hipLaunchKernelGGL(k_pcg_update_amg, dim3(c->P), dim3(TPB), 0, c->stream, c->n, c->nchunks, c->P, parity, c->d_scal,
                      c->d_part_pAp, c->d_part_rz, c->d_part_zz, x, c->d_r, c->d_p, c->d_Ap, c->d_dinv,
                      c->amg[0].omega, c->amg[0].GP.nrow > 0 ? static_cast<double*>(nullptr) : c->d_z);
diff --git a/heatflow_amd/csrc/hf_spmv_body.inc b/heatflow_amd/csrc/hf_spmv_body.inc
--- /dev/null
+++ b/heatflow_amd/csrc/hf_spmv_body.inc
@@ -0,0 +1,391 @@
+  extern __shared__ double sprod[];
+  __shared__ double s4[TS / 64];
+  __shared__ int s_own;
+  constexpr bool BDF = MODE >= 12 && MODE <= 15;
+  auto opnd = [&](int c) { return BDF ? bdf2_operand(x[c], bvec[c]) : x[c]; };
+  if ((MODE == 3 || MODE == 4 || MODE == 6 || MODE == 9 || MODE == 16) && scal->done) return;
+  if ((MODE == 0 || MODE == 7) && scal != nullptr && scal->done) return;
+  double acc0 = 0.0, acc1 = 0.0, acc2 = 0.0;
+  double beta = 0.0;
+  double alpha = 0.0;
+  bool first9 = false;
+  if (MODE == 9) {
+    first9 = scal->first != 0;
+    if (!first9) {
+      double v0 = 0.0, v1 = 0.0, v2 = 0.0;
+      for (int k = threadIdx.x; k < npart; k += TS) {
+        v0 += part1[parity * MAXP + k];
+        v1 += part1[(parity ^ 1) * MAXP + k];
+        v2 += part2[k];
+      }
+      const double rz_new = block_sum<TS / 64>(v0, s4);
+      const double rz_old = block_sum<TS / 64>(v1, s4);
+      const double zz = block_sum<TS / 64>(v2, s4);
+      const bool conv = zz <= scal->tol2;
+      if (HF_WG == 0 && threadIdx.x == 0) {
+        scal->zz = zz;
+        if (conv) scal->done = 1;
+      }
+      if (conv) return;
+      beta = rz_new / rz_old;
+    }
+  }
+  auto cycle_gate = [&]() {
+    if (!((MODE == 3 || MODE == 0) && part2 != nullptr)) return false;
+    double v2 = 0.0;
+    for (int k = threadIdx.x; k < npart; k += TS) v2 += part2[k];
+    const double zz = block_sum<TS / 64>(v2, s4);
+    const bool conv = zz <= scal->tol2;
+    if (HF_WG == 0 && threadIdx.x == 0) {
+      if (conv) { scal->zz = zz; scal->done = 1; }
+      mirror_publish(scal->mirror, zz, scal->iters, conv ? 1 : 0, scal->epoch);
+    }
+    return conv;
+  };
+  constexpr bool PIPELINED = C16 && !VC && (HF_PIPE == 2 || (HF_PIPE == 1 && sizeof(VT) == 4));
+  static_assert(MODE != 16 || PIPELINED, "the recurrence of the restricted residual runs in the chunk pipeline only");
+  static_assert(!VC || (C16 && sizeof(VT) == 8), "value lists: the fine operator's f64 arrays on compressed columns");
+  if (!PIPELINED && cycle_gate()) return;
+  const ChunkIter sched(HF_SCHED);
+  HF_STAMP(0);
+  int stamp_at = 1;
+  (void)stamp_at;
+  const int tpr = (MODE == 0 || MODE == 6 || MODE == 7 || MODE == 16) ? TS / rpc : 1;
+  const int prel = static_cast<int>(threadIdx.x) / tpr;
+  const int psub = static_cast<int>(threadIdx.x) % tpr;
+  struct RowOps { double b, d, y, p, x; };
+  auto row_operands = [&](int prc, bool from_slice) {
+    RowOps e{0.0, 0.0, 0.0, 0.0, 0.0};
+    if (MODE == 2 || MODE == 3 || MODE == 4 || MODE == 5 || MODE == 7 || MODE == 8 || MODE == 11 || MODE == 13 || MODE == 15) e.b = bvec[prc];
+    if (MODE == 2 || MODE == 4 || MODE == 5 || MODE == 10 || MODE == 11 || MODE == 14 || MODE == 15) e.d = dinv[prc];
+    if (MODE == 6 || MODE == 16 || (MODE == 9 && !first9)) e.y = y[prc];
+    if (MODE == 9 && !first9) e.p = pvec[prc];
+    if ((MODE == 4 || MODE == 8 || MODE == 9 || MODE == 11) && !from_slice) e.x = x[prc];
+    if (BDF) e.x = x[prc];
+    return e;
+  };
+  auto rows_phase = [&](bool pin, int prow, int pa, int pb, const RowOps& e) {
+    if ((MODE == 0 || MODE == 6 || MODE == 7 || MODE == 16) && tpr > 1) {
+      double s = 0.0;
+      if (pin)
+        for (int j = pa + psub; j < pb; j += tpr) s += sprod[j];
+      for (int o = tpr >> 1; o > 0; o >>= 1) s += __shfl_down(s, o, 64);
+      if (pin && psub == 0) {
+        y[prow] = (MODE == 6) ? e.y + s : (MODE == 16) ? e.y - alpha * s : s;
+        if (MODE == 7) acc0 += e.b * s;
+      }
+    } else if (pin) {
+      const int row = prow;
+      double s = 0.0;
+      for (int j = pa; j < pb; ++j) s += sprod[j];
+      if (MODE == 0) {
+        y[row] = s;
+      } else if (MODE == 2) {
+        const double ri = e.b - s;
+        const double zi = e.d * ri;
+        y[row] = ri;
+        pvec[row] = zi;
+        acc0 += ri * zi;
+        acc1 += zi * zi;
+        acc2 += (e.d * e.b) * (e.d * e.b);
+      } else if (MODE == 3) {
+        y[row] = e.b - s;
+      } else if (MODE == 4) {
+        const double yi = e.x + w * e.d * (e.b - s);
+        y[row] = yi;
+        acc0 += e.b * yi;
+      } else if (MODE == 5) {
+        const double ri = e.b - s;
+        y[row] = ri;
+        pvec[row] = w * e.d * ri;
+        acc1 += (e.d * ri) * (e.d * ri);
+        acc2 += (e.d * e.b) * (e.d * e.b);
+      } else if (MODE == 7) {
+        y[row] = s;
+        acc0 += e.b * s;
+      } else if (MODE == 6) {
+        y[row] = e.y + s;
+      } else if (MODE == 16) {
+        y[row] = e.y - alpha * s;
+      } else if (MODE == 8) {
+        y[row] = s;
+        pvec[row] = 2.0 * e.x - e.b;
+      } else if (MODE == 10) {
+        y[row] = s + w * e.d;
+      } else if (MODE == 11) {
+        y[row] = s + w * e.d;
+        pvec[row] = 2.0 * e.x - e.b;
+      } else if (BDF) {
+        y[row] = (MODE == 14 || MODE == 15) ? s + w * e.d : s;
+        pvec[row] = (MODE == 13 || MODE == 15) ? 2.0 * e.x - e.b : e.x;
+      } else {
+        const double api = first9 ? s : s + beta * e.y;
+        const double pi = first9 ? e.x : e.x + beta * e.p;
+        y[row] = api;
+        pvec[row] = pi;
+        acc0 += pi * api;
+      }
+    }
+  };
+  if (PIPELINED) {
+    struct Bounds { int k0, k1, d0, d1; };
+    auto bounds = [&](int ch) {
+      Bounds q;
+      const int a0 = ch * rpc, a1 = min(n, a0 + rpc);
+      q.k0 = rowptr[a0]; q.k1 = rowptr[a1];
+      q.d0 = comp.dptr[ch]; q.d1 = comp.dptr[ch + 1];
+      return q;
+    };
+    int lhead[HF_STAGE_U];
+    double v[UN];
+    int id[UN];
+    auto heads = [&](const Bounds& q, bool live) {
+      const int dl = max(q.d1 - 1, 0), kl = max(q.k1 - 1, 0);
+      const int t = static_cast<int>(threadIdx.x);
+#pragma unroll
+      for (int u = 0; u < HF_STAGE_U; ++u) lhead[u] = comp.dict[min(q.d0 + (live ? t + u * TS : (t & 31)), dl)];
+      __builtin_amdgcn_sched_barrier(0);
+#pragma unroll
+      for (int u = 0; u < UN; ++u) {
+        const int kk = min(q.k0 + (live ? t + u * TS : (t & 31)), kl);
+        v[u] = static_cast<double>(stream_load(&vals[kk]));
+        id[u] = static_cast<int>(stream_load(&comp.id[kk]));
+      }
+    };
+    double* xd = sprod + comp.xd_off;
+    Bounds cur = bounds(min(sched.chunk, nchunks - 1));
+    heads(cur, sched.chunk < sched.end);
+    if (cycle_gate()) return;
+    if (MODE == 16) {
+      const double pAp = sum_partials_wide<TS>(part0, npart, s4);
+      const double rz = sum_partials_wide<TS>(part1 + parity * MAXP, npart, s4);
+      if (!(pAp > 0.0)) return;
+      alpha = rz / pAp;
+    }
+    for (int chunk = sched.chunk; chunk < sched.end; chunk += sched.step) {
+      const bool more = chunk + sched.step < sched.end;
+      const int r0 = chunk * rpc, r1 = min(n, r0 + rpc);
+      const int k0 = cur.k0, k1 = cur.k1, d0 = cur.d0, nd = cur.d1 - cur.d0;
+      const int prow = r0 + prel;
+      const bool pin = prow < r1;
+      const int prc = min(prow, r1 - 1);
+      int c0[HF_STAGE_U];
+      double x0[HF_STAGE_U];
+#pragma unroll
+      for (int u = 0; u < HF_STAGE_U; ++u) { c0[u] = lhead[u]; x0[u] = opnd(c0[u]); }
+      const Bounds nxt = bounds(more ? chunk + sched.step : chunk);
+      const int pa = rowptr[prc] - k0, pb = rowptr[prc + 1] - k0;
+      RowOps e = row_operands(prc, comp.own != 0);
+#pragma unroll
+      for (int u = 0; u < HF_STAGE_U; ++u) {
+        const int i = static_cast<int>(threadIdx.x) + u * TS;
+        if (i < nd) {
+          xd[i] = x0[u];
+          if ((MODE == 4 || MODE == 8 || MODE == 9 || MODE == 11) && c0[u] == r0) s_own = i;
+        }
+      }
+      for (int i = threadIdx.x + HF_STAGE_U * TS; i < nd; i += HF_STAGE_U * TS) {
+        int c[HF_STAGE_U];
+        double xv[HF_STAGE_U];
+#pragma unroll
+        for (int u = 0; u < HF_STAGE_U; ++u) c[u] = comp.dict[d0 + min(i + u * TS, nd - 1)];
+#pragma unroll
+        for (int u = 0; u < HF_STAGE_U; ++u) xv[u] = opnd(c[u]);
+#pragma unroll
+        for (int u = 0; u < HF_STAGE_U; ++u)
+          if (i + u * TS < nd) {
+            xd[i + u * TS] = xv[u];
+            if ((MODE == 4 || MODE == 8 || MODE == 9 || MODE == 11) && c[u] == r0) s_own = i + u * TS;
+          }
+      }
+      __syncthreads();
+      HF_STAMP(stamp_at); ++stamp_at;
+      if ((MODE == 4 || MODE == 8 || MODE == 9 || MODE == 11) && comp.own && pin) e.x = xd[s_own + (prow - r0)];
+#pragma unroll
+      for (int u = 0; u < UN; ++u) {
+        const int kk = k0 + static_cast<int>(threadIdx.x) + u * TS;
+        if (kk < k1) sprod[kk - k0] = v[u] * xd[id[u]];
+      }
+      for (int kb = k0 + UN * TS; kb < k1; kb += UN * TS) {
+#pragma unroll
+        for (int u = 0; u < UN; ++u) {
+          const int kk = min(kb + static_cast<int>(threadIdx.x) + u * TS, k1 - 1);
+          v[u] = static_cast<double>(stream_load(&vals[kk]));
+          id[u] = static_cast<int>(stream_load(&comp.id[kk]));
+        }
+#pragma unroll
+        for (int u = 0; u < UN; ++u) {
+          const int kk = kb + static_cast<int>(threadIdx.x) + u * TS;
+          if (kk < k1) sprod[kk - k0] = v[u] * xd[id[u]];
+        }
+      }
+      heads(nxt, more);
+      __syncthreads();
+      HF_STAMP(stamp_at); ++stamp_at;
+      rows_phase(pin, prow, pa, pb, e);
+      __syncthreads();
+      HF_STAMP(stamp_at); ++stamp_at;
+      cur = nxt;
+    }
+  } else {
+  const ChunkIter& sched_ = sched;
+  for (int chunk = sched_.chunk; chunk < sched_.end; chunk += sched_.step) {
+    const int r0 = chunk * rpc;
+    const int r1 = min(n, r0 + rpc);
+    const int k0 = rowptr[r0];
+    const int k1 = rowptr[r1];
+    const int prow = r0 + prel;
+    const bool pin = prow < r1;
+    int pa = 0, pb = 0;
+    if (pin) {
+      pa = rowptr[prow] - k0;
+      pb = rowptr[prow + 1] - k0;
+    }
+    RowOps e = row_operands(min(prow, r1 - 1), C16 && comp.own != 0);
+    if constexpr (VC) {
+      double* xd = sprod + comp.xd_off;
+      double* vl = sprod + comp.vl_off;
+      const int d0 = comp.dptr[chunk], nd = comp.dptr[chunk + 1] - d0;
+      const int v0 = comp.vptr[chunk], nv = comp.vptr[chunk + 1] - v0;
+      const bool vin = nv <= comp.vcap;
+      int k = k0 + threadIdx.x;
+      std::uint32_t cw[HF_UNROLL];
+#pragma unroll
+      for (int u = 0; u < HF_UNROLL; ++u) cw[u] = (k + u * TS < k1) ? stream_load(&comp.cv[k + u * TS]) : 0u;
+      double lv[2];
+#pragma unroll
+      for (int u = 0; u < 2; ++u) {
+        const int i = static_cast<int>(threadIdx.x) + u * TS;
+        lv[u] = (vin && i < nv) ? comp.vlist[v0 + i] : 0.0;
+      }
+      for (int i = threadIdx.x; i < nd; i += HF_STAGE_U * TS) {
+        int c[HF_STAGE_U];
+        double xv[HF_STAGE_U];
+#pragma unroll
+        for (int u = 0; u < HF_STAGE_U; ++u) c[u] = (i + u * TS < nd) ? comp.dict[d0 + i + u * TS] : 0;
+#pragma unroll
+        for (int u = 0; u < HF_STAGE_U; ++u) xv[u] = (i + u * TS < nd) ? opnd(c[u]) : 0.0;
+#pragma unroll
+        for (int u = 0; u < HF_STAGE_U; ++u)
+          if (i + u * TS < nd) {
+            xd[i + u * TS] = xv[u];
+            if ((MODE == 4 || MODE == 8 || MODE == 9 || MODE == 11) && c[u] == r0) s_own = i + u * TS;
+          }
+      }
+#pragma unroll
+      for (int u = 0; u < 2; ++u) {
+        const int i = static_cast<int>(threadIdx.x) + u * TS;
+        if (vin && i < nv) vl[i] = lv[u];
+      }
+      if (vin)
+        for (int i = threadIdx.x + 2 * TS; i < nv; i += TS) vl[i] = comp.vlist[v0 + i];
+      __syncthreads();
+      HF_STAMP(stamp_at); ++stamp_at;
+      if ((MODE == 4 || MODE == 8 || MODE == 9 || MODE == 11) && comp.own && pin) e.x = xd[s_own + (prow - r0)];
+      while (k < k1) {
+        const int kn = k + HF_UNROLL * TS;
+        std::uint32_t cn[HF_UNROLL];
+#pragma unroll
+        for (int u = 0; u < HF_UNROLL; ++u) cn[u] = (kn + u * TS < k1) ? stream_load(&comp.cv[kn + u * TS]) : 0u;
+        if (vin) {
+#pragma unroll
+          for (int u = 0; u < HF_UNROLL; ++u)
+            if (k + u * TS < k1) sprod[k - k0 + u * TS] = vl[cw[u] >> 16] * xd[cw[u] & 0xffffu];
+        } else {
+          double gv[HF_UNROLL];
+#pragma unroll
+          for (int u = 0; u < HF_UNROLL; ++u) gv[u] = (k + u * TS < k1) ? comp.vlist[v0 + static_cast<int>(cw[u] >> 16)] : 0.0;
+#pragma unroll
+          for (int u = 0; u < HF_UNROLL; ++u)
+            if (k + u * TS < k1) sprod[k - k0 + u * TS] = gv[u] * xd[cw[u] & 0xffffu];
+        }
+#pragma unroll
+        for (int u = 0; u < HF_UNROLL; ++u) cw[u] = cn[u];
+        k = kn;
+      }
+    } else if (C16) {
+      double* xd = sprod + comp.xd_off;
+      const int d0 = comp.dptr[chunk], nd = comp.dptr[chunk + 1] - d0;
+      int k = k0 + threadIdx.x;
+      double v[HF_UNROLL];
+      int id[HF_UNROLL];
+#pragma unroll
+      for (int u = 0; u < HF_UNROLL; ++u) {
+        const bool in = k + u * TS < k1;
+        v[u] = in ? static_cast<double>(stream_load(&vals[k + u * TS])) : 0.0;
+        id[u] = in ? static_cast<int>(stream_load(&comp.id[k + u * TS])) : 0;
+      }
+      for (int i = threadIdx.x; i < nd; i += HF_STAGE_U * TS) {
+        int c[HF_STAGE_U];
+        double xv[HF_STAGE_U];
+#pragma unroll
+        for (int u = 0; u < HF_STAGE_U; ++u) c[u] = (i + u * TS < nd) ? comp.dict[d0 + i + u * TS] : 0;
+#pragma unroll
+        for (int u = 0; u < HF_STAGE_U; ++u) xv[u] = (i + u * TS < nd) ? opnd(c[u]) : 0.0;
+#pragma unroll
+        for (int u = 0; u < HF_STAGE_U; ++u)
+          if (i + u * TS < nd) {
+            xd[i + u * TS] = xv[u];
+            if ((MODE == 4 || MODE == 8 || MODE == 9 || MODE == 11) && c[u] == r0) s_own = i + u * TS;
+          }
+      }
+      __syncthreads();
+      HF_STAMP(stamp_at); ++stamp_at;
+      if ((MODE == 4 || MODE == 8 || MODE == 9 || MODE == 11) && comp.own && pin) e.x = xd[s_own + (prow - r0)];
+      while (k < k1) {
+        const int kn = k + HF_UNROLL * TS;
+        double vn[HF_UNROLL];
+        int idn[HF_UNROLL];
+#pragma unroll
+        for (int u = 0; u < HF_UNROLL; ++u) {
+          const bool in = kn + u * TS < k1;
+          vn[u] = in ? static_cast<double>(stream_load(&vals[kn + u * TS])) : 0.0;
+          idn[u] = in ? static_cast<int>(stream_load(&comp.id[kn + u * TS])) : 0;
+        }
+#pragma unroll
+        for (int u = 0; u < HF_UNROLL; ++u)
+          if (k + u * TS < k1) sprod[k - k0 + u * TS] = v[u] * xd[id[u]];
+#pragma unroll
+        for (int u = 0; u < HF_UNROLL; ++u) { v[u] = vn[u]; id[u] = idn[u]; }
+        k = kn;
+      }
+    } else {
+      for (int k = k0 + threadIdx.x; k < k1; k += HF_UNROLL * TS) {
+        int c[HF_UNROLL];
+        double v[HF_UNROLL], xv[HF_UNROLL];
+#pragma unroll
+        for (int u = 0; u < HF_UNROLL; ++u) {
+          const bool in = k + u * TS < k1;
+          c[u] = in ? colidx[k + u * TS] : 0;
+          v[u] = in ? static_cast<double>(vals[k + u * TS]) : 0.0;
+        }
+#pragma unroll
+        for (int u = 0; u < HF_UNROLL; ++u) xv[u] = (k + u * TS < k1) ? opnd(c[u]) : 0.0;
+#pragma unroll
+        for (int u = 0; u < HF_UNROLL; ++u)
+          if (k + u * TS < k1) sprod[k - k0 + u * TS] = v[u] * xv[u];
+      }
+    }
+    __syncthreads();
+    HF_STAMP(stamp_at); ++stamp_at;
+    rows_phase(pin, prow, pa, pb, e);
+    __syncthreads();
+    HF_STAMP(stamp_at); ++stamp_at;
+  }
+  }
+  if (MODE == 2 || MODE == 7 || MODE == 9 || (MODE == 4 && part0 != nullptr)) {
+    const double t0 = block_sum<TS / 64>(acc0, s4);
+    if (threadIdx.x == 0) {
+      part0[HF_WG] = t0;
+      for (int q = HF_WG + HF_NWG; q < npart; q += HF_NWG) part0[q] = 0.0;
+    }
+  }
+  if (MODE == 2 || MODE == 5) {
+    const double t1 = block_sum<TS / 64>(acc1, s4);
+    const double t2 = block_sum<TS / 64>(acc2, s4);
+    if (threadIdx.x == 0) {
+      part1[HF_WG] = t1;
+      part2[HF_WG] = t2;
+      for (int q = HF_WG + HF_NWG; q < npart; q += HF_NWG) { part1[q] = 0.0; part2[q] = 0.0; }
+    }
+  }
diff --git a/heatflow_amd/hip_backend.py b/heatflow_amd/hip_backend.py
--- a/heatflow_amd/hip_backend.py
+++ b/heatflow_amd/hip_backend.py
@@ -26,7 +26,7 @@
 EXPORTS = [
     "hf_version", "hf_create", "hf_destroy", "hf_last_error", "hf_set_mesh", "hf_set_mesh_prebuilt", "hf_pattern_export_size",
     "hf_pattern_export", "hf_amg_export_size", "hf_amg_export", "hf_amg_install", "hf_set_materials",
-    "hf_update_kappa", "hf_set_dirichlet", "hf_assemble", "hf_set_time_scheme", "hf_set_precond", "hf_set_start_vector", "hf_get_response_solves", "hf_get_amg_info", "hf_get_amg_fallbacks", "hf_set_state", "hf_get_state", "hf_sample", "hf_step", "hf_run",
+    "hf_update_kappa", "hf_set_dirichlet", "hf_assemble", "hf_set_time_scheme", "hf_set_precond", "hf_set_start_vector", "hf_get_response_solves", "hf_get_amg_info", "hf_get_iteration_form", "hf_debug_level_rhs", "hf_get_amg_fallbacks", "hf_set_state", "hf_get_state", "hf_sample", "hf_step", "hf_run",
     "hf_batch_begin", "hf_batch_load_column", "hf_batch_set_affine", "hf_batch_set_state", "hf_batch_get_state", "hf_batch_run", "hf_batch_run_flux", "hf_batch_end",
     "hf_flux_setup", "hf_flux_project", "hf_flux_solve", "hf_flux_sample",
     "hf_steady_setup", "hf_steady_solve", "hf_steady_picard_setup", "hf_steady_picard_solve", "hf_set_load", "hf_get_load", "hf_hold_load",
@@ -107,6 +107,8 @@
         "hf_get_response_solves": [vp, C.POINTER(i64)],
         "hf_get_amg_info": [vp, pi, pi, i32, pd, pd],
         "hf_get_amg_fallbacks": [vp, C.POINTER(i64)],
+        "hf_get_iteration_form": [vp, pi],
+        "hf_debug_level_rhs": [vp, i32, pd, i64],
         "hf_set_state": [vp, pd],
         "hf_get_state": [vp, pd],
         "hf_sample": [vp, i32, pi, pd],
@@ -333,6 +335,17 @@
         return {"levels": nl.value, "rows": rows[:nl.value].tolist(), "op_complexity": opc.value, "setup_s": secs.value,
                 "jacobi_fallbacks": fb.value}
 
+    def iteration_form(self):
+        f = C.c_int32()
+        self._check(self._lib.hf_get_iteration_form(self._ctx, C.byref(f)))
+        return int(f.value)
+
+    def debug_level_rhs(self, level):
+        rows = self.amg_info()["rows"]
+        out = np.zeros(rows[level], dtype=np.float64)
+        self._check(self._lib.hf_debug_level_rhs(self._ctx, int(level), _pd(out), out.size))
+        return out
+
     def assemble(self, dt, mode=ASM_LDS_ATOMIC):
         self._check(self._lib.hf_assemble(self._ctx, float(dt), int(mode)))
 
diff --git a/include/heatflow_hip.h b/include/heatflow_hip.h
--- a/include/heatflow_hip.h
+++ b/include/heatflow_hip.h
@@ -59,6 +59,9 @@
 int hf_set_precond(hf_ctx* ctx, int32_t kind, int32_t reuse);
 int hf_get_amg_info(hf_ctx* ctx, int32_t* n_levels, int32_t* level_rows, int32_t max_levels, double* op_complexity,
                     double* setup_seconds);
+
+int hf_get_iteration_form(hf_ctx* ctx, int32_t* form);
+int hf_debug_level_rhs(hf_ctx* ctx, int32_t level, double* out, int64_t n);
 
 int hf_amg_export_size(hf_ctx* ctx, int64_t* bytes);
 int hf_amg_export(hf_ctx* ctx, void* blob, int64_t bytes);
```
